# florianwechsung/alfi

Measured on AMD Instinct MI355X. Metric: V-cycles/sec on ldc3d P2-P0 (DoF*smooths/sec in dof_smooths_per_s), higher is better.
Workload: dtype f64

## Files before the change

### alfi_amd/_lib.py

```python
import ctypes
import os

from . import env

_HERE = os.path.dirname(os.path.abspath(__file__))
LIB_PATH = env.hip_lib() or os.path.join(_HERE, "libalfi_hip.so")

c_i32p = ctypes.POINTER(ctypes.c_int32)
c_i64p = ctypes.POINTER(ctypes.c_int64)
c_f64p = ctypes.POINTER(ctypes.c_double)
vp = ctypes.c_void_p


class CsrHost(ctypes.Structure):
    _fields_ = [("nrows", ctypes.c_int64), ("ncols", ctypes.c_int64), ("rowptr", vp), ("colidx", vp), ("vals", vp)]


class BsrHost(ctypes.Structure):
    _fields_ = [("nbrows", ctypes.c_int64), ("nbcols", ctypes.c_int64), ("rowptr", vp), ("colidx", vp), ("vals", vp)]


SIGNATURES = {
    "alfi_ctx_create": (ctypes.c_int, [ctypes.c_int, vp, ctypes.POINTER(vp)]),
    "alfi_ctx_destroy": (ctypes.c_int, [vp]),
# ... 6 lines not shown
    "alfi_memset0": (ctypes.c_int, [vp, vp, ctypes.c_int64]),
    "alfi_prof_enable": (ctypes.c_int, [vp, ctypes.c_int]),
    "alfi_prof_reset": (ctypes.c_int, [vp]),
    "alfi_prof_get": (ctypes.c_int, [vp, ctypes.c_int, ctypes.POINTER(ctypes.c_double), ctypes.POINTER(ctypes.c_int64)]),
    "alfi_prof_get_level": (ctypes.c_int, [vp, ctypes.c_int, ctypes.c_int, ctypes.POINTER(ctypes.c_double),
                                           ctypes.POINTER(ctypes.c_int64)]),
    "alfi_ctx_set_comm": (ctypes.c_int, [vp, vp, vp, vp, ctypes.c_int64]),
    "alfi_comm_unique_id": (ctypes.c_int, [vp, ctypes.c_int64]),
    "alfi_ctx_comm_init": (ctypes.c_int, [vp, vp, ctypes.c_int, ctypes.c_int]),
    "alfi_level_set_sum_exchange": (ctypes.c_int, [vp, ctypes.c_int, vp, vp, vp, ctypes.c_int64, vp, vp, vp]),
    "alfi_ctx_comm_stats": (ctypes.c_int, [vp, ctypes.POINTER(ctypes.c_int64), ctypes.POINTER(ctypes.c_int64),
                                           ctypes.POINTER(ctypes.c_int64), ctypes.c_int]),
    "alfi_ctx_comm_size": (ctypes.c_int, [vp, ctypes.POINTER(ctypes.c_int), ctypes.POINTER(ctypes.c_int)]),
    "alfi_ctx_comm_destroy": (ctypes.c_int, [vp]),
    "alfi_level_set_neighbours": (ctypes.c_int, [vp, ctypes.c_int, vp, vp, vp]),
    "alfi_level_set_partition": (ctypes.c_int, [vp, ctypes.c_int64, ctypes.c_int, ctypes.c_int64, vp, vp, vp,
                                                ctypes.c_int64]),
    "alfi_level_set_overlap": (ctypes.c_int, [vp, ctypes.c_int64, ctypes.c_int64]),
    "alfi_level_id": (ctypes.c_int, [vp, ctypes.POINTER(ctypes.c_int)]),
    "alfi_level_create": (ctypes.c_int, [vp, ctypes.c_int64, ctypes.c_int, vp, vp, vp, vp, ctypes.c_int64,
                                         ctypes.POINTER(vp)]),
    "alfi_level_destroy": (ctypes.c_int, [vp]),
    "alfi_level_update_values": (ctypes.c_int, [vp, vp]),
    "alfi_ctx_comm_allow_self": (ctypes.c_int, [vp, ctypes.c_int]),
    "alfi_vec_axpy": (ctypes.c_int, [vp, vp, vp, ctypes.c_double, ctypes.c_int64]),
    "alfi_vec_copy": (ctypes.c_int, [vp, vp, vp, ctypes.c_int64]),
    "alfi_vec_gather": (ctypes.c_int, [vp, vp, vp, vp, ctypes.c_int64, ctypes.c_int]),
    "alfi_vec_gather_csr": (ctypes.c_int, [vp, vp, vp, vp, vp, vp, ctypes.c_int64, ctypes.c_int]),
    "alfi_level_zero_bc": (ctypes.c_int, [vp, vp]),
    "alfi_saddle_dot": (ctypes.c_int, [vp, vp, vp, ctypes.POINTER(ctypes.c_double)]),
    "alfi_transfer_stats": (ctypes.c_int, [ctypes.POINTER(ctypes.c_int64), ctypes.POINTER(ctypes.c_int64), ctypes.c_int]),
    "alfi_level_halo_sum": (ctypes.c_int, [vp, vp]),
    "alfi_level_set_assembly": (ctypes.c_int, [vp, ctypes.c_int64, ctypes.c_int, vp, vp, vp, vp, vp, vp, ctypes.c_int, vp, vp, vp]),
    "alfi_ctx_set_assembly_scratch": (ctypes.c_int, [vp, ctypes.c_int64]),
    "alfi_level_assemble_supg": (ctypes.c_int, [vp, ctypes.c_double, ctypes.c_double, ctypes.c_double, vp, ctypes.c_double,
                                                ctypes.c_double, ctypes.c_int]),
    "alfi_level_assemble": (ctypes.c_int, [vp, ctypes.c_double, ctypes.c_double, ctypes.c_double, vp, ctypes.c_int]),
    "alfi_level_set_assembly_bc": (ctypes.c_int, [vp, vp, ctypes.c_int64]),
    "alfi_level_assembly_state_size": (ctypes.c_int, [vp, ctypes.POINTER(ctypes.c_int64)]),
    "alfi_level_assemble_mult": (ctypes.c_int, [vp, ctypes.c_double, ctypes.c_double, ctypes.c_double, vp, vp, vp]),
    "alfi_level_set_supg": (ctypes.c_int, [vp, ctypes.c_int, vp, vp, vp, vp, vp]),
    "alfi_level_supg": (ctypes.c_int, [vp, ctypes.c_double, ctypes.c_double, ctypes.c_double, vp, ctypes.c_int, vp]),
    "alfi_level_set_supg_load": (ctypes.c_int, [vp, vp]),
    "alfi_level_assemble_gls": (ctypes.c_int, [vp, ctypes.c_double, ctypes.c_double, ctypes.c_double, vp, vp, ctypes.c_double,
                                               ctypes.c_double, ctypes.c_int]),
    "alfi_level_gls": (ctypes.c_int, [vp, ctypes.c_double, ctypes.c_double, ctypes.c_double, vp, vp, ctypes.c_int, vp]),
    "alfi_level_apply_bc": (ctypes.c_int, [vp]),
    "alfi_level_set_facet_blocks": (ctypes.c_int, [vp, ctypes.c_int]),
    "alfi_level_set_burman": (ctypes.c_int, [vp, ctypes.c_int64, ctypes.c_int, ctypes.c_int, ctypes.c_int, ctypes.c_int] + [vp] * 14),
    "alfi_level_burman": (ctypes.c_int, [vp, ctypes.c_double, vp, ctypes.c_int, vp]),
    "alfi_patches_set_facet_correction": (ctypes.c_int, [vp, ctypes.c_int64, ctypes.c_int64, vp, vp, vp, vp]),
    "alfi_level_set_facet_beta": (ctypes.c_int, [vp, vp, ctypes.c_double]),
    "alfi_level_assemble_burman": (ctypes.c_int, [vp, ctypes.c_double, ctypes.c_double, ctypes.c_double, vp, ctypes.c_double,
                                                  ctypes.c_int]),
    "alfi_level_transpose": (ctypes.c_int, [vp]),
    "alfi_level_get_values": (ctypes.c_int, [vp, vp]),
    "alfi_level_size": (ctypes.c_int, [vp, ctypes.POINTER(ctypes.c_int64)]),
    "alfi_spmv": (ctypes.c_int, [vp, vp, vp]),
    "alfi_residual": (ctypes.c_int, [vp, vp, vp, vp]),
    "alfi_patches_set": (ctypes.c_int, [vp, ctypes.c_int64, vp, vp]),
    "alfi_patches_factor": (ctypes.c_int, [vp]),
    "alfi_patches_set_groups": (ctypes.c_int, [vp, vp]),
    "alfi_patches_factor_bytes": (ctypes.c_int, [vp, ctypes.POINTER(ctypes.c_int64)]),
    "alfi_patches_find_groups": (ctypes.c_int, [vp, vp]),
    "alfi_ctx_set_condense_min_bytes": (ctypes.c_int, [vp, ctypes.c_int64]),
    "alfi_patches_condensed": (ctypes.c_int, [vp, ctypes.POINTER(ctypes.c_int)]),
    "alfi_patches_set_storage": (ctypes.c_int, [vp, ctypes.c_int]),
    "alfi_patches_storage": (ctypes.c_int, [vp, ctypes.POINTER(ctypes.c_int)]),
    "alfi_patches_set_macro_storage": (ctypes.c_int, [vp, ctypes.c_int]),
    "alfi_ctx_set_f32_work_bytes": (ctypes.c_int, [vp, ctypes.c_int64]),
    "alfi_ctx_f32_work_bytes": (ctypes.c_int, [vp, ctypes.POINTER(ctypes.c_int64)]),
    "alfi_patches_set_canonical_order": (ctypes.c_int, [vp, vp]),
    "alfi_patch_apply_split": (ctypes.c_int, [vp, ctypes.c_int64, vp, vp]),
    "alfi_patches_check": (ctypes.c_int, [vp, ctypes.POINTER(ctypes.c_double), ctypes.POINTER(ctypes.c_int64),
                                          ctypes.POINTER(ctypes.c_int64), ctypes.POINTER(ctypes.c_double)]),
    "alfi_patches_set_partition_of_unity": (ctypes.c_int, [vp, ctypes.c_int]),
    "alfi_patches_set_multiplicative": (ctypes.c_int, [vp, ctypes.c_int64, vp, ctypes.c_int]),
    "alfi_patches_multiplicative_levels": (ctypes.c_int, [vp, ctypes.POINTER(ctypes.c_int64)]),
    "alfi_patch_apply": (ctypes.c_int, [vp, vp, vp]),
    "alfi_patches_stats": (ctypes.c_int, [vp, ctypes.POINTER(ctypes.c_int64), ctypes.POINTER(ctypes.c_int64),
                                          ctypes.POINTER(ctypes.c_int64)]),
    "alfi_patch_get_inverse": (ctypes.c_int, [vp, ctypes.c_int64, vp]),
    "alfi_smooth_fgmres": (ctypes.c_int, [vp, ctypes.c_int, vp, vp, ctypes.c_int]),
    "alfi_level_set_jacobi": (ctypes.c_int, [vp, ctypes.c_int]),
    "alfi_smooth_chebyshev": (ctypes.c_int, [vp, ctypes.c_int, ctypes.c_double, ctypes.c_double, vp, vp, ctypes.c_int]),
    "alfi_level_arnoldi": (ctypes.c_int, [vp, ctypes.c_int, vp, vp, ctypes.POINTER(ctypes.c_int)]),
    "alfi_coarse_factor": (ctypes.c_int, [vp]),
    "alfi_coarse_factor_sparse": (ctypes.c_int, [vp, vp, ctypes.c_int, ctypes.c_int]),
    "alfi_coarse_factor_bytes": (ctypes.c_int, [vp, ctypes.POINTER(ctypes.c_int64)]),
    "alfi_coarse_residual": (ctypes.c_int, [vp, ctypes.POINTER(ctypes.c_double)]),
    "alfi_coarse_set_inverse": (ctypes.c_int, [vp, vp, ctypes.c_int]),
    "alfi_coarse_solve": (ctypes.c_int, [vp, vp, vp]),
    "alfi_transfer_create": (ctypes.c_int, [vp, vp, vp, ctypes.POINTER(BsrHost), ctypes.POINTER(BsrHost),
                                            ctypes.POINTER(BsrHost), ctypes.POINTER(BsrHost), ctypes.POINTER(BsrHost),
                                            ctypes.c_int64, ctypes.c_int, vp, vp, vp, ctypes.POINTER(vp)]),
    "alfi_transfer_destroy": (ctypes.c_int, [vp]),
    "alfi_transfer_update": (ctypes.c_int, [vp, ctypes.c_double, ctypes.c_double]),
    "alfi_transfer_get_block_inverse": (ctypes.c_int, [vp, ctypes.c_int64, vp]),
    "alfi_prolong": (ctypes.c_int, [vp, vp, vp]),
    "alfi_transfer_set_injection": (ctypes.c_int, [vp, vp]),
    "alfi_transfer_set_injection_matrix": (ctypes.c_int, [vp, ctypes.POINTER(CsrHost)]),
    "alfi_inject": (ctypes.c_int, [vp, vp, vp]),
    "alfi_restrict": (ctypes.c_int, [vp, vp, vp, ctypes.c_int]),
    "alfi_mg_create": (ctypes.c_int, [vp, ctypes.c_int, ctypes.POINTER(vp), ctypes.POINTER(vp), ctypes.c_int,
                                      ctypes.c_int, ctypes.POINTER(vp)]),
    "alfi_mg_destroy": (ctypes.c_int, [vp]),
    "alfi_mg_vcycle": (ctypes.c_int, [vp, vp, vp]),
    "alfi_mg_fcycle": (ctypes.c_int, [vp, vp, vp]),
    "alfi_mg_set_smoother": (ctypes.c_int, [vp, ctypes.c_int, vp, vp]),
    "alfi_mg_set_cycles": (ctypes.c_int, [vp, ctypes.c_int]),
    "alfi_mg_cg": (ctypes.c_int, [vp, vp, vp, ctypes.c_double, ctypes.c_double, ctypes.c_int, ctypes.c_int,
                                  ctypes.POINTER(ctypes.c_int), ctypes.POINTER(ctypes.c_double)]),
    "alfi_ctx_set_graph": (ctypes.c_int, [vp, ctypes.c_int]),
    "alfi_saddle_create": (ctypes.c_int, [vp, ctypes.POINTER(CsrHost), ctypes.POINTER(CsrHost), vp, ctypes.c_double,
                                          ctypes.c_double, ctypes.c_int, ctypes.POINTER(vp)]),
    "alfi_saddle_destroy": (ctypes.c_int, [vp]),
    "alfi_saddle_set_mass_inverse": (ctypes.c_int, [vp, ctypes.POINTER(CsrHost)]),
    "alfi_saddle_update": (ctypes.c_int, [vp, ctypes.c_double, ctypes.c_double]),
    "alfi_saddle_solve": (ctypes.c_int, [vp, vp, vp, ctypes.c_double, ctypes.c_double, ctypes.c_int, ctypes.c_int,
                                         ctypes.POINTER(ctypes.c_int), ctypes.POINTER(ctypes.c_double)]),
    "alfi_level_halo_forward": (ctypes.c_int, [vp, vp]),
    "alfi_level_halo_reverse_add": (ctypes.c_int, [vp, vp]),
    "alfi_csr_create": (ctypes.c_int, [vp, ctypes.POINTER(CsrHost), ctypes.POINTER(vp)]),
    "alfi_csr_destroy": (ctypes.c_int, [vp]),
    "alfi_csr_mult": (ctypes.c_int, [vp, vp, vp, vp, ctypes.c_double, ctypes.c_int]),
    "alfi_saddle_mult": (ctypes.c_int, [vp, vp, vp]),
    "alfi_saddle_precond": (ctypes.c_int, [vp, vp, vp]),
    "alfi_saddle_set_velocity_solver": (ctypes.c_int, [vp, ctypes.c_int]),
    "alfi_saddle_factor_velocity": (ctypes.c_int, [vp, vp, ctypes.c_int, ctypes.c_int, ctypes.c_int64]),
    "alfi_saddle_velocity_solve": (ctypes.c_int, [vp, vp, vp]),
    "alfi_saddle_velocity_info": (ctypes.c_int, [vp, ctypes.POINTER(ctypes.c_int64), ctypes.POINTER(ctypes.c_double)]),
    "alfi_ctx_set_block_kernels": (ctypes.c_int, [vp, ctypes.c_int]),
    "alfi_patch_apply_block_info": (ctypes.c_int, [vp, ctypes.POINTER(ctypes.c_int)]),
    "alfi_spmv_block_info": (ctypes.c_int, [vp, ctypes.POINTER(ctypes.c_int)]),
    "alfi_patch_apply_block_width": (ctypes.c_int, [vp, ctypes.POINTER(ctypes.c_int)]),
    "alfi_spmv_block_width": (ctypes.c_int, [vp, ctypes.POINTER(ctypes.c_int)]),
    "alfi_ctx_set_block_lds_bytes": (ctypes.c_int, [vp, ctypes.c_int64]),
    "alfi_patch_apply_block": (ctypes.c_int, [vp, ctypes.c_int, vp, ctypes.c_int, vp, ctypes.c_int64, vp, ctypes.c_int64]),
    "alfi_spmv_block": (ctypes.c_int, [vp, ctypes.c_int, vp, ctypes.c_int, vp, ctypes.c_int64, vp, ctypes.c_int64]),
    "alfi_residual_block": (ctypes.c_int, [vp, ctypes.c_int, vp, ctypes.c_int, vp, ctypes.c_int64, vp, ctypes.c_int64, vp,
                                           ctypes.c_int64]),
    "alfi_smooth_fgmres_block_info": (ctypes.c_int, [vp, ctypes.c_int, ctypes.POINTER(ctypes.c_int)]),
    "alfi_smooth_fgmres_block_mode": (ctypes.c_int, [vp, ctypes.c_int, ctypes.POINTER(ctypes.c_int)]),
    "alfi_ctx_set_block_fused": (ctypes.c_int, [vp, ctypes.c_int]),
    "alfi_smooth_fgmres_block": (ctypes.c_int, [vp, ctypes.c_int, ctypes.c_int, vp, ctypes.c_int, vp, ctypes.c_int64, vp,
                                                ctypes.c_int64, ctypes.c_int]),
    "alfi_mg_vcycle_block": (ctypes.c_int, [vp, ctypes.c_int, vp, ctypes.c_int, vp, ctypes.c_int64, vp, ctypes.c_int64]),
    "alfi_mg_fcycle_block": (ctypes.c_int, [vp, ctypes.c_int, vp, ctypes.c_int, vp, ctypes.c_int64, vp, ctypes.c_int64]),
    "alfi_saddle_mult_block": (ctypes.c_int, [vp, ctypes.c_int, vp, ctypes.c_int, vp, ctypes.c_int64, vp, ctypes.c_int64]),
    "alfi_saddle_precond_block": (ctypes.c_int, [vp, ctypes.c_int, vp, ctypes.c_int, vp, ctypes.c_int64, vp, ctypes.c_int64]),
    "alfi_saddle_solve_block": (ctypes.c_int, [vp, ctypes.c_int, vp, ctypes.c_int, vp, ctypes.c_int64, vp, ctypes.c_int64,
                                               ctypes.c_double, ctypes.c_double, ctypes.c_int, ctypes.c_int, vp, vp]),
}

COMM_ID_BYTES = 128

EVENTS = ["PATCH_APPLY", "PATCH_SCATTER", "PATCH_FACTOR", "MATMULT", "BLAS1", "PROLONG", "RESTRICT", "COARSE", "COMM"]
PETSC_EVENT_NAMES = {"PATCH_APPLY": "PCPATCHApply", "PATCH_SCATTER": "PCPATCHScatter", "PATCH_FACTOR": "PCPatchComputeOp",
                     "MATMULT": "MatMult", "BLAS1": "KSPGMRESOrthog", "PROLONG": "SchoeberlProlong", "RESTRICT": "SchoeberlRestrict",
                     "COARSE": "MatSolve", "COMM": "SFBcastOpBegin"}

_lib = None


def comm_unique_id():
    buf = ctypes.create_string_buffer(COMM_ID_BYTES)
    lib = load()
    rc = lib.alfi_comm_unique_id(ctypes.cast(buf, vp), COMM_ID_BYTES)
    if rc != 0:
        raise RuntimeError("alfi_comm_unique_id failed (%d): %s" % (rc, lib.alfi_last_error(None).decode()))
    return buf.raw


def load():
    global _lib
    if _lib is not None:
        return _lib
    try:
        import torch
    except ImportError:
        pass
    if not os.path.exists(LIB_PATH):
        raise RuntimeError("libalfi_hip.so is missing (%s): build it with `python -m alfi_amd.build`; "
                           "alfi_amd has no CPU fallback" % LIB_PATH)
    lib = ctypes.CDLL(LIB_PATH)
    for name, (res, args) in SIGNATURES.items():
        fn = getattr(lib, name)
        fn.restype, fn.argtypes = res, args
    _lib = lib
    return lib
```

### alfi_amd/csrc/api_block.hip

```cpp
#include "api_internal.h"
#include "block_cols.h"

int alfi_ctx_set_block_kernels(alfi_ctx* ctx, int on) {
  if (!ctx) return alfi_set_error(nullptr, ALFI_E_ARG, "NULL context");
  ctx->block_kernels = on != 0;
  return 0;
}
int alfi_ctx_set_block_fused(alfi_ctx* ctx, int on) {
  if (!ctx) return alfi_set_error(nullptr, ALFI_E_ARG, "NULL context");
  ctx->block_fused = on != 0;
  return 0;
}

static int block_apply_waves(const alfi_level* L) {
  if (!L->ctx->block_kernels || !L->factored || L->jacobi || L->mult || level_is_partitioned(L)) return 0;
  if (L->held != HELD_F64 && L->held != HELD_F32) return 0;
  const int W = patch_apply_dense_waves(L, L->held == HELD_F32);
  return patch_apply_block_waves_ok(W) ? W : 0;
}
static int block_cond_apply_width(const alfi_level* L) {
  if (!L->ctx->block_kernels || !L->factored || L->jacobi || L->mult || level_is_partitioned(L)) return 0;
  if (L->held != HELD_COND || L->npatch < COND_PER_PATCH_MIN) return 0;
  if (L->lay.sum_n > INT32_MAX / BLOCK_NV) return 0;
  return block_cond_width(L->cplan.lds_front, L->cplan.lds_back, L->ctx->block_lds_bytes);
}
static int block_big_apply_width(const alfi_level* L) {
  if (!L->ctx->block_kernels || !L->factored || L->jacobi || L->mult || level_is_partitioned(L)) return 0;
  if (L->held != HELD_F64 && L->held != HELD_F32) return 0;
  if (L->lay.max_np <= SMALL_PATCH_MAX || L->npatch < BIG_BLOCK_MIN_PATCHES) return 0;
  if (L->lay.stage_len > INT32_MAX / BLOCK_NV) return 0;
  return block_big_width(L->lay.max_np, L->ctx->block_lds_bytes);
}
static int block_piece_apply_width(const alfi_level* L) {
  return L->held == HELD_COND ? block_cond_apply_width(L) : block_big_apply_width(L);
}
static int block_apply_width(const alfi_level* L) {
  return block_apply_waves(L) != 0 ? BLOCK_NV : block_piece_apply_width(L);
}
static int block_spmv_width(const alfi_level* L) {
  if (!L->ctx->block_kernels || level_is_partitioned(L)) return 0;
  const int w = bsr_spmv_block_width(L->A_own, L->ctx->block_lds_bytes);
  return w >= 2 ? w : 0;
}

int alfi_patch_apply_block_info(alfi_level* L, int* batched) {
  if (!L || !batched) return alfi_set_error(L ? L->ctx : nullptr, ALFI_E_ARG, "alfi_patch_apply_block_info: NULL argument");
  *batched = block_apply_width(L) >= 2 ? 1 : 0;
  return 0;
}
int alfi_patch_apply_block_width(alfi_level* L, int* width) {
  if (!L || !width) return alfi_set_error(L ? L->ctx : nullptr, ALFI_E_ARG, "alfi_patch_apply_block_width: NULL argument");
  *width = block_apply_width(L);
  return 0;
}
int alfi_ctx_set_block_lds_bytes(alfi_ctx* ctx, int64_t bytes) {
  if (!ctx) return alfi_set_error(nullptr, ALFI_E_ARG, "NULL context");
  int limit = 0;
  ALFI_HIP_CHECK(ctx, hipDeviceGetAttribute(&limit, hipDeviceAttributeMaxSharedMemoryPerBlock, ctx->device));
  ctx->block_lds_bytes = (int)std::min<int64_t>(std::max<int64_t>(bytes, 0), limit);
  return 0;
}
static bool level_applies_il(const alfi_level* L) { return L->il_valid && L->held == HELD_F64; }
static int block_smoother_mode(alfi_level* L, int k) {
  BlockSmoothFacts f;
  f.block_kernels = L->ctx->block_kernels;
  f.block_fused = L->ctx->block_fused;
  f.partitioned = level_is_partitioned(L);
  f.fused_iteration = smoother_takes_fused_iteration(L, k);
  f.applies_il = L->factored && level_applies_il(L);
  f.apply_waves = block_apply_waves(L);
  f.piece_width = block_piece_apply_width(L);
  return block_smooth_mode(f);
}
static bool block_smoother_lockstep(alfi_level* L, int k) { return block_smoother_mode(L, k) == BLOCK_SMOOTH_LOCKSTEP; }
int alfi_smooth_fgmres_block_mode(alfi_level* L, int k, int* mode) {
  if (!L || !mode || k < 1) return alfi_set_error(L ? L->ctx : nullptr, ALFI_E_ARG, "alfi_smooth_fgmres_block_mode: bad argument");
  *mode = block_smoother_mode(L, k);
  return 0;
}
int alfi_smooth_fgmres_block_info(alfi_level* L, int k, int* lockstep) {
  if (!L || !lockstep || k < 1) return alfi_set_error(L ? L->ctx : nullptr, ALFI_E_ARG, "alfi_smooth_fgmres_block_info: bad argument");
  *lockstep = block_smoother_lockstep(L, k) ? 1 : 0;
  return 0;
}
int alfi_spmv_block_info(alfi_level* L, int* batched) {
  if (!L || !batched) return alfi_set_error(L ? L->ctx : nullptr, ALFI_E_ARG, "alfi_spmv_block_info: NULL argument");
  *batched = block_spmv_width(L) >= 2 ? 1 : 0;
  return 0;
}
int alfi_spmv_block_width(alfi_level* L, int* width) {
  if (!L || !width) return alfi_set_error(L ? L->ctx : nullptr, ALFI_E_ARG, "alfi_spmv_block_width: NULL argument");
  *width = block_spmv_width(L);
  return 0;
}

int krylov_ws_ensure(alfi_ctx* ctx, KrylovWs* ws, int slots, int K, int64_t n) {
  if (ws->K == K && ws->slots == slots) return 0;
  ALFI_HIP_CHECK(ctx, hipStreamSynchronize(ctx->stream));
  krylov_ws_release(ws);
  ws->ldv = krylov_ldv(n);
  const KrylovWsDoubles d = krylov_ws_doubles(slots, K, ws->ldv);
  ALFI_CHECK(dev_alloc(ctx, &ws->V, d.V));
  ALFI_CHECK(dev_alloc(ctx, &ws->Z, d.Z));
  ALFI_CHECK(dev_alloc(ctx, &ws->w, d.w));
  ALFI_CHECK(dev_alloc(ctx, &ws->hs, d.hs));
  ALFI_HIP_CHECK(ctx, hipMemsetAsync(ws->hs, 0, sizeof(double) * (size_t)d.hs, ctx->stream));
  ws->K = K;
  ws->slots = slots;
  return 0;
}
void krylov_ws_release(KrylovWs* ws) {
  dev_free(ws->V);
  dev_free(ws->Z);
  dev_free(ws->w);
  dev_free(ws->hs);
  *ws = KrylovWs();
}

int slot_buf_resize(alfi_ctx* ctx, SlotBuf* buf, int slots, int64_t per) {
  ALFI_HIP_CHECK(ctx, hipStreamSynchronize(ctx->stream));
  slot_buf_release(buf);
  ALFI_CHECK(dev_alloc(ctx, &buf->p, slots * per));
  ALFI_HIP_CHECK(ctx, hipMemsetAsync(buf->p, 0, sizeof(double) * (size_t)std::max<int64_t>(slots * per, 1), ctx->stream));
  buf->slots = slots;
  buf->per = per;
  return 0;
}
int slot_buf_ensure(alfi_ctx* ctx, SlotBuf* buf, int ncol, int64_t per) {
  const int need = slot_buf_needed(*buf, ncol);
  return need == buf->slots ? 0 : slot_buf_resize(ctx, buf, need, per);
}
void slot_buf_release(SlotBuf* buf) {
  dev_free(buf->p);
  *buf = SlotBuf();
}

void block_release_patch_buffers(alfi_level* L) {
  slot_buf_release(&L->blk_stage);
  slot_buf_release(&L->blk_ctmp);
}
void release_workspaces(alfi_level* L) {
  block_release_patch_buffers(L);
  for (SlotBuf* b : {&L->blk_carry, &L->blk_part, &L->blk_mg_b, &L->blk_mg_x, &L->blk_mg_r}) slot_buf_release(b);
  krylov_ws_release(&L->ws);
  krylov_ws_release(&L->blk_ws);
}
void release_workspaces(alfi_saddle* S) {
  slot_buf_release(&S->blk_tmp_u);
  krylov_ws_release(&S->ws);
  krylov_ws_release(&S->blk_ws);
}

static int ensure_block_smoother(alfi_level* L, int ncol) {
  return krylov_ws_ensure(L->ctx, &L->blk_ws, block_slots_needed(L->blk_ws.slots, ncol), L->ws.K, L->n);
}

int block_patch_apply(alfi_level* L, const BlockCols& ic, const BlockCols& oc, const double* X, int64_t ldx, double* Y, int64_t ldy) {
  alfi_ctx* ctx = L->ctx;
  ctx->cur_tag = L->id;
  const int W = ic.n > 1 ? block_apply_waves(L) : 0;
  if (W != 0) {
    ALFI_CHECK(slot_buf_ensure(ctx, &L->blk_stage, ic.n, L->lay.stage_len));
    return launch_patch_apply_block(L, W, ic, oc, X, ldx, Y, ldy, L->blk_stage.p);
  }
  const int width = ic.n > 1 ? block_piece_apply_width(L) : 0;
  for (int k = 0; k < block_pieces(ic.n, width); ++k) {
    const BlockCols pi = block_piece(ic, width, k), po = block_piece(oc, width, k);
    if (pi.n == 1) {
      ALFI_CHECK(level_patch_apply(L, X + pi.c[0] * ldx, Y + po.c[0] * ldy));
      continue;
    }
    ALFI_CHECK(slot_buf_ensure(ctx, &L->blk_stage, pi.n, L->lay.stage_len));
    if (L->held != HELD_COND) {
      ALFI_CHECK(launch_big_apply_block(L, pi, po, X, ldx, Y, ldy, L->blk_stage.p));
      continue;
    }
    ALFI_CHECK(slot_buf_ensure(ctx, &L->blk_ctmp, pi.n, L->lay.sum_n));
    ALFI_CHECK(launch_cond_apply_block(L, pi, po, X, ldx, Y, ldy, L->blk_stage.p, L->blk_ctmp.p));
  }
  return 0;
}

int block_spmv(alfi_level* L, const BlockCols& ic, const BlockCols& oc, const double* X, int64_t ldx, double* Y, int64_t ldy,
               const double* B, int64_t ldb, int mode) {
  alfi_ctx* ctx = L->ctx;
  ctx->cur_tag = L->id;
  const int width = ic.n > 1 ? block_spmv_width(L) : 0;
  for (int k = 0; k < block_pieces(ic.n, width); ++k) {
    const BlockCols pi = block_piece(ic, width, k), po = block_piece(oc, width, k);
    if (pi.n == 1) {
      ALFI_CHECK(level_spmv(L, X + pi.c[0] * ldx, Y + po.c[0] * ldy, mode ? B + pi.c[0] * ldb : nullptr, mode));
      continue;
    }
    const DevBSR& A = L->A_own;
    if (!A.aligned) {
      const int64_t nchunks = (A.nnzb + SPMV_CHUNK - 1) / SPMV_CHUNK;
      ALFI_CHECK(slot_buf_ensure(ctx, &L->blk_carry, pi.n, nchunks * A.bs));
    }
    ProfScope prof(ctx, ALFI_EV_MATMULT);
    ALFI_CHECK(launch_bsr_spmv_block(ctx, A, pi, po, X, ldx, Y, ldy, B, ldb, 1.0, mode, L->blk_carry.p));
  }
  return 0;
}

static int block_smooth_fgmres_fused(alfi_level* L, int k, const BlockCols& cols, const double* B, int64_t ldb, double* X, int64_t ldx,
                                     int nonzero_guess) {
  alfi_ctx* ctx = L->ctx;
  const int nc = cols.n;
  ALFI_CHECK(ensure_block_smoother(L, nc));
  ALFI_CHECK(slot_buf_ensure(ctx, &L->blk_part, nc, block_partial_per_slot(RED_BLOCKS, RED_MAXV)));
  ALFI_CHECK(slot_buf_ensure(ctx, &L->blk_stage, nc, L->lay.stage_len));
  if (L->held == HELD_COND) ALFI_CHECK(slot_buf_ensure(ctx, &L->blk_ctmp, nc, L->lay.sum_n));
  const int64_t ldv = L->blk_ws.ldv;
  const BlockCols slots = block_chunk(nc, nullptr, 0);
  if (nonzero_guess) ALFI_CHECK(block_spmv(L, cols, slots, X, ldx, L->blk_ws.w, ldv, B, ldb, 1));
  {
    ProfScope prof(ctx, ALFI_EV_BLAS1);
    ALFI_CHECK(launch_first_norm_block(L, cols, nonzero_guess ? nullptr : B, ldb, X, ldx));
  }
  const int G = red_blocks_for(L->n);
  const bool il = level_applies_il(L);
  const int W = il ? 0 : block_apply_waves(L), width = il || W != 0 ? BLOCK_NV : block_piece_apply_width(L);
  const double* stage[BLOCK_NV];
  for (int s = 0; s < BLOCK_NV; ++s) stage[s] = L->blk_stage.slot(s < nc ? s : 0);
  for (int j = 0; j < k; ++j) {
    if (il) {
      ALFI_CHECK(launch_patch_apply_il_block(L, nc, L->blk_ws.w, ldv, L->blk_stage.p));
    } else if (W != 0) {
      ALFI_CHECK(launch_patch_apply_block(L, W, slots, slots, L->blk_ws.w, ldv, nullptr, 0, L->blk_stage.p));
    } else {
      for (int q = 0; q < block_pieces(nc, width); ++q) {
        const BlockCols pi = block_piece(slots, width, q);
        double* st = L->blk_stage.slot(pi.c[0]);
        if (pi.n == 1) {
          ALFI_CHECK(launch_patch_apply_range(L, 0, L->npatch, L->blk_ws.wv(pi.c[0])));
          stage[pi.c[0]] = L->stage;
        } else if (L->held != HELD_COND) {
          ALFI_CHECK(launch_big_apply_block(L, pi, pi, L->blk_ws.w, ldv, nullptr, 0, st));
        } else {
          ALFI_CHECK(launch_cond_apply_block(L, pi, pi, L->blk_ws.w, ldv, nullptr, 0, st, L->blk_ctmp.p));
        }
      }
    }
    {
      ProfScope prof(ctx, ALFI_EV_PATCH_SCATTER);
      ALFI_CHECK(launch_patch_sum_scale_block(L, nc, stage, j == 0 ? 0 : 1, G, j));
    }
    int nb = 0;
    {
      ProfScope prof(ctx, ALFI_EV_MATMULT);
      ALFI_CHECK(launch_bsr_spmv_dot_block(L, nc, j, &nb));
    }
    ProfScope prof(ctx, ALFI_EV_BLAS1);
    ALFI_CHECK(launch_multi_axpy_norm_block(L, nc, j, nb));
  }
  ProfScope prof(ctx, ALFI_EV_BLAS1);
  return launch_fgmres_finish_update_block(L, cols, k, G, X, ldx);
}

int block_smooth_fgmres(alfi_level* L, int k, const BlockCols& cols, const double* B, int64_t ldb, double* X, int64_t ldx,
                        int nonzero_guess) {
  ALFI_CHECK(ensure_fgmres_workspace(L, k));
  L->ctx->cur_tag = L->id;
  const int mode = cols.n == 1 ? BLOCK_SMOOTH_LOOP : block_smoother_mode(L, k);
  if (mode == BLOCK_SMOOTH_FUSED) return block_smooth_fgmres_fused(L, k, cols, B, ldb, X, ldx, nonzero_guess);
  if (mode == BLOCK_SMOOTH_LOOP) {
    for (int i = 0; i < cols.n; ++i) ALFI_CHECK(alfi_smooth_fgmres(L, k, B + cols.c[i] * ldb, X + cols.c[i] * ldx, nonzero_guess));
    return 0;
  }
  ALFI_CHECK(ensure_block_smoother(L, cols.n));
  return smooth_fgmres_general(L, L->blk_ws, k, cols, B, ldb, X, ldx, nonzero_guess);
}

int check_block_call(alfi_level* L, const char* what, int ncol, const int* cols, int nx, const BlockOperand* ops, int nops) {
  if (!L) return alfi_set_error(nullptr, ALFI_E_ARG, "%s: NULL level", what);
  if (level_is_partitioned(L)) return alfi_set_error(L->ctx, ALFI_E_ARG, "%s on a partitioned level (serial levels only)", what);
  return check_block_operands(L->ctx, what, L->n, ncol, cols, nx, ops, nops);
}
int check_block_operands(alfi_ctx* ctx, const char* what, int64_t n, int ncol, const int* cols, int nx, const BlockOperand* ops,
                         int nops) {
  for (int a = 0; a < nops; ++a) {
    if (!ops[a].p) return alfi_set_error(ctx, ALFI_E_ARG, "%s: NULL operand", what);
    if (const char* err = block_operand_error(n, ncol, cols, nx, ops[a].ld)) return alfi_set_error(ctx, ALFI_E_ARG, "%s: %s", what, err);
  }
  for (int a = 0; a < nops; ++a)
    for (int b = 0; b < nops; ++b)
      if (a != b && ops[a].written && block_operands_overlap(ops[a].p, ops[a].ld, ops[b].p, ops[b].ld, nx, n))
        return alfi_set_error(ctx, ALFI_E_ARG, "%s: an operand that is written overlaps another one", what);
  return 0;
}

int alfi_patch_apply_block(alfi_level* L, int ncol, const int* cols, int nx, const double* X, int64_t ldx, double* Y, int64_t ldy) {
  const BlockOperand ops[2] = {{X, ldx, false}, {Y, ldy, true}};
  ALFI_CHECK(check_block_call(L, "alfi_patch_apply_block", ncol, cols, nx, ops, 2));
  if (!level_pc_ready(L)) return alfi_set_error(L->ctx, ALFI_E_STATE, "alfi_patch_apply_block before alfi_patches_factor");
  for (int q = 0; q < block_chunks(ncol); ++q) {
    const BlockCols c = block_chunk(ncol, cols, q);
    ALFI_CHECK(block_patch_apply(L, c, c, X, ldx, Y, ldy));
  }
  return 0;
}

int alfi_spmv_block(alfi_level* L, int ncol, const int* cols, int nx, const double* X, int64_t ldx, double* Y, int64_t ldy) {
  const BlockOperand ops[2] = {{X, ldx, false}, {Y, ldy, true}};
  ALFI_CHECK(check_block_call(L, "alfi_spmv_block", ncol, cols, nx, ops, 2));
  for (int q = 0; q < block_chunks(ncol); ++q) {
    const BlockCols c = block_chunk(ncol, cols, q);
    ALFI_CHECK(block_spmv(L, c, c, X, ldx, Y, ldy, nullptr, 0, 0));
  }
  return 0;
}

int alfi_residual_block(alfi_level* L, int ncol, const int* cols, int nx, const double* B, int64_t ldb, const double* X, int64_t ldx,
                        double* R, int64_t ldr) {
  const BlockOperand ops[3] = {{B, ldb, false}, {X, ldx, false}, {R, ldr, true}};
  ALFI_CHECK(check_block_call(L, "alfi_residual_block", ncol, cols, nx, ops, 3));
  for (int q = 0; q < block_chunks(ncol); ++q) {
    const BlockCols c = block_chunk(ncol, cols, q);
    ALFI_CHECK(block_spmv(L, c, c, X, ldx, R, ldr, B, ldb, 1));
  }
  return 0;
}

int alfi_smooth_fgmres_block(alfi_level* L, int k, int ncol, const int* cols, int nx, const double* B, int64_t ldb, double* X,
                             int64_t ldx, int nonzero_guess) {
  const BlockOperand ops[2] = {{B, ldb, false}, {X, ldx, true}};
  ALFI_CHECK(check_block_call(L, "alfi_smooth_fgmres_block", ncol, cols, nx, ops, 2));
  if (k < 1) return alfi_set_error(L->ctx, ALFI_E_ARG, "k must be >= 1");
  if (!level_pc_ready(L)) return alfi_set_error(L->ctx, ALFI_E_STATE, "alfi_smooth_fgmres_block before alfi_patches_factor");
  for (int q = 0; q < block_chunks(ncol); ++q)
    ALFI_CHECK(block_smooth_fgmres(L, k, block_chunk(ncol, cols, q), B, ldb, X, ldx, nonzero_guess));
  return 0;
}
```

### alfi_amd/csrc/api_cycles.hip

```cpp
#include "api_internal.h"
#include "block_cols.h"

int alfi_coarse_set_inverse(alfi_level* L, const double* inv, int inv_is_device) {
  alfi_ctx* ctx = L->ctx;
  ALFI_HIP_CHECK(ctx, hipStreamSynchronize(ctx->stream));
  if (L->cinv_owned) dev_free(L->cinv);
  L->cinv = nullptr;
  L->cinv_owned = false;
  mf_free(L->mf);
  L->mf = nullptr;
  if (inv_is_device) {
    L->cinv = const_cast<double*>(inv);
  } else {
    ALFI_CHECK(dev_upload(ctx, &L->cinv, inv, L->n * L->n));
    L->cinv_owned = true;
  }
  return 0;
}

int alfi_coarse_factor(alfi_level* L) {
  alfi_ctx* ctx = L->ctx;
  if (L->has_halo && L->n_own != L->n)
    return alfi_set_error(ctx, ALFI_E_STATE, "alfi_coarse_factor needs a level owned by one rank");
  if (L->n > ((int64_t)1 << 17)) return alfi_set_error(ctx, ALFI_E_ARG, "coarse level of %lld dofs: the dense inverse would "
// ... 337 lines not shown
  if (par) ALFI_CHECK(halo_rev(T->coarse, drc));
  ProfScope prof(ctx, ALFI_EV_RESTRICT);
  ALFI_CHECK(launch_zero_dofs(ctx, drc, T->coarse->bc_dofs, T->coarse->nbc));
  return 0;
}

int alfi_mg_create(alfi_ctx* ctx, int nlevels, alfi_level** levels, alfi_transfer** transfers, int k,
                   int robust_restriction, alfi_mg** out) {
  if (!ctx || nlevels < 1 || !levels || (nlevels > 1 && !transfers) || !out)
    return alfi_set_error(ctx, ALFI_E_ARG, "bad arguments");
  for (int l = 1; l < nlevels; ++l) {
    if (transfers[l - 1]->coarse != levels[l - 1] || transfers[l - 1]->fine != levels[l])
      return alfi_set_error(ctx, ALFI_E_ARG, "transfer %d does not link levels %d and %d", l - 1, l - 1, l);
  }
  alfi_mg* mg = new alfi_mg();
  mg->ctx = ctx;
  mg->levels.assign(levels, levels + nlevels);
  if (nlevels > 1) mg->transfers.assign(transfers, transfers + nlevels - 1);
  mg->k = k;
  mg->robust = robust_restriction;
  for (int l = 0; l < nlevels; ++l) {
    alfi_level* L = levels[l];
    int rc = 0;
    if (!L->mg_b) rc = dev_alloc(ctx, &L->mg_b, L->n);
    if (rc == 0 && !L->mg_x) rc = dev_alloc(ctx, &L->mg_x, L->n);
    if (rc == 0 && !L->mg_r) rc = dev_alloc(ctx, &L->mg_r, L->n);
    if (rc == 0 && l > 0 && L->n_own > 0) rc = ensure_fgmres_workspace(L, k);
    if (rc != 0) {
      delete mg;
      return rc;
    }
  }
  *out = mg;
  return 0;
}

int alfi_mg_destroy(alfi_mg* mg) {
  if (!mg) return 0;
  (void)hipStreamSynchronize(mg->ctx->stream);
  for (CycleGraph& g : mg->graphs)
    if (g.exec) (void)hipGraphExecDestroy(g.exec);
  dev_free(mg->cg_r);
  dev_free(mg->cg_z);
  dev_free(mg->cg_p);
  dev_free(mg->cg_w);
  dev_free(mg->cg_s);
  delete mg;
  return 0;
}

static int mg_require_serial(alfi_mg* mg, const char* what) {
  for (alfi_level* L : mg->levels)
    if (level_is_partitioned(L)) return alfi_set_error(mg->ctx, ALFI_E_ARG, "%s on a partitioned hierarchy (serial levels only)", what);
  return 0;
}

int alfi_mg_set_smoother(alfi_mg* mg, int type, const double* emin, const double* emax) {
  if (!mg) return alfi_set_error(nullptr, ALFI_E_ARG, "NULL multigrid");
  alfi_ctx* ctx = mg->ctx;
  if (type != ALFI_SMOOTHER_FGMRES && type != ALFI_SMOOTHER_CHEBYSHEV)
    return alfi_set_error(ctx, ALFI_E_ARG, "smoother type %d (0 FGMRES, 1 Chebyshev)", type);
  if (type == ALFI_SMOOTHER_FGMRES) {
    mg->smoother = type;
    return 0;
  }
  ALFI_CHECK(mg_require_serial(mg, "alfi_mg_set_smoother(Chebyshev)"));
  const int nl = (int)mg->levels.size();
  if (nl > 1 && (!emin || !emax)) return alfi_set_error(ctx, ALFI_E_ARG, "Chebyshev smoother without intervals");
  for (int l = 1; l < nl; ++l)
    if (!(emin[l - 1] > 0.0) || !(emax[l - 1] > emin[l - 1]) || !std::isfinite(emax[l - 1]))
      return alfi_set_error(ctx, ALFI_E_ARG, "Chebyshev interval [%g, %g] of level %d: need 0 < emin < emax", emin[l - 1],
                            emax[l - 1], l);
  for (int l = 1; l < nl; ++l) ALFI_CHECK(ensure_cheb_workspace(mg->levels[l]));
  mg->emin.assign((size_t)nl, 0.0);
  mg->emax.assign((size_t)nl, 0.0);
  for (int l = 1; l < nl; ++l) {
    mg->emin[l] = emin[l - 1];
    mg->emax[l] = emax[l - 1];
  }
  mg->smoother = type;
  return 0;
}

int alfi_mg_set_cycles(alfi_mg* mg, int cycles) {
  if (!mg) return alfi_set_error(nullptr, ALFI_E_ARG, "NULL multigrid");
  if (cycles != 1 && cycles != 2) return alfi_set_error(mg->ctx, ALFI_E_ARG, "cycles %d (1 V, 2 W)", cycles);
  if (cycles > 1) ALFI_CHECK(mg_require_serial(mg, "alfi_mg_set_cycles(W)"));
  mg->cycles = cycles;
  return 0;
}

struct MgWork {
  double *b, *x, *r;
  int64_t ld;
};
typedef MgWork (*MgWorkOf)(const alfi_level*);
static MgWork own_work(const alfi_level* L) { return {L->mg_b, L->mg_x, L->mg_r, 0}; }
static MgWork block_work(const alfi_level* L) { return {L->blk_mg_b.p, L->blk_mg_x.p, L->blk_mg_r.p, L->blk_mg_b.per}; }

static int mg_smooth(alfi_mg* mg, int l, const BlockCols& cols, const double* B, int64_t ldb, double* X, int64_t ldx,
                     int nonzero_guess) {
  alfi_level* L = mg->levels[l];
  if (mg->smoother == ALFI_SMOOTHER_CHEBYSHEV) {
    for (int i = 0; i < cols.n; ++i)
      ALFI_CHECK(alfi_smooth_chebyshev(L, mg->k, mg->emin[l], mg->emax[l], B + cols.c[i] * ldb, X + cols.c[i] * ldx, nonzero_guess));
    return 0;
  }
  return block_smooth_fgmres(L, mg->k, cols, B, ldb, X, ldx, nonzero_guess);
}

static int vcycle(alfi_mg* mg, MgWorkOf work, int l, const BlockCols& cols, const double* B, int64_t ldb, double* X, int64_t ldx,
                  bool x_zero) {
  alfi_ctx* ctx = mg->ctx;
  alfi_level* L = mg->levels[l];
  const int nc = cols.n;
  if (l == 0) {
    for (int i = 0; i < nc && L->n_own > 0; ++i) ALFI_CHECK(alfi_coarse_solve(L, B + cols.c[i] * ldb, X + cols.c[i] * ldx));
    return 0;
  }
  alfi_transfer* T = mg->transfers[l - 1];
  const BlockCols slots = block_chunk(nc, nullptr, 0);
  const MgWork wl = work(L), wc = work(mg->levels[l - 1]);
  ALFI_CHECK(mg_smooth(mg, l, cols, B, ldb, X, ldx, x_zero ? 0 : 1));
  ALFI_CHECK(block_spmv(L, cols, slots, X, ldx, wl.r, wl.ld, B, ldb, 1));
  for (int i = 0; i < nc; ++i) ALFI_CHECK(alfi_restrict(T, wl.r + i * wl.ld, wc.b + i * wc.ld, mg->robust));
  const int cycles = l == 1 ? 1 : mg->cycles;
  for (int c = 0; c < cycles; ++c) ALFI_CHECK(vcycle(mg, work, l - 1, slots, wc.b, wc.ld, wc.x, wc.ld, c == 0));
  for (int i = 0; i < nc; ++i) ALFI_CHECK(alfi_prolong(T, wc.x + i * wc.ld, wl.r + i * wl.ld));
  ctx->cur_tag = L->id;
  for (int i = 0; i < nc; ++i) {
    ProfScope prof(ctx, ALFI_EV_BLAS1);
    ALFI_CHECK(launch_axpy(ctx, X + cols.c[i] * ldx, wl.r + i * wl.ld, 1.0, L->n_own));
  }
  return mg_smooth(mg, l, cols, B, ldb, X, ldx, 1);
}

static int fcycle(alfi_mg* mg, MgWorkOf work, const BlockCols& cols, const double* B, int64_t ldb, double* X, int64_t ldx) {
  const int Lmax = (int)mg->levels.size() - 1, nc = cols.n;
  if (Lmax == 0) return vcycle(mg, work, 0, cols, B, ldb, X, ldx, false);
  const BlockCols slots = block_chunk(nc, nullptr, 0);
  for (int i = 0; i < nc; ++i) {
    const double* bf = B + cols.c[i] * ldb;
    for (int l = Lmax; l >= 1; --l) {
      const MgWork wc = work(mg->levels[l - 1]);
      ALFI_CHECK(alfi_restrict(mg->transfers[l - 1], bf, wc.b + i * wc.ld, mg->robust));
      bf = wc.b + i * wc.ld;
    }
  }
  for (int l = 0; l < Lmax; ++l) {
    const MgWork wl = work(mg->levels[l]), wn = work(mg->levels[l + 1]);
    ALFI_CHECK(vcycle(mg, work, l, slots, wl.b, wl.ld, wl.x, wl.ld, l == 0));
    for (int i = 0; i < nc; ++i)
      ALFI_CHECK(alfi_prolong(mg->transfers[l], wl.x + i * wl.ld, l + 1 == Lmax ? X + cols.c[i] * ldx : wn.x + i * wn.ld));
  }
  return vcycle(mg, work, Lmax, cols, B, ldb, X, ldx, false);
}

static void cycle_signature(alfi_mg* mg, std::vector<uint64_t>* sig) {
  auto push = [&](const void* q) { sig->push_back((uint64_t)(uintptr_t)q); };
  auto pushd = [&](double v) {
    uint64_t u;
    memcpy(&u, &v, sizeof(u));
    sig->push_back(u);
  };
  sig->clear();
  sig->push_back((uint64_t)mg->k);
  sig->push_back((uint64_t)mg->robust);
  sig->push_back((uint64_t)mg->smoother);
  sig->push_back((uint64_t)mg->cycles);
  if (mg->smoother == ALFI_SMOOTHER_CHEBYSHEV)
    for (size_t l = 1; l < mg->levels.size(); ++l) {
      pushd(mg->emin[l]);
      pushd(mg->emax[l]);
    }
  for (alfi_level* L : mg->levels) {
    sig->push_back((uint64_t)(L->jacobi ? 1 : 0));
    push(L->jac_diag);
    push(L->cheb_d);
    push(L->A.vals);
    push(L->inv);
    push(L->inv32);
    sig->push_back((uint64_t)(L->held == HELD_F32 ? 1 : 0));
    push(L->cd.mat);
    push(L->cd.sinv);
    push(L->patch_ptr);
    push(L->patch_dofs);
    push(L->cinv);
    push(L->mf);
    push(L->ws.V);
    push(L->mult_seq);
    sig->push_back((uint64_t)L->npatch);
    sig->push_back((uint64_t)L->ws.K);
    sig->push_back((uint64_t)(L->mult ? 1 + (L->mult_symmetrise ? 1 : 0) + 4 * L->sweep.wave_ptr.size() : 0));
  }
  for (alfi_transfer* T : mg->transfers) {
    push(T->binv);
    pushd(T->nu);
    pushd(T->gamma);
  }
}

static int mg_ready(alfi_mg* mg) {
  alfi_ctx* ctx = mg->ctx;
  for (size_t l = 1; l < mg->levels.size(); ++l) {
    alfi_level* L = mg->levels[l];
    if (L->n_own > 0 && !level_pc_ready(L))
      return alfi_set_error(ctx, ALFI_E_STATE, "level %d: patches not factored", (int)l);
    if (mg->smoother == ALFI_SMOOTHER_CHEBYSHEV) ALFI_CHECK(ensure_cheb_workspace(L));
    if (L->jacobi && L->jac_version != L->op_version) {
      ALFI_CHECK(launch_jacobi_diag(ctx, L->A, L->jac_diag));
      L->jac_version = L->op_version;
    }
  }
  alfi_level* C = mg->levels[0];
  if (C->n_own > 0 && !C->cinv && !C->mf) return alfi_set_error(ctx, ALFI_E_STATE, "coarse level has no inverse");
  return 0;
}

static int run_cycle(alfi_mg* mg, int kind, const double* db, double* dx) {
  alfi_ctx* ctx = mg->ctx;
  ALFI_CHECK(mg_ready(mg));
  const BlockCols one = block_chunk(1, nullptr, 0);
  auto eager = [&]() {
    return kind ? fcycle(mg, own_work, one, db, 0, dx, 0) : vcycle(mg, own_work, (int)mg->levels.size() - 1, one, db, 0, dx, 0, false);
  };
  bool ok = ctx->use_graph && ctx->prof == 0;
  for (alfi_level* L : mg->levels) ok = ok && !L->has_halo;
  if (!ok) return eager();
  std::vector<uint64_t> sig;
  cycle_signature(mg, &sig);
  CycleGraph* G = nullptr;
  for (CycleGraph& g : mg->graphs)
    if (g.kind == kind && g.b == db && g.x == dx) G = &g;
  if (!G) {
    if (mg->graphs.size() >= 16) {
      for (CycleGraph& g : mg->graphs)
        if (g.exec) (void)hipGraphExecDestroy(g.exec);
      mg->graphs.clear();
    }
    CycleGraph g;
    g.kind = kind;
    g.b = db;
    g.x = dx;
    mg->graphs.push_back(g);
    return eager();
  }
  if (G->failed) return eager();
  if (G->exec && G->sig != sig) {
    (void)hipGraphExecDestroy(G->exec);
    G->exec = nullptr;
  }
  if (!G->exec) {
// ... 147 lines not shown
```

### alfi_amd/csrc/api_internal.h

```cpp
#pragma once
#include <cmath>
#include <cstdarg>
#include <cstdlib>
#include <cstring>
#include <algorithm>
#include "common.h"
#include "hs_layout.h"

template <typename T>
inline int dev_alloc(alfi_ctx* ctx, T** p, int64_t count) {
  *p = nullptr;
  if (count <= 0) count = 1;
  ALFI_HIP_CHECK(ctx, hipMalloc((void**)p, (size_t)count * sizeof(T)));
  return 0;
}
template <typename T>
inline int dev_upload(alfi_ctx* ctx, T** p, const T* host, int64_t count) {
  ALFI_CHECK(dev_alloc(ctx, p, count));
  if (count > 0) ALFI_HIP_CHECK(ctx, hipMemcpy(*p, host, (size_t)count * sizeof(T), hipMemcpyHostToDevice));
  return 0;
}
inline void dev_free(void* p) {
  if (p) (void)hipFree(p);
}
template <typename T>
inline int cond_upload(alfi_level* L, const T** dst, const std::vector<T>& src) {
  T* d = nullptr;
  ALFI_CHECK(dev_upload(L->ctx, &d, src.data(), (int64_t)src.size()));
  L->cond_allocs.push_back(d);
  *dst = d;
  return 0;
}

int check_dev_err(alfi_ctx* ctx);
int build_chunk_tables(alfi_ctx* ctx, DevBSR* d, const int32_t* rowptr, int64_t nbrows, int64_t break_row,
                       int64_t* nchunks_before = nullptr);
int upload_bsr(alfi_ctx* ctx, DevBSR* d, const alfi_bsr_host* h, int bs);
void free_bsr(DevBSR* d);
void free_cond(alfi_level* L);
int comm_allreduce(alfi_level* L, int64_t offset, int64_t count);
int halo_fwd(alfi_level* L, double* v);
int halo_fwd_begin(alfi_level* L, const double* v);
int halo_fwd_end(alfi_level* L, double* v);
int halo_rev(alfi_level* L, double* v);
int halo_sum(alfi_level* L, double* v);
int halo_rev_begin(alfi_level* L, const double* v);
int halo_rev_end(alfi_level* L, double* v);
void free_assembly(AssemblyDev* S);
int level_spmv(alfi_level* L, const double* dx, double* dy, const double* db, int mode, bool ghosts_current = false);
int level_patch_apply(alfi_level* L, const double* dx, double* dy, bool* ghosts_current = nullptr);
inline bool level_pc_ready(const alfi_level* L) { return L->factored || L->jacobi; }
inline bool level_is_partitioned(const alfi_level* L) { return L->distributed || L->has_halo || L->n_own != L->n; }
inline void set_held(alfi_level* L, PatchStoreHeld h) {
  L->held = h;
  L->cond = h == HELD_COND;
}
inline bool wants_f32(const alfi_level* L) { return L->store_req != STORE_REQ_F64; }
inline bool is_or_will_be_f32(const alfi_level* L) { return wants_f32(L) || L->held == HELD_F32; }
inline bool cond_by_caller(const alfi_level* L) { return L->cond && L->cond_by == COND_BY_CALLER; }
inline bool cond_by_own_choice(const alfi_level* L) { return L->cond && L->cond_by == COND_BY_LIBRARY; }
inline bool facet_rule_active(const alfi_level* L) { return L->fc_ptr && L->fc_scale != 0.0; }
void free_patch_factors(alfi_level* L);
void free_mult_schedule(alfi_level* L);
bool auto_cond_to_dense(alfi_level* L);
int ensure_fgmres_workspace(alfi_level* L, int k);
int ensure_cheb_workspace(alfi_level* L);
bool smoother_takes_fused_iteration(const alfi_level* L, int k, bool* flat_spmv = nullptr);
int smooth_fgmres_general(alfi_level* L, const KrylovWs& ws, int k, const BlockCols& cols, const double* B, int64_t ldb, double* X,
                          int64_t ldx, int nonzero_guess);
int krylov_ws_ensure(alfi_ctx* ctx, KrylovWs* ws, int slots, int K, int64_t n);
void krylov_ws_release(KrylovWs* ws);
int slot_buf_ensure(alfi_ctx* ctx, SlotBuf* buf, int ncol, int64_t per);
int slot_buf_resize(alfi_ctx* ctx, SlotBuf* buf, int slots, int64_t per);
void slot_buf_release(SlotBuf* buf);
void block_release_patch_buffers(alfi_level* L);
void release_workspaces(alfi_level* L);
void release_workspaces(alfi_saddle* S);
struct BlockCols;
struct BlockOperand {
  const double* p;
  int64_t ld;
  bool written;
};
int check_block_call(alfi_level* L, const char* what, int ncol, const int* cols, int nx, const BlockOperand* ops, int nops);
int check_block_operands(alfi_ctx* ctx, const char* what, int64_t n, int ncol, const int* cols, int nx, const BlockOperand* ops,
                         int nops);
int mg_fcycle_block_chunk(alfi_mg* mg, const BlockCols& cols, const double* B, int64_t ldb, double* X, int64_t ldx);
int block_patch_apply(alfi_level* L, const BlockCols& ic, const BlockCols& oc, const double* X, int64_t ldx, double* Y, int64_t ldy);
int block_spmv(alfi_level* L, const BlockCols& ic, const BlockCols& oc, const double* X, int64_t ldx, double* Y, int64_t ldy,
               const double* B, int64_t ldb, int mode);
int block_smooth_fgmres(alfi_level* L, int k, const BlockCols& cols, const double* B, int64_t ldb, double* X, int64_t ldx,
                        int nonzero_guess);
int upload_csr(alfi_ctx* ctx, DevCSR* d, const alfi_csr_host* h);
void free_csr(DevCSR* d);
```

### alfi_amd/csrc/api_saddle.hip

```cpp
#include "api_internal.h"
#include "block_cols.h"

int upload_csr(alfi_ctx* ctx, DevCSR* d, const alfi_csr_host* h) {
  d->nrows = h->nrows;
  d->ncols = h->ncols;
  d->nnz = h->rowptr[h->nrows];
  ALFI_CHECK(dev_upload(ctx, &d->rowptr, h->rowptr, h->nrows + 1));
  ALFI_CHECK(dev_upload(ctx, &d->colidx, h->colidx, d->nnz));
  ALFI_CHECK(dev_upload(ctx, &d->vals, h->vals, d->nnz));
  return 0;
}
void free_csr(DevCSR* d) {
  dev_free(d->rowptr);
  dev_free(d->colidx);
  dev_free(d->vals);
  *d = DevCSR();
}

int alfi_level_halo_forward(alfi_level* L, double* dv) {
  if (!L->distributed) return 0;
  L->ctx->cur_tag = L->id;
  return halo_fwd(L, dv);
}

// ... 435 lines not shown
    ctx->cur_tag = F->id;
    return comm_allreduce(F, offset, count);
  };
  auto list = [&](const bool* on) {
    BlockCols b = block_chunk(nc, nullptr, 0);
    int m = 0;
    for (int s = 0; s < nc; ++s)
      if (on[s]) b.c[m++] = s;
    b.n = m;
    for (int i = m; i < BLOCK_NV; ++i) b.c[i] = m ? b.c[0] : 0;
    return b;
  };
  auto read = [&](const bool* on, int off, double* out) -> int {
    for (int s = 0; s < nc; ++s)
      if (on[s]) ALFI_HIP_CHECK(ctx, hipMemcpyAsync(out + s, ws.h(s) + off, sizeof(double), hipMemcpyDeviceToHost, ctx->stream));
    ALFI_HIP_CHECK(ctx, hipStreamSynchronize(ctx->stream));
    return 0;
  };
  auto norm_init = [&](int s) -> int {
    ALFI_CHECK(launch_norm_partials(ctx, ws.wv(s), n));
    if (par) {
      ALFI_CHECK(launch_reduce_partials(ctx, ctx->red_partial, G, 1, nrm2));
      ALFI_CHECK(allreduce(RED_MAXV, 1));
      return launch_norm_init_finish(ctx, nrm2, 1, ws.h(s), K);
    }
    return launch_norm_init_finish(ctx, ctx->red_partial, G, ws.h(s), K);
  };
  bool active[BLOCK_NV] = {false, false, false, false}, all[BLOCK_NV] = {false, false, false, false};
  double bnorm[BLOCK_NV] = {0, 0, 0, 0}, tol[BLOCK_NV] = {0, 0, 0, 0}, val[BLOCK_NV] = {0, 0, 0, 0};
  int its[BLOCK_NV] = {0, 0, 0, 0};
  for (int s = 0; s < nc; ++s) {
    all[s] = true;
    ALFI_HIP_CHECK(ctx, hipMemsetAsync(ws.h(s), 0, sizeof(double) * hl.total, ctx->stream));
    ALFI_HIP_CHECK(ctx, hipMemsetAsync(xcol(s), 0, sizeof(double) * n, ctx->stream));
    ALFI_CHECK(launch_copy(ctx, ws.wv(s), bcol(s), n));
    ALFI_CHECK(norm_init(s));
  }
  ALFI_CHECK(read(all, hl.beta, bnorm));
  int nactive = 0;
  for (int s = 0; s < nc; ++s) {
    tol[s] = std::max(rtol * bnorm[s], atol);
    active[s] = !(bnorm[s] <= tol[s]);
    nactive += active[s] ? 1 : 0;
  }
  auto residual_of = [&](const bool* on) -> int {
    for (int s = 0; s < nc; ++s) {
      if (!on[s]) continue;
      ALFI_CHECK(alfi_saddle_mult(S, xcol(s), ws.wv(s)));
      ALFI_CHECK(launch_xmy(ctx, ws.wv(s), bcol(s), n));
      ALFI_CHECK(norm_init(s));
    }
    return 0;
  };
  int it = 0;
  while (nactive > 0 && it < max_it) {
    for (int s = 0; s < nc; ++s)
      if (active[s]) ALFI_CHECK(launch_scale_by_inv(ctx, ws.v(s, 0), ws.wv(s), ws.h(s) + hl.beta, n));
    int j = 0;
    bool cycle[BLOCK_NV];
    for (int s = 0; s < nc; ++s) cycle[s] = active[s];
    int ncycle = nactive;
    for (; j < K && it < max_it && ncycle > 0; ++j) {
      const BlockCols a = list(cycle);
      ALFI_CHECK(saddle_precond_chunk(S, a, nc, ws.v(0, j), ws.vs(), ws.z(0, j), ws.zs()));
      ALFI_CHECK(saddle_mult_chunk(S, a, ws.z(0, j), ws.zs(), ws.w, ldv));
      for (int s = 0; s < nc; ++s) {
        if (!cycle[s]) continue;
        double *hs = ws.h(s), *hdots = hdots_of(s);
        ALFI_CHECK(launch_multi_dot(ctx, ws.v(s, 0), ldv, j + 1, ws.wv(s), hdots, n));
        if (par) ALFI_CHECK(allreduce(0, j + 1));
        ALFI_CHECK(launch_multi_axpy_norm(ctx, ws.v(s, 0), ldv, j + 1, hdots, ws.wv(s), n, ctx->red_partial2, 0));
        if (par) {
          ALFI_CHECK(launch_reduce_partials(ctx, ctx->red_partial2, G, 1, nrm2));
          ALFI_CHECK(allreduce(RED_MAXV, 1));
        }
        ALFI_CHECK(launch_hessenberg_update(ctx, normpart, nblk, hdots, hs, j, K, nullptr));
      }
      ++it;
      ALFI_CHECK(read(cycle, hl.grs + j + 1, val));
      for (int s = 0; s < nc; ++s) {
        if (!cycle[s]) continue;
        its[s] = it;
        if (std::fabs(val[s]) <= tol[s]) {
          ALFI_CHECK(launch_fgmres_finish(ctx, ws.h(s), j + 1, K));
          ALFI_CHECK(launch_update_solution(ctx, xcol(s), ws.z(s, 0), ldv, j + 1, ws.h(s) + hl.y, n));
          cycle[s] = active[s] = false;
          --ncycle;
          --nactive;
        } else if (j + 1 < K) {
          ALFI_CHECK(launch_scale_by_inv(ctx, ws.v(s, j + 1), ws.wv(s), ws.h(s) + hl.tt, n));
        }
      }
    }
    for (int s = 0; s < nc; ++s) {
      if (!cycle[s]) continue;
      ALFI_CHECK(launch_fgmres_finish(ctx, ws.h(s), j, K));
      ALFI_CHECK(launch_update_solution(ctx, xcol(s), ws.z(s, 0), ldv, j, ws.h(s) + hl.y, n));
    }
    if (nactive == 0 || it >= max_it) break;
    ALFI_CHECK(residual_of(active));
    ALFI_CHECK(read(active, hl.beta, val));
    for (int s = 0; s < nc; ++s)
      if (active[s] && val[s] <= tol[s]) {
        active[s] = false;
        --nactive;
      }
  }
  ALFI_CHECK(residual_of(all));
  ALFI_CHECK(read(all, hl.beta, val));
  for (int s = 0; s < nc; ++s) {
    its_out[s] = its[s];
    rn_out[s] = val[s];
  }
  return 0;
}

static int check_restart(alfi_ctx* ctx, int restart) {
  if (restart < 1 || restart > RED_MAXV - 2) return alfi_set_error(ctx, ALFI_E_ARG, "restart must be in 1..%d", RED_MAXV - 2);
  return 0;
}

int alfi_saddle_solve(alfi_saddle* S, const double* db, double* dx, double rtol, double atol, int max_it, int restart,
                      int* iterations, double* residual_norm) {
  alfi_ctx* ctx = S->ctx;
  ALFI_CHECK(check_restart(ctx, restart));
  ALFI_CHECK(krylov_ws_ensure(ctx, &S->ws, 1, restart, S->nu_dofs + S->np_dofs));
  int its = 0;
  double rn = 0.0;
  ALFI_CHECK(saddle_solve_chunk(S, S->ws, block_chunk(1, nullptr, 0), db, 0, dx, 0, rtol, atol, max_it, &its, &rn));
  if (iterations) *iterations = its;
  if (residual_norm) *residual_norm = rn;
  return check_dev_err(ctx);
}

int alfi_saddle_solve_block(alfi_saddle* S, int ncol, const int* cols, int nx, const double* B, int64_t ldb, double* X, int64_t ldx,
                            double rtol, double atol, int max_it, int restart, int* iterations, double* residual_norms) {
  const BlockOperand ops[2] = {{B, ldb, false}, {X, ldx, true}};
  ALFI_CHECK(saddle_block_check(S, "alfi_saddle_solve_block", ncol, cols, nx, ops, 2));
  alfi_ctx* ctx = S->ctx;
  if (!iterations || !residual_norms) return alfi_set_error(ctx, ALFI_E_ARG, "alfi_saddle_solve_block: NULL result arrays");
  ALFI_CHECK(check_restart(ctx, restart));
  ALFI_CHECK(krylov_ws_ensure(ctx, &S->blk_ws, block_slots_needed(S->blk_ws.slots, ncol), restart, S->nu_dofs + S->np_dofs));
  for (int q = 0; q < block_chunks(ncol); ++q)
    ALFI_CHECK(saddle_solve_chunk(S, S->blk_ws, block_chunk(ncol, cols, q), B, ldb, X, ldx, rtol, atol, max_it,
                                  iterations + q * BLOCK_NV, residual_norms + q * BLOCK_NV));
  return check_dev_err(ctx);
}
```

### alfi_amd/csrc/api_smoother.hip

```cpp
#include <optional>
#include "api_internal.h"

int ensure_fgmres_workspace(alfi_level* L, int k) {
  if (k <= L->ws.K) return 0;
  if (k > RED_MAXV - 1) return alfi_set_error(L->ctx, ALFI_E_ARG, "k = %d exceeds the supported maximum %d", k, RED_MAXV - 1);
  return krylov_ws_ensure(L->ctx, &L->ws, 1, k, L->n);
}

static int smooth_fgmres_fused(alfi_level* L, int k, const double* db, double* dx, int nonzero_guess, bool flat_spmv) {
  alfi_ctx* ctx = L->ctx;
  const int K = L->ws.K;
  const int64_t n = L->n, ldv = L->ws.ldv;
  HsLayout hl(K);
  double *V = L->ws.V, *Z = L->ws.Z, *w = L->ws.w, *hs = L->ws.hs;
  double* hdots = hs + hl.hd;
  if (nonzero_guess) {
    ALFI_CHECK(alfi_residual(L, db, dx, w));
  } else {
    ALFI_HIP_CHECK(ctx, hipMemsetAsync(dx, 0, sizeof(double) * n, ctx->stream));
    ProfScope prof(ctx, ALFI_EV_BLAS1);
    ALFI_CHECK(launch_copy(ctx, w, db, n));
  }
  {
    ProfScope prof(ctx, ALFI_EV_BLAS1);
    ALFI_CHECK(launch_norm_partials(ctx, w, n));
  }
  const int G = red_blocks_for(n);
  const double* normpart = ctx->red_partial;
  for (int j = 0; j < k; ++j) {
    double* zj = Z + (int64_t)j * ldv;
    ALFI_CHECK(launch_patch_apply_range(L, 0, L->npatch, w));
    {
      ProfScope prof(ctx, ALFI_EV_PATCH_SCATTER);
      ALFI_CHECK(launch_patch_sum_scale(L, w, zj, V + (int64_t)j * ldv, normpart, G, hdots, hs, j, K));
    }
    int nb = 0;
    if (!flat_spmv) {
      ProfScope prof(ctx, ALFI_EV_MATMULT);
      ALFI_CHECK(launch_bsr_spmv_dot(ctx, L->A_own, zj, w, V, ldv, j + 1, ctx->red_partial, &nb));
    } else {
      const bool in_consumer = G <= 256;
      {
        ProfScope prof(ctx, ALFI_EV_MATMULT);
        ALFI_CHECK(launch_bsr_spmv(ctx, L->A_own, zj, w, nullptr, 1.0, 0));
      }
      ProfScope prof(ctx, ALFI_EV_BLAS1);
      ALFI_CHECK(launch_multi_dot(ctx, V, ldv, j + 1, w, in_consumer ? nullptr : hdots, n));
      nb = in_consumer ? G : 0;
    }
    ProfScope prof(ctx, ALFI_EV_BLAS1);
    ALFI_CHECK(launch_multi_axpy_norm(ctx, V, ldv, j + 1, hdots, w, n, ctx->red_partial2, nb));
    normpart = ctx->red_partial2;
  }
  ProfScope prof(ctx, ALFI_EV_BLAS1);
  ALFI_CHECK(launch_fgmres_finish_fused(ctx, normpart, G, hdots, hs, k, K));
  ALFI_CHECK(launch_update_solution(ctx, dx, Z, ldv, k, hs + hl.y, n));
  return 0;
}

bool smoother_takes_fused_iteration(const alfi_level* L, int k, bool* flat_spmv) {
  constexpr int64_t small_n = 50000;
  const bool fusable = !alfi_test_large_paths() && !L->distributed && L->n_own == L->n && !L->mult && k + 1 <= 16 &&
                       L->A_own.flat && !L->jacobi;
  const bool short_rows = L->max_row_blocks <= 32 || L->n <= small_n;
  if (flat_spmv) *flat_spmv = !short_rows;
  return fusable && short_rows;
}

int alfi_smooth_fgmres(alfi_level* L, int k, const double* db, double* dx, int nonzero_guess) {
  alfi_ctx* ctx = L->ctx;
  if (k < 1) return alfi_set_error(ctx, ALFI_E_ARG, "k must be >= 1");
  if (!level_pc_ready(L)) return alfi_set_error(ctx, ALFI_E_STATE, "alfi_smooth_fgmres before alfi_patches_factor");
  ALFI_CHECK(ensure_fgmres_workspace(L, k));
  ctx->cur_tag = L->id;
  bool flat_spmv = false;
  if (smoother_takes_fused_iteration(L, k, &flat_spmv)) return smooth_fgmres_fused(L, k, db, dx, nonzero_guess, flat_spmv);
  return smooth_fgmres_general(L, L->ws, k, block_chunk(1, nullptr, 0), db, 0, dx, 0, nonzero_guess);
}

namespace {
class Blas1Event {
 public:
  explicit Blas1Event(alfi_ctx* ctx) : ctx_(ctx) { open(); }
  void open() { ev_.emplace(ctx_, ALFI_EV_BLAS1); }
  void close() { ev_.reset(); }

 private:
  alfi_ctx* ctx_;
  std::optional<ProfScope> ev_;
};
}

int smooth_fgmres_general(alfi_level* L, const KrylovWs& ws, int k, const BlockCols& cols, const double* B, int64_t ldb, double* X,
                          int64_t ldx, int nonzero_guess) {
  alfi_ctx* ctx = L->ctx;
  const int K = ws.K, nc = cols.n;
  const bool one = nc == 1;
  const int64_t n = L->n_own;
  const int64_t ldv = ws.ldv;
  const bool par = L->distributed;
  HsLayout hl(K);
  const BlockCols slots = block_chunk(nc, nullptr, 0);
  auto hdots_of = [&](int s) { return par ? ctx->dred : ws.h(s) + hl.hd; };
  double* nrm2 = par ? ctx->dred + RED_MAXV : nullptr;
  auto event_ends = [&](Blas1Event& ev, bool reduce, int64_t offset, int64_t count) -> int {
    if (!one) return 0;
    ev.close();
    if (reduce) ALFI_CHECK(comm_allreduce(L, offset, count));
    ev.open();
    return 0;
  };
  if (nonzero_guess) {
    ALFI_CHECK(block_spmv(L, cols, slots, X, ldx, ws.w, ldv, B, ldb, 1));
  } else {
    for (int s = 0; s < nc; ++s) {
      ALFI_HIP_CHECK(ctx, hipMemsetAsync(X + cols.c[s] * ldx, 0, sizeof(double) * L->n, ctx->stream));
      ProfScope prof(ctx, ALFI_EV_BLAS1);
      ALFI_CHECK(launch_copy(ctx, ws.wv(s), B + cols.c[s] * ldb, n));
    }
  }
  const int G = red_blocks_for(n);
  const bool fused = !par && G <= 256 && k + 1 <= 16;
  const double* part1 = par ? nrm2 : ctx->red_partial;
  const double* part2 = par ? nrm2 : ctx->red_partial2;
  const int nblk = par ? 1 : G;
  for (int s = 0; s < nc; ++s) {
    Blas1Event ev(ctx);
    ALFI_CHECK(launch_norm_partials(ctx, ws.wv(s), n));
    if (par) ALFI_CHECK(launch_reduce_partials(ctx, ctx->red_partial, G, 1, nrm2));
    ALFI_CHECK(event_ends(ev, par, RED_MAXV, 1));
    ALFI_CHECK(launch_norm_init_finish(ctx, part1, nblk, ws.h(s), K));
    ALFI_CHECK(launch_scale_by_inv(ctx, ws.v(s, 0), ws.wv(s), ws.h(s) + hl.beta, n));
  }
  for (int j = 0; j < k; ++j) {
    if (one) {
      bool zghosts = false;
      ALFI_CHECK(level_patch_apply(L, ws.v(0, j), ws.z(0, j), &zghosts));
      ALFI_CHECK(level_spmv(L, ws.z(0, j), ws.w, nullptr, 0, zghosts));
    } else {
      ALFI_CHECK(block_patch_apply(L, slots, slots, ws.v(0, j), ws.vs(), ws.z(0, j), ws.zs()));
      ALFI_CHECK(block_spmv(L, slots, slots, ws.z(0, j), ws.zs(), ws.w, ldv, nullptr, 0, 0));
    }
    const bool pyth = par && !ctx->exact_norm;
    for (int s = 0; s < nc; ++s) {
      double *V = ws.v(s, 0), *w = ws.wv(s), *hs = ws.h(s), *hdots = hdots_of(s);
      const double* ww = pyth ? hdots + (j + 1) : nullptr;
      Blas1Event ev(ctx);
      ALFI_CHECK(launch_multi_dot(ctx, V, ldv, j + 1, w, fused ? nullptr : hdots, n));
      if (pyth) {
        ALFI_CHECK(launch_norm_partials(ctx, w, n));
        ALFI_CHECK(launch_reduce_partials(ctx, ctx->red_partial, G, 1, hdots + (j + 1)));
      }
      ALFI_CHECK(event_ends(ev, par, 0, pyth ? j + 2 : j + 1));
      ALFI_CHECK(launch_multi_axpy_norm(ctx, V, ldv, j + 1, hdots, w, n, ctx->red_partial2, fused ? G : 0));
      if (par && !pyth) ALFI_CHECK(launch_reduce_partials(ctx, ctx->red_partial2, G, 1, nrm2));
      ALFI_CHECK(event_ends(ev, par && !pyth, RED_MAXV, 1));
      if (j + 1 < k)
        ALFI_CHECK(launch_hessenberg_scale(ctx, part2, nblk, hdots, hs, j, K, ws.v(s, j + 1), w, n, ww));
      else
        ALFI_CHECK(launch_hessenberg_update(ctx, part2, nblk, hdots, hs, j, K, ww));
    }
  }
  for (int s = 0; s < nc; ++s) {
    ProfScope prof(ctx, ALFI_EV_BLAS1);
    ALFI_CHECK(launch_fgmres_finish(ctx, ws.h(s), k, K));
    ALFI_CHECK(launch_update_solution(ctx, X + cols.c[s] * ldx, ws.z(s, 0), ldv, k, ws.h(s) + hl.y, n));
  }
  return 0;
}

int ensure_cheb_workspace(alfi_level* L) {
  alfi_ctx* ctx = L->ctx;
  if (L->cheb_d) return 0;
  ALFI_HIP_CHECK(ctx, hipSetDevice(ctx->device));
  ALFI_CHECK(dev_alloc(ctx, &L->cheb_r, L->n));
  ALFI_CHECK(dev_alloc(ctx, &L->cheb_z, L->n));
  ALFI_CHECK(dev_alloc(ctx, &L->cheb_d, L->n));
  return 0;
}

int alfi_smooth_chebyshev(alfi_level* L, int k, double emin, double emax, const double* db, double* dx, int nonzero_guess) {
  if (!L) return alfi_set_error(nullptr, ALFI_E_ARG, "NULL level");
  alfi_ctx* ctx = L->ctx;
  if (level_is_partitioned(L))
    return alfi_set_error(ctx, ALFI_E_ARG, "alfi_smooth_chebyshev on a partitioned level (serial levels only)");
  if (k < 1) return alfi_set_error(ctx, ALFI_E_ARG, "k must be >= 1");
  if (!(emin > 0.0) || !(emax > emin) || !std::isfinite(emax))
    return alfi_set_error(ctx, ALFI_E_ARG, "Chebyshev interval [%g, %g]: need 0 < emin < emax", emin, emax);
  if (!db || !dx || db == dx) return alfi_set_error(ctx, ALFI_E_ARG, "alfi_smooth_chebyshev: b and x must be distinct vectors");
  if (!level_pc_ready(L)) return alfi_set_error(ctx, ALFI_E_STATE, "alfi_smooth_chebyshev before alfi_patches_factor");
  ALFI_CHECK(ensure_cheb_workspace(L));
  ctx->cur_tag = L->id;
  const int64_t n = L->n;
  const double theta = 0.5 * (emax + emin), delta = 0.5 * (emax - emin), sigma1 = theta / delta;
  double rho = 1.0 / sigma1;
  for (int i = 0; i < k; ++i) {
    const bool x_is_zero = i == 0 && !nonzero_guess;
    const double* r = db;
    if (!x_is_zero) {
      ALFI_CHECK(alfi_residual(L, db, dx, L->cheb_r));
      r = L->cheb_r;
    }
    ALFI_CHECK(level_patch_apply(L, r, L->cheb_z));
    double a = 0.0, c = 1.0 / theta;
    if (i > 0) {
      const double rho_new = 1.0 / (2.0 * sigma1 - rho);
      a = rho_new * rho;
      c = 2.0 * rho_new / delta;
      rho = rho_new;
    }
    ProfScope prof(ctx, ALFI_EV_BLAS1);
    ALFI_CHECK(launch_cheb_update(ctx, L->cheb_d, dx, L->cheb_z, a, c, n, i > 0 ? 0 : (x_is_zero ? 2 : 1)));
  }
  return 0;
}

int alfi_level_arnoldi(alfi_level* L, int m, const double* dv0, double* H_host, int* m_done) {
  if (!L) return alfi_set_error(nullptr, ALFI_E_ARG, "NULL level");
  alfi_ctx* ctx = L->ctx;
  if (level_is_partitioned(L))
    return alfi_set_error(ctx, ALFI_E_ARG, "alfi_level_arnoldi on a partitioned level (serial levels only)");
  if (m < 1 || m > 30) return alfi_set_error(ctx, ALFI_E_ARG, "Arnoldi steps %d not in 1..30", m);
  if (!dv0 || !H_host || !m_done) return alfi_set_error(ctx, ALFI_E_ARG, "NULL argument");
  if (!level_pc_ready(L)) return alfi_set_error(ctx, ALFI_E_STATE, "alfi_level_arnoldi before alfi_patches_factor");
  ALFI_HIP_CHECK(ctx, hipSetDevice(ctx->device));
  ctx->cur_tag = L->id;
  const int64_t n = L->n, ld = krylov_ldv(n);
  const int G = red_blocks_for(n);
  const int ldh = m + 2;
  double *V = nullptr, *z = nullptr, *w = nullptr, *Hd = nullptr;
  int rc = dev_alloc(ctx, &V, (int64_t)(m + 1) * ld);
  if (rc == 0) rc = dev_alloc(ctx, &z, ld);
  if (rc == 0) rc = dev_alloc(ctx, &w, ld);
  if (rc == 0) rc = dev_alloc(ctx, &Hd, (int64_t)m * ldh);
  if (rc == 0 && hipMemsetAsync(Hd, 0, sizeof(double) * m * ldh, ctx->stream) != hipSuccess) rc = ALFI_E_HIP;
  auto run = [&]() -> int {
    double* beta = Hd + (m + 1);
    {
      ProfScope prof(ctx, ALFI_EV_BLAS1);
      ALFI_CHECK(launch_norm_partials(ctx, dv0, n));
      ALFI_CHECK(launch_reduce_partials(ctx, ctx->red_partial, G, 1, beta));
      ALFI_CHECK(launch_sqrt_inplace(ctx, beta));
      ALFI_CHECK(launch_scale_by_inv(ctx, V, dv0, beta, n));
    }
    for (int j = 0; j < m; ++j) {
      double* h = Hd + (int64_t)j * ldh;
      ALFI_CHECK(level_spmv(L, V + (int64_t)j * ld, z, nullptr, 0));
      ALFI_CHECK(level_patch_apply(L, z, w));
// ... 33 lines not shown
```

### alfi_amd/csrc/common.h

```cpp
#pragma once
#include <hip/hip_runtime.h>
#include <atomic>
#include <cstdint>
#include <cstdio>
#include <string>
#include <thread>
#include <vector>
#include "alfi_hip.h"
#include "env.h"
#include "krylov_ws.h"
#include "patch_plan.h"

inline std::atomic<int64_t> g_alfi_h2d_bytes{0}, g_alfi_d2h_bytes{0};
inline hipError_t alfi_counted_memcpy(void* dst, const void* src, size_t n, hipMemcpyKind kind) {
  if (kind == hipMemcpyHostToDevice) g_alfi_h2d_bytes += (int64_t)n;
  else if (kind == hipMemcpyDeviceToHost) g_alfi_d2h_bytes += (int64_t)n;
  return hipMemcpy(dst, src, n, kind);
}
inline hipError_t alfi_counted_memcpy_async(void* dst, const void* src, size_t n, hipMemcpyKind kind, hipStream_t s) {
  if (kind == hipMemcpyHostToDevice) g_alfi_h2d_bytes += (int64_t)n;
  else if (kind == hipMemcpyDeviceToHost) g_alfi_d2h_bytes += (int64_t)n;
  return hipMemcpyAsync(dst, src, n, kind, s);
}
#define hipMemcpy(dst, src, n, kind) alfi_counted_memcpy(dst, src, n, kind)
// ... 311 lines not shown
  double* chk = nullptr;
  int32_t* chk_list = nullptr;
  int chk_cap = 0;
  double chk_worst = -1.0, chk_worst_after = -1.0;
  int64_t chk_flagged = 0, chk_repaired = 0;
  PatchStoreRequest store_req = STORE_REQ_F64;
  PatchStoreHeld held = HELD_NONE;
  CondDecision cond_by = COND_UNDECIDED;
  bool cond = false;
  CondDev cd;
  std::vector<void*> cond_allocs;
  CondPlan cplan;
  float* inv32 = nullptr;
  int64_t* inv32_ptr = nullptr;
  std::vector<int64_t> f32_ptr;
  int64_t inv32_floats = 0;
  int32_t* canon_rank = nullptr;
  bool mult = false, mult_symmetrise = false;
  int32_t* mult_seq = nullptr;
  SweepPlan sweep;
  int32_t *mult_items = nullptr, *mult_pred0 = nullptr, *mult_pred = nullptr, *mult_succ_ptr = nullptr, *mult_succ = nullptr;
  int32_t* mult_ctl = nullptr;
  int32_t* mult_rowtab = nullptr;
  KrylovWs ws, blk_ws;
  SlotBuf blk_part;
  bool jacobi = false;
  double* jac_diag = nullptr;
  uint64_t jac_version = ~(uint64_t)0;
  double *cheb_r = nullptr, *cheb_z = nullptr, *cheb_d = nullptr;
  double* cinv = nullptr;
  bool cinv_owned = false;
  struct MfDev* mf = nullptr;
  double cinv_residual = -1.0;
  double *mg_b = nullptr, *mg_x = nullptr, *mg_r = nullptr;
  SlotBuf blk_mg_b, blk_mg_x, blk_mg_r;
};

struct alfi_transfer {
  alfi_ctx* ctx = nullptr;
  alfi_level *coarse = nullptr, *fine = nullptr;
  int bs = 0;
  DevBSR P, PT, PTp, DI, DIT;
  bool ptp_alias = false;
  int64_t nblk = 0;
  int m = 0, ld = 0;
  int32_t* blk_dofs = nullptr;
  double *KII = nullptr, *DII = nullptr;
  double* binv = nullptr;
  bool patch_mode = false;
  int64_t bstride = 0;
  int64_t *pm_ptr = nullptr, *pm_inv_ptr = nullptr, *pm_stage_ptr = nullptr;
  int32_t* pm_iota = nullptr;
  double* pm_tmp = nullptr;
  double* pm_res = nullptr;
  double* pm_cor = nullptr;
  double* AIIt = nullptr;
  double *tI = nullptr, *bI = nullptr;
  double* tmp_f = nullptr;
  int32_t* inj = nullptr;
  struct DevCSR* injm = nullptr;
  double gamma = 0, nu = 0;
  bool ready = false;
  int* status = nullptr;
};

struct CycleGraph {
  int kind = 0;
  const double* b = nullptr;
  double* x = nullptr;
  std::vector<uint64_t> sig;
  hipGraphExec_t exec = nullptr;
  bool failed = false;
};

struct alfi_mg {
  alfi_ctx* ctx = nullptr;
  std::vector<alfi_level*> levels;
  std::vector<alfi_transfer*> transfers;
  int k = 0;
  int robust = 0;
  int smoother = 0;
  std::vector<double> emin, emax;
  int cycles = 1;
  double *cg_r = nullptr, *cg_z = nullptr, *cg_p = nullptr, *cg_w = nullptr, *cg_s = nullptr;
  std::vector<CycleGraph> graphs;
};

struct DevCSR {
  int64_t nrows = 0, ncols = 0, nnz = 0;
  int32_t* rowptr = nullptr;
  int32_t* colidx = nullptr;
  double* vals = nullptr;
};

struct alfi_saddle {
  alfi_ctx* ctx = nullptr;
  alfi_mg* mg = nullptr;
  alfi_level* fine = nullptr;
  int64_t nu_dofs = 0, np_dofs = 0;
  DevCSR B, BT;
  double* minv = nullptr;
  DevCSR Minv;
  bool has_Minv = false;
  double nu = 0, gamma = 0;
  bool remove_nullspace = false;
  bool par = false;
  int64_t n_loc = 0;
  double np_global = 0.0;
  double *wa = nullptr, *wb = nullptr, *wc = nullptr;
  KrylovWs ws, blk_ws;
  double *tmp_u = nullptr, *tmp_p = nullptr;
  double* dotbuf = nullptr;
  SlotBuf blk_tmp_u;
  int vkind = 0;
  struct MfDev* vmf = nullptr;
  uint64_t vmf_version = 0;
  double vmf_residual = -1.0;
};

int launch_bsr_spmv(alfi_ctx* ctx, const DevBSR& A, const double* x, double* y, const double* b, double alpha, int mode);
int upload_bsr_values(alfi_ctx* ctx, DevBSR* d, const double* host_vals);
int build_spmv_dedup(alfi_ctx* ctx, DevBSR* d);
struct BlockCols;
int bsr_spmv_block_width(const DevBSR& A, int64_t budget_bytes);
bool bsr_spmv_block_batched(const DevBSR& A, int64_t budget_bytes);
bool bsr_spmv_is_dedup(const DevBSR& A);
int launch_bsr_spmv_dedup_block(alfi_ctx* ctx, const DevBSR& A, const BlockCols& cols, const BlockCols& ocols, const double* X,
                                int64_t ldx, double* Y, int64_t ldy, const double* B, int64_t ldb, double alpha, int mode,
                                double* carry);
int launch_bsr_spmv_block(alfi_ctx* ctx, const DevBSR& A, const BlockCols& cols, const BlockCols& ocols, const double* X,
                          int64_t ldx, double* Y, int64_t ldy, const double* B, int64_t ldb, double alpha, int mode, double* carry);
int patch_apply_dense_waves(const alfi_level* lvl, bool f32);
bool patch_apply_block_waves_ok(int W);
int launch_patch_apply_block(alfi_level* lvl, int W, const BlockCols& cols, const BlockCols& ocols, const double* X, int64_t ldx,
                             double* Y, int64_t ldy, double* stage);
int launch_patch_sum_block(alfi_level* lvl, const BlockCols& cols, const BlockCols& ocols, const double* X, int64_t ldx, double* Y,
                           int64_t ldy, const double* stage);
int launch_cond_apply_block(alfi_level* lvl, const BlockCols& cols, const BlockCols& ocols, const double* X, int64_t ldx, double* Y,
                            int64_t ldy, double* stage, double* ctmp);
int launch_big_apply_block(alfi_level* lvl, const BlockCols& cols, const BlockCols& ocols, const double* X, int64_t ldx, double* Y,
                           int64_t ldy, double* stage);
int launch_patch_apply_il_block(alfi_level* lvl, int nc, const double* X, int64_t ldx, double* stage);
int launch_first_norm_block(alfi_level* lvl, const BlockCols& cols, const double* B, int64_t ldb, double* X, int64_t ldx);
int launch_patch_sum_scale_block(alfi_level* lvl, int nc, const double* const* stage, int normset, int nblocks, int j);
int launch_bsr_spmv_dot_block(alfi_level* lvl, int nc, int j, int* nblocks);
int launch_multi_axpy_norm_block(alfi_level* lvl, int nc, int j, int hblocks);
int launch_fgmres_finish_update_block(alfi_level* lvl, const BlockCols& cols, int k, int nblocks, double* X, int64_t ldx);
int launch_patch_gather_dense(alfi_level* lvl, double* inv, bool ranked);
int launch_patch_invert(alfi_level* lvl, double* inv);
struct PatchCheckAcc {
  double worst = -1.0, worst_after = -1.0;
  int64_t flagged = 0, repaired = 0;
};
int patch_probe_vector(alfi_level* lvl, double** probe_vec);
int patch_verify_and_repair_range(alfi_level* lvl, double* inv, int unpivoted_status, int64_t p0, int64_t p1,
                                  const double* probe_vec, PatchCheckAcc* acc);
int patch_check_finish(alfi_level* lvl, const PatchCheckAcc& acc);
int launch_patch_invert_arrays(alfi_ctx* ctx, int64_t npatch, int max_np, const int64_t* patch_ptr,
                               const int64_t* inv_ptr, double* inv, int* status);
int launch_patch_apply_arrays(alfi_ctx* ctx, int64_t npatch, const int64_t* patch_ptr, const int32_t* patch_dofs,
                              const int64_t* inv_ptr, const int64_t* stage_ptr, const double* inv, const double* x,
                              double* stage);
int launch_patch_apply(alfi_level* lvl, const double* x, double* y);
int launch_patch_apply_range(alfi_level* lvl, int64_t p0, int64_t p1, const double* x);
int launch_patch_apply_f64_range(alfi_level* lvl, const double* inv, int64_t p0, int64_t p1, const double* x);
int launch_big_apply_range(alfi_level* lvl, const double* inv, int64_t p0, int64_t p1, const double* x);
int launch_big_factor_transfer(alfi_transfer* tr);
int launch_big_apply_arrays(alfi_ctx* ctx, int64_t npatch, int max_np, const int64_t* patch_ptr,
                            const int32_t* patch_dofs, const int64_t* inv_ptr, const int64_t* stage_ptr, const double* inv,
                            const double* x, double* stage);
int mf_factor(alfi_level* lvl, const double* coords, int dim, int leaf_nodes);
int mf_solve(alfi_level* lvl, const double* b, double* x);
int mf_factor_slot(alfi_level* lvl, struct MfDev** slot, const double* coords, int dim, int leaf_nodes, int64_t max_bytes);
int mf_solve_slot(alfi_level* lvl, const struct MfDev* m, const double* b, double* x);
void mf_free(struct MfDev* m);
int64_t mf_bytes(const struct MfDev* m);
int launch_coarse_factor(alfi_level* lvl, double* out);
int launch_big_factor_range(alfi_level* lvl, double* inv, int64_t p0, int64_t p1);
int launch_big_apply_f32_range(alfi_level* lvl, int64_t p0, int64_t p1, const double* x);
int launch_cond_factor(alfi_level* lvl);
int launch_cond_apply_range(alfi_level* lvl, int64_t p0, int64_t p1, const double* x);
int launch_cond_schur_one(alfi_level* lvl, int64_t p, const int64_t* d_zero, double* scr);
int launch_patch_f32_convert_range(alfi_level* lvl, const double* src, int64_t p0, int64_t p1);
int launch_patch_unrank(alfi_level* lvl, double* inv);
int build_patch_il(alfi_level* lvl, const double* inv);
int launch_patch_sum(alfi_level* lvl, const double* x, double* y);
int launch_patch_sum_range(alfi_level* lvl, int64_t i0, int64_t i1, const double* x, double* y);
int launch_patch_mult_wave(alfi_level* lvl, const int32_t* seq, int64_t count, const double* x, double* y);
int launch_patch_mult_persistent(alfi_level* lvl, const double* x, double* y);
int launch_big_mult_wave(alfi_level* lvl, const int32_t* seq, int64_t count, const double* x, double* y);
int launch_big_mult_persistent(alfi_level* lvl, const double* x, double* y);
int launch_invert_small_any(alfi_ctx* ctx, int nmax, int64_t nmat, const int64_t* ptr, const int64_t* inv_ptr,
                            int fixed_n, int64_t fixed_stride, double* inv, int* status);
int launch_block_build_invert(alfi_transfer* tr);
int launch_block_gemv(alfi_transfer* tr, const double* in, double* out, bool gather_in);
int launch_scatter_sub(alfi_ctx* ctx, double* x, const int32_t* idx, const double* t, double alpha, int64_t n);
int launch_zero_dofs(alfi_ctx* ctx, double* x, const int32_t* idx, int64_t n);
int launch_copy_dofs(alfi_ctx* ctx, double* y, const double* x, const int32_t* idx, int64_t n);
int launch_dense_gemv(alfi_ctx* ctx, const double* A, const double* x, double* y, int64_t n);
int launch_copy(alfi_ctx* ctx, double* y, const double* x, int64_t n);
int launch_axpy(alfi_ctx* ctx, double* y, const double* x, double a, int64_t n);
int launch_norm_partials(alfi_ctx* ctx, const double* r, int64_t n);
int launch_norm_init_finish(alfi_ctx* ctx, const double* partial, int nblocks, double* hs, int K);
int launch_reduce_partials(alfi_ctx* ctx, const double* partial, int nblocks, int nv, double* out);
int red_blocks_for(int64_t n);
int launch_hessenberg_update(alfi_ctx* ctx, const double* partial, int nblocks, const double* h, double* hs, int j,
                             int K, const double* ww);
int launch_hessenberg_scale(alfi_ctx* ctx, const double* partial, int nblocks, const double* h, double* hs, int j, int K,
                            double* vnext, const double* w, int64_t n, const double* ww);
int launch_csr_spmv(alfi_ctx* ctx, const DevCSR& A, const double* x, double* y, const double* b, double alpha, int mode);
int launch_scale_rows(alfi_ctx* ctx, double* y, const double* x, const double* d, double a, int64_t n);
int launch_remove_mean(alfi_ctx* ctx, double* x, int64_t n);
int launch_inject_csr(alfi_ctx* ctx, const struct DevCSR& J, int bs, const double* xf, double* xc);
int launch_gather_csr(alfi_ctx* ctx, double* dst, const double* src, const int32_t* rowptr, const int32_t* colidx,
                      const double* w, int64_t nrows, int bs);
int launch_sum_to(alfi_ctx* ctx, const double* x, int64_t n, double* out);
int launch_sub_scaled(alfi_ctx* ctx, double* x, int64_t n, const double* s, double f);
int launch_add(alfi_ctx* ctx, double* y, const double* a, const double* b, int64_t n);
int launch_xmy(alfi_ctx* ctx, double* w, const double* b, int64_t n);
int launch_halo_pack(alfi_ctx* ctx, double* buf, const double* v, const int32_t* nodes, int64_t nnodes, int bs);
int launch_halo_sum(alfi_ctx* ctx, double* v, const double* buf, const int32_t* nodes, const int32_t* ptr, const int32_t* src,
                    int64_t nshared, int bs);
int launch_halo_add(alfi_ctx* ctx, double* v, const double* buf, const int32_t* rev_nodes, const int32_t* rev_ptr,
                    const int32_t* rev_pos, int64_t nuniq, int bs);
int launch_scale_by_inv(alfi_ctx* ctx, double* v, const double* w, const double* scal, int64_t n);
int launch_multi_dot(alfi_ctx* ctx, const double* V, int64_t stride, int nv, const double* w, double* out, int64_t n);
int launch_multi_axpy_norm(alfi_ctx* ctx, const double* V, int64_t stride, int nv, double* h, double* w, int64_t n,
                           double* norm_partial, int hblocks);
int launch_fgmres_finish(alfi_ctx* ctx, double* hs, int k, int K);
int launch_patch_sum_scale(alfi_level* lvl, const double* w, double* z, double* v, const double* normpart, int nblocks,
                           const double* h, double* hs, int j, int K);
int launch_bsr_spmv_dot(alfi_ctx* ctx, const DevBSR& A, const double* z, double* w, const double* V, int64_t stride, int nv,
                        double* partial, int* nblocks);
enum { ALFI_STAB_NONE = 0, ALFI_STAB_SUPG = 1, ALFI_STAB_GLS = 2 };
int launch_operator_refresh(alfi_level* lvl, double nu, double gamma, double adv, const double* d_state, bool with_elements,
                            int stab, const double* d_wind, double weight, double magic, bool accumulate, bool apply_bc,
                            double* out_vals);
int launch_element_mult(alfi_level* lvl, double nu, double gamma, double adv, const double* d_state, const double* dx, double* dy);
int launch_supg_residual(alfi_level* lvl, double nu, double weight, double magic, const double* d_state, const double* d_wind,
                         double* d_F);
int launch_burman(alfi_level* lvl, double weight, const double* d_state, bool add_to_operator, double* d_F);
int launch_patch_facet_correct(alfi_level* lvl, int64_t p0, int64_t nb, const int64_t* mat_ptr, double* dst, int big);
bool element_kernel_exists(int d, int nloc);
int launch_vals_from_lanes(alfi_ctx* ctx, const DevBSR& A, double* d_out);
int launch_transpose_mirror(alfi_ctx* ctx, const DevBSR& A, int32_t* mirror, int* bad);
int launch_transpose_swap(alfi_ctx* ctx, const DevBSR& A, const int32_t* mirror);
int launch_probe_fill(alfi_ctx* ctx, double* e, int64_t n);
int launch_probe_residual(alfi_ctx* ctx, const double* r, int64_t n, double* worst_host);
int launch_apply_bc(alfi_level* lvl);
int launch_patch_invert_mfma(alfi_ctx* ctx, int64_t npatch, int max_np, const int64_t* patch_ptr, const int64_t* inv_ptr,
                             double* inv, int* status, int* handled);
int launch_fgmres_finish_fused(alfi_ctx* ctx, const double* normpart, int nblocks, const double* h, double* hs, int k, int K);
int launch_update_solution(alfi_ctx* ctx, double* x, const double* Z, int64_t stride, int k, const double* y, int64_t n);
int launch_cheb_update(alfi_ctx* ctx, double* d, double* x, const double* z, double a, double c, int64_t n, int mode);
int launch_jacobi_diag(alfi_ctx* ctx, const DevBSR& A, double* diag);
int launch_jacobi_apply(alfi_ctx* ctx, double* y, const double* x, const double* diag, const uint8_t* bc, int64_t n);
int launch_cg_update_xr(alfi_ctx* ctx, double* x, double* r, const double* p, const double* w, const double* s, int cur, int64_t n);
int launch_cg_update_p(alfi_ctx* ctx, double* p, const double* z, const double* s, int cur, int first, int64_t n);
int launch_sqrt_inplace(alfi_ctx* ctx, double* s);
```

### alfi_amd/csrc/hs_layout.h

```cpp
#pragma once
#ifdef __HIPCC__
#define HS_LAYOUT_HD __host__ __device__
#else
#define HS_LAYOUT_HD
#endif
struct HsLayout {
  int K;
  int beta, tt, cs, sn, grs, y, hd, total;
  HS_LAYOUT_HD explicit HsLayout(int K_) : K(K_) {
    beta = 0;
    tt = 1;
    cs = 8 + K * (K + 1);
    sn = cs + K;
    grs = sn + K;
    y = grs + K + 1;
    hd = y + K;
    total = hd + K + 1;
  }
  HS_LAYOUT_HD int H(int j) const { return 8 + j * (K + 1); }
};
#undef HS_LAYOUT_HD

#ifdef __HIPCC__
__device__ inline double pythagoras_norm2(const double* ww, const double* h, int j) {
  double s = *ww;
  for (int i = 0; i <= j; ++i) s -= h[i] * h[i];
  return s > 0.0 ? s : 0.0;
}

__device__ inline void hessenberg_column(double* __restrict__ hs, int K, int j, const double* __restrict__ h,
                                                  double tt) {
  HsLayout L(K);
  hs[L.tt] = tt;
  double* hcol = hs + L.H(j);
  for (int i = 0; i <= j; ++i) hcol[i] = h[i];
  hcol[j + 1] = tt;
  double* cs = hs + L.cs;
  double* sn = hs + L.sn;
  double* grs = hs + L.grs;
  for (int i = 0; i < j; ++i) {
    const double t = hcol[i];
    hcol[i] = cs[i] * t + sn[i] * hcol[i + 1];
    hcol[i + 1] = -sn[i] * t + cs[i] * hcol[i + 1];
  }
  const double den = hypot(hcol[j], hcol[j + 1]);
  if (den != 0.0) {
    cs[j] = hcol[j] / den;
    sn[j] = hcol[j + 1] / den;
  } else {
    cs[j] = 1.0;
    sn[j] = 0.0;
  }
  grs[j + 1] = -sn[j] * grs[j];
  grs[j] = cs[j] * grs[j];
  hcol[j] = den;
  hcol[j + 1] = 0.0;
}


__device__ inline void fgmres_back_substitution(double* __restrict__ hs, int k, int K) {
  HsLayout L(K);
  double* y = hs + L.y;
  const double* grs = hs + L.grs;
  for (int i = k - 1; i >= 0; --i) {
    double s = grs[i];
    for (int q = i + 1; q < k; ++q) s -= hs[L.H(q) + i] * y[q];
    const double d = hs[L.H(i) + i];
    y[i] = d != 0.0 ? s / d : 0.0;
  }
}
#endif
```

### alfi_amd/csrc/kernels_block_fused.hip

```cpp
#include "common.h"
#include "hs_layout.h"
#include "block_cols.h"
#include "reduce.h"
#include "load_pair.h"

template <int G, bool NT, int NV>
__global__ __launch_bounds__(256) void patch_apply_il_block_kernel(int64_t p0, int64_t p1, int nc,
                                                                    const int64_t* __restrict__ patch_ptr,
                                                                    const int32_t* __restrict__ patch_dofs,
                                                                    const int64_t* __restrict__ stage_ptr,
                                                                    const double* __restrict__ il,
                                                                    const double* __restrict__ X, int64_t ldx,
                                                                    double* __restrict__ stage, int64_t stage_len) {
  constexpr int PW = 64 / G, LW = PW * G;
  const int wave = threadIdx.x >> 6, lane = threadIdx.x & 63;
  const int64_t w = p0 / PW + (int64_t)blockIdx.x * 4 + wave;
  const int q = lane / G, l = lane - q * G;
  const int64_t p = w * PW + q;
  const bool inwave = lane < LW && w * PW < p1;
  const bool live = inwave && p >= p0 && p < p1;
  int n = 0;
  int64_t off = 0;
  if (live) {
    off = patch_ptr[p];
// ... 185 lines not shown
}

__global__ __launch_bounds__(256) void first_norm_block_kernel(const double* __restrict__ B, int64_t ldb, double* __restrict__ X,
                                                                int64_t ldx, BlockCols cols, double* __restrict__ W, int64_t ldw,
                                                                double* __restrict__ partial, int64_t pstride, int64_t n) {
  const int s = blockIdx.y;
  double* w = W + s * ldw;
  const int64_t n2 = n >> 1;
  const bool last = (n & 1) && blockIdx.x == gridDim.x - 1 && threadIdx.x == 255;
  if (B) {
    const int64_t c = block_col(cols, s);
    const double* b = B + c * ldb;
    double* x = X + c * ldx;
    for (int64_t i = (int64_t)blockIdx.x * 256 + threadIdx.x; i < n2; i += (int64_t)gridDim.x * 256) {
      vec_d2 t;
      t.x = b[2 * i];
      t.y = b[2 * i + 1];
      st2(w, i, t);
      x[2 * i] = 0.0;
      x[2 * i + 1] = 0.0;
    }
    if (last) {
      w[n - 1] = b[n - 1];
      x[n - 1] = 0.0;
    }
  }
  double acc[1] = {0.0};
#pragma unroll 2
  for (int64_t i = (int64_t)blockIdx.x * 256 + threadIdx.x; i < n2; i += (int64_t)gridDim.x * 256) {
    const vec_d2 wi = ld2(w, i);
    const vec_d2 a = ld2(w, i);
    acc[0] = __builtin_fma(a.y, wi.y, __builtin_fma(a.x, wi.x, acc[0]));
  }
  if (last) {
    const double wi = w[n - 1];
    acc[0] = __builtin_fma(w[n - 1], wi, acc[0]);
  }
  block_store_partials<1>(acc, partial + s * pstride);
}

template <int NV>
__global__ __launch_bounds__(256) void multi_axpy_norm_block_kernel(const double* __restrict__ Vb, int64_t vs, int64_t stride,
                                                                     double* __restrict__ hb, int64_t hstride,
                                                                     double* __restrict__ Wb, int64_t ldw,
                                                                     double* __restrict__ partial, int64_t n,
                                                                     const double* __restrict__ hpart, int64_t pstride,
                                                                     int hblocks) {
  const int s = blockIdx.y;
  const double* V = Vb + s * vs;
  double* h = hb + s * hstride;
  double* w = Wb + s * ldw;
  double hv[NV];
  block_reduce_partials<NV>(hpart + s * pstride, hblocks, hv);
  if (blockIdx.x == 0 && threadIdx.x == 0) {
#pragma unroll
    for (int v = 0; v < NV; ++v) h[v] = hv[v];
  }
  double acc[1] = {0.0};
  const int64_t n2 = n >> 1;
#pragma unroll 2
  for (int64_t i = (int64_t)blockIdx.x * 256 + threadIdx.x; i < n2; i += (int64_t)gridDim.x * 256) {
    vec_d2 wi = ld2(w, i);
#pragma unroll
    for (int v = 0; v < NV; ++v) {
      const vec_d2 a = ld2(V + v * stride, i);
      wi.x = __builtin_fma(-hv[v], a.x, wi.x);
      wi.y = __builtin_fma(-hv[v], a.y, wi.y);
    }
    st2(w, i, wi);
    acc[0] = __builtin_fma(wi.y, wi.y, __builtin_fma(wi.x, wi.x, acc[0]));
  }
  if ((n & 1) && blockIdx.x == gridDim.x - 1 && threadIdx.x == 255) {
    double wi = w[n - 1];
#pragma unroll
    for (int v = 0; v < NV; ++v) wi = __builtin_fma(-hv[v], V[v * stride + n - 1], wi);
    w[n - 1] = wi;
    acc[0] = __builtin_fma(wi, wi, acc[0]);
  }
  block_store_partials<1>(acc, partial + s * pstride);
}

__global__ __launch_bounds__(256) void fgmres_finish_fused_block_kernel(const double* __restrict__ normpart, int64_t pstride,
                                                                        int nblocks, double* __restrict__ hsb, int64_t hstride,
                                                                        int k, int K) {
  double s2[1];
  block_reduce_partials<1>(normpart + blockIdx.y * pstride, nblocks, s2);
  if (threadIdx.x != 0) return;
  HsLayout L(K);
  double* hs = hsb + blockIdx.y * hstride;
  hessenberg_column(hs, K, k - 1, hs + L.hd, sqrt(s2[0]));
  double* y = hs + L.y;
  const double* grs = hs + L.grs;
  for (int i = k - 1; i >= 0; --i) {
    double s = grs[i];
    for (int q = i + 1; q < k; ++q) s -= hs[L.H(q) + i] * y[q];
    const double d = hs[L.H(i) + i];
    y[i] = d != 0.0 ? s / d : 0.0;
  }
}

template <int NV, bool VEC>
__global__ __launch_bounds__(256) void multi_axpy_add_block_kernel(const double* __restrict__ Zb, int64_t zs, int64_t stride,
                                                                    const double* __restrict__ yb, int64_t hstride,
                                                                    double* __restrict__ X, int64_t ldx, BlockCols cols,
                                                                    int64_t n) {
  const int s = blockIdx.y;
  const double* Z = Zb + s * zs;
  const double* y = yb + s * hstride;
  double* x = X + (int64_t)block_col(cols, s) * ldx;
  double yv[NV];
#pragma unroll
  for (int v = 0; v < NV; ++v) yv[v] = y[v];
  if (VEC) {
    const int64_t n2 = n >> 1;
#pragma unroll 2
    for (int64_t i = (int64_t)blockIdx.x * 256 + threadIdx.x; i < n2; i += (int64_t)gridDim.x * 256) {
      vec_d2 xi = ld2(x, i);
#pragma unroll
      for (int v = 0; v < NV; ++v) {
        const vec_d2 a = ld2(Z + v * stride, i);
        xi.x = __builtin_fma(yv[v], a.x, xi.x);
        xi.y = __builtin_fma(yv[v], a.y, xi.y);
      }
      st2(x, i, xi);
    }
    if ((n & 1) && blockIdx.x == 0 && threadIdx.x == 0) {
      double xi = x[n - 1];
#pragma unroll
      for (int v = 0; v < NV; ++v) xi = __builtin_fma(yv[v], Z[v * stride + n - 1], xi);
      x[n - 1] = xi;
    }
  } else {
    for (int64_t i = (int64_t)blockIdx.x * 256 + threadIdx.x; i < n; i += (int64_t)gridDim.x * 256) {
      double xi = x[i];
#pragma unroll
      for (int v = 0; v < NV; ++v) xi = __builtin_fma(yv[v], Z[v * stride + i], xi);
      x[i] = xi;
    }
  }
}

namespace {
struct Slots {
  int nc, K;
  int64_t n, ldv, vs, zs, hstride, pstride;
  double *V, *Z, *w, *hs, *part1, *part2;
};
Slots slots_of(const alfi_level* L, int nc) {
  Slots S;
  const KrylovWs& ws = L->blk_ws;
  S.nc = nc;
  S.K = ws.K;
  S.n = L->n;
  S.ldv = ws.ldv;
  S.vs = ws.vs();
  S.zs = ws.zs();
  S.hstride = ws.hstride();
  S.pstride = L->blk_part.per;
  S.V = ws.V;
  S.Z = ws.Z;
  S.w = ws.w;
  S.hs = ws.hs;
  S.part1 = L->blk_part.p;
  S.part2 = L->blk_part.p + block_partial_set(RED_BLOCKS, RED_MAXV);
  return S;
}
int check_slots(alfi_level* L, int nc) {
  if (nc < 2 || nc > BLOCK_NV || nc > L->blk_ws.slots || nc > L->blk_part.slots || L->blk_ws.K != L->ws.K)
    return alfi_set_error(L->ctx, ALFI_E_STATE, "block fused iteration on %d columns without its workspace", nc);
  return 0;
}
dim3 fused_ew_grid(int64_t n, int nc) {
  int64_t b = (n + 255) / 256;
  if (b > 8192) b = 8192;
  if (b < 1) b = 1;
  return dim3((unsigned)b, (unsigned)nc);
}
}

int launch_patch_apply_il_block(alfi_level* L, int nc, const double* X, int64_t ldx, double* stage) {
  alfi_ctx* ctx = L->ctx;
// ... 61 lines not shown

namespace {
template <int BS, int LPR, int NVEC>
int launch_spmv_dot_block_nc(alfi_ctx* ctx, const DevBSR& A, const Slots& S, int j, int nvec, int* nblocks) {
  const int64_t rows_per_block = 256 / LPR;
  int64_t g = (A.nbrows + rows_per_block - 1) / rows_per_block;
  if (g > RED_BLOCKS) g = RED_BLOCKS;
  if (g < 1) g = 1;
  *nblocks = (int)g;
#define ALFI_SDB(NCC)                                                                                                          \
  hipLaunchKernelGGL((bsr_spmv_dot_block_kernel<BS, LPR, NVEC, NCC>), dim3((unsigned)g), dim3(256), 0, ctx->stream, A.nbrows,   \
                     A.rowptr, A.colidx, A.vals, S.Z + (int64_t)j * S.ldv, S.zs, S.w, S.ldv, S.V, S.vs, S.ldv, nvec, S.part1,    \
                     S.pstride)
  switch (S.nc) {
    case 2: ALFI_SDB(2); break;
    case 3: ALFI_SDB(3); break;
    default: ALFI_SDB(4); break;
  }
#undef ALFI_SDB
  ALFI_HIP_CHECK(ctx, hipGetLastError());
  return 0;
}
template <int BS, int LPR>
int launch_spmv_dot_block_lpr(alfi_ctx* ctx, const DevBSR& A, const Slots& S, int j, int nvec, int* nblocks) {
  switch (block_dot_vectors(nvec)) {
    case 4: return launch_spmv_dot_block_nc<BS, LPR, 4>(ctx, A, S, j, nvec, nblocks);
    case 8: return launch_spmv_dot_block_nc<BS, LPR, 8>(ctx, A, S, j, nvec, nblocks);
    case 16: return launch_spmv_dot_block_nc<BS, LPR, 16>(ctx, A, S, j, nvec, nblocks);
  }
  return alfi_set_error(ctx, ALFI_E_STATE, "block fused SpMV with %d dot vectors", nvec);
}
}

int launch_bsr_spmv_dot_block(alfi_level* L, int nc, int j, int* nblocks) {
  alfi_ctx* ctx = L->ctx;
  ALFI_CHECK(check_slots(L, nc));
  const Slots S = slots_of(L, nc);
  const DevBSR& A = L->A_own;
  const int nvec = j + 1;
  if (!A.flat || nvec < 1 || nvec > 16) return alfi_set_error(ctx, ALFI_E_STATE, "fused SpMV needs the flat layout and <= 16 vectors");
  const double avg = A.nbrows > 0 ? (double)A.nnzb / (double)A.nbrows : 0.0;
  if (A.bs == 2) {
    if (avg <= 12) return launch_spmv_dot_block_lpr<2, 4>(ctx, A, S, j, nvec, nblocks);
    if (avg <= 40) return launch_spmv_dot_block_lpr<2, 8>(ctx, A, S, j, nvec, nblocks);
    return launch_spmv_dot_block_lpr<2, 32>(ctx, A, S, j, nvec, nblocks);
  }
  if (A.bs == 3) {
    if (avg <= 24) return launch_spmv_dot_block_lpr<3, 8>(ctx, A, S, j, nvec, nblocks);
    if (avg <= 48) return launch_spmv_dot_block_lpr<3, 16>(ctx, A, S, j, nvec, nblocks);
    return launch_spmv_dot_block_lpr<3, 32>(ctx, A, S, j, nvec, nblocks);
  }
  return alfi_set_error(ctx, ALFI_E_ARG, "unsupported block size %d", A.bs);
}

int launch_multi_axpy_norm_block(alfi_level* L, int nc, int j, int hblocks) {
  alfi_ctx* ctx = L->ctx;
  ALFI_CHECK(check_slots(L, nc));
  const Slots S = slots_of(L, nc);
  const int nvec = j + 1;
  if (nvec < 1 || nvec > 16 || hblocks < 1) return alfi_set_error(ctx, ALFI_E_STATE, "block fused projection with %d vectors", nvec);
  if (!vec2_ok(S.V, S.w, S.ldv)) return alfi_set_error(ctx, ALFI_E_STATE, "block workspace off a 16-byte boundary");
  const dim3 grid((unsigned)red_blocks_for(S.n), (unsigned)nc), block(256);
  const int64_t hd = HsLayout(S.K).hd;
#define ALFI_CASE(N)                                                                                                           \
  case N:                                                                                                                      \
    hipLaunchKernelGGL((multi_axpy_norm_block_kernel<N>), grid, block, 0, ctx->stream, S.V, S.vs, S.ldv, S.hs + hd, S.hstride,  \
                       S.w, S.ldv, S.part2, S.n, S.part1, S.pstride, hblocks);                                                  \
    break;
  switch (nvec) {
    ALFI_CASE(1) ALFI_CASE(2) ALFI_CASE(3) ALFI_CASE(4) ALFI_CASE(5) ALFI_CASE(6) ALFI_CASE(7) ALFI_CASE(8) ALFI_CASE(9)
    ALFI_CASE(10) ALFI_CASE(11) ALFI_CASE(12) ALFI_CASE(13) ALFI_CASE(14) ALFI_CASE(15) ALFI_CASE(16)
  }
#undef ALFI_CASE
  ALFI_HIP_CHECK(ctx, hipGetLastError());
  return 0;
}

int launch_fgmres_finish_update_block(alfi_level* L, const BlockCols& cols, int k, int nblocks, double* X, int64_t ldx) {
  alfi_ctx* ctx = L->ctx;
  ALFI_CHECK(check_slots(L, cols.n));
  const Slots S = slots_of(L, cols.n);
  if (k < 1 || k > 16) return alfi_set_error(ctx, ALFI_E_STATE, "block fused update with %d vectors", k);
  hipLaunchKernelGGL(fgmres_finish_fused_block_kernel, dim3(1, (unsigned)S.nc), dim3(256), 0, ctx->stream, S.part2, S.pstride,
                     nblocks, S.hs, S.hstride, k, S.K);
  ALFI_HIP_CHECK(ctx, hipGetLastError());
  if (S.n <= 0) return 0;
  const bool vec = vec2_ok(S.Z, X + (int64_t)cols.c[0] * ldx, S.ldv) && (ldx & 1) == 0;
  const dim3 grid = fused_ew_grid(vec ? (S.n + 1) / 2 : S.n, S.nc), block(256);
  const int64_t yo = HsLayout(S.K).y;
#define ALFI_CASE(N)                                                                                                           \
  case N:                                                                                                                      \
    if (vec)                                                                                                                   \
      hipLaunchKernelGGL((multi_axpy_add_block_kernel<N, true>), grid, block, 0, ctx->stream, S.Z, S.zs, S.ldv, S.hs + yo,      \
                         S.hstride, X, ldx, cols, S.n);                                                                        \
    else                                                                                                                       \
      hipLaunchKernelGGL((multi_axpy_add_block_kernel<N, false>), grid, block, 0, ctx->stream, S.Z, S.zs, S.ldv, S.hs + yo,     \
                         S.hstride, X, ldx, cols, S.n);                                                                        \
    break;
  switch (k) {
    ALFI_CASE(1) ALFI_CASE(2) ALFI_CASE(3) ALFI_CASE(4) ALFI_CASE(5) ALFI_CASE(6) ALFI_CASE(7) ALFI_CASE(8) ALFI_CASE(9)
    ALFI_CASE(10) ALFI_CASE(11) ALFI_CASE(12) ALFI_CASE(13) ALFI_CASE(14) ALFI_CASE(15) ALFI_CASE(16)
  }
#undef ALFI_CASE
  ALFI_HIP_CHECK(ctx, hipGetLastError());
  return 0;
}
```

### alfi_amd/csrc/kernels_vec.hip

```cpp
#include <cstdlib>
#include <cstring>
#include "common.h"
#include "hs_layout.h"
#include "reduce.h"

template <int BS, int LPR>
__global__ __launch_bounds__(256) void bsr_spmv_kernel(int64_t nbrows, const int32_t* __restrict__ rowptr,
                                                        const int32_t* __restrict__ colidx,
                                                        const double* __restrict__ vals, const double* __restrict__ x,
                                                        double* __restrict__ y, const double* __restrict__ b,
                                                        double alpha, int mode) {
  const int64_t row = ((int64_t)blockIdx.x * 256 + threadIdx.x) / LPR;
  const int l = threadIdx.x % LPR;
  double acc[BS];
#pragma unroll
  for (int r = 0; r < BS; ++r) acc[r] = 0.0;
  if (row < nbrows) {
    const int32_t lo = rowptr[row], hi = rowptr[row + 1];
    for (int32_t k = lo + l; k < hi; k += LPR) {
      const int64_t col = colidx[k];
      const double* v = vals + (int64_t)k * BS * BS;
      double xv[BS];
#pragma unroll
      for (int c = 0; c < BS; ++c) xv[c] = x[col * BS + c];
// ... 759 lines not shown
    }
  }
  for (int64_t i = (int64_t)blockIdx.x * 256 + threadIdx.x; i < n; i += (int64_t)gridDim.x * 256) {
    double s = 0.0;
    const int32_t q0 = dof_ptr[i], q1 = dof_ptr[i + 1];
    for (int32_t q = q0; q < q1; ++q) s += stage[dof_pos[q]];
    if (pou && q1 - q0 > 1) s /= (double)(q1 - q0);
    const double wi = w[i];
    z[i] = f * (bc_mask[i] ? wi : s);
    v[i] = f * wi;
  }
}

template <int BS, int LPR, int NV>
__global__ __launch_bounds__(256) void bsr_spmv_dot_kernel(int64_t nbrows, const int32_t* __restrict__ rowptr,
                                                            const int32_t* __restrict__ colflag,
                                                            const double* __restrict__ vals,
                                                            const double* __restrict__ z, double* __restrict__ w,
                                                            const double* __restrict__ V, int64_t stride,
                                                            double* __restrict__ partial) {
  constexpr int BB = BS * BS;
  const int l = threadIdx.x % LPR;
  double acc[NV];
#pragma unroll
  for (int v = 0; v < NV; ++v) acc[v] = 0.0;
  for (int64_t row = ((int64_t)blockIdx.x * 256 + threadIdx.x) / LPR; row < nbrows;
       row += (int64_t)gridDim.x * (256 / LPR)) {
    double s[BS];
#pragma unroll
    for (int r = 0; r < BS; ++r) s[r] = 0.0;
    const int32_t lo = rowptr[row], hi = rowptr[row + 1];
    for (int32_t k = lo + l; k < hi; k += LPR) {
      const int64_t col = colflag[k] & 0x7fffffff;
      const double* vb = vals + ((int64_t)k >> 6) * (64 * BB);
      const int kl = k & 63;
      double a[BB], xv[BS];
#pragma unroll
      for (int q = 0; q < BB / 2; ++q) {
        const spmv_d2 t = *(reinterpret_cast<const spmv_d2*>(vb + q * 128) + kl);
        a[2 * q] = t.x;
        a[2 * q + 1] = t.y;
      }
      if (BB & 1) a[BB - 1] = vb[(BB / 2) * 128 + kl];
#pragma unroll
      for (int c = 0; c < BS; ++c) xv[c] = z[col * BS + c];
#pragma unroll
      for (int r = 0; r < BS; ++r)
#pragma unroll
        for (int c = 0; c < BS; ++c) s[r] = __builtin_fma(a[r * BS + c], xv[c], s[r]);
    }
#pragma unroll
    for (int o = LPR / 2; o > 0; o >>= 1)
#pragma unroll
      for (int r = 0; r < BS; ++r) s[r] += __shfl_xor(s[r], o);
    if (l == 0) {
#pragma unroll
      for (int r = 0; r < BS; ++r) {
        const int64_t i = row * BS + r;
        w[i] = s[r];
#pragma unroll
        for (int v = 0; v < NV; ++v) acc[v] = __builtin_fma(V[v * stride + i], s[r], acc[v]);
      }
    }
  }
  block_store_partials<NV>(acc, partial);
}

__global__ __launch_bounds__(256) void hessenberg_update_kernel(const double* __restrict__ partial, int nblocks,
                                                                 const double* __restrict__ h,
                                                                 double* __restrict__ hs, int j, int K,
                                                                 const double* __restrict__ ww) {
  __shared__ double red[256];
  double s = 0.0;
  for (int b = threadIdx.x; b < nblocks; b += 256) s += partial[(int64_t)b * RED_MAXV];
  red[threadIdx.x] = s;
  __syncthreads();
  for (int o = 128; o > 0; o >>= 1) {
    if (threadIdx.x < o) red[threadIdx.x] += red[threadIdx.x + o];
    __syncthreads();
  }
  if (threadIdx.x == 0) hessenberg_column(hs, K, j, h, sqrt(ww ? pythagoras_norm2(ww, h, j) : red[0]));
}

__global__ void fgmres_finish_kernel(double* __restrict__ hs, int k, int K) {
  if (threadIdx.x != 0 || blockIdx.x != 0) return;
  fgmres_back_substitution(hs, k, K);
}

#define ALFI_NV_SWITCH(NVAL, MACRO) \
  switch (NVAL) {                   \
    MACRO(1) MACRO(2) MACRO(3) MACRO(4) MACRO(5) MACRO(6) MACRO(7) MACRO(8) MACRO(9) MACRO(10) MACRO(11) MACRO(12) \
    MACRO(13) MACRO(14) MACRO(15) MACRO(16)                                                                         \
  }

int red_blocks_for(int64_t n) {
  const int64_t g = (n + 4095) / 4096;
  return (int)(g < 1 ? 1 : (g > RED_BLOCKS ? RED_BLOCKS : g));
}

int launch_multi_dot(alfi_ctx* ctx, const double* V, int64_t stride, int nv, const double* w, double* out, int64_t n) {
  const int G = red_blocks_for(n);
  for (int v0 = 0; v0 < nv; v0 += 16) {
    const int cnt = nv - v0 < 16 ? nv - v0 : 16;
    const bool vec = vec2_ok(V + (int64_t)v0 * stride, w, stride);
#define ALFI_CASE(N)                                                                                              \
  case N:                                                                                                         \
    if (vec)                                                                                                      \
      hipLaunchKernelGGL((multi_dot_kernel<N, true>), dim3(G), dim3(256), 0, ctx->stream, V + (int64_t)v0 * stride, \
                         stride, w, ctx->red_partial, n);                                                         \
    else                                                                                                          \
      hipLaunchKernelGGL((multi_dot_kernel<N, false>), dim3(G), dim3(256), 0, ctx->stream, V + (int64_t)v0 * stride, \
                         stride, w, ctx->red_partial, n);                                                         \
    break;
    ALFI_NV_SWITCH(cnt, ALFI_CASE)
#undef ALFI_CASE
    ALFI_HIP_CHECK(ctx, hipGetLastError());
    if (out) {
      hipLaunchKernelGGL(reduce_partials_kernel, dim3(1), dim3(256), 0, ctx->stream, ctx->red_partial, G, cnt, out + v0);
      ALFI_HIP_CHECK(ctx, hipGetLastError());
    }
  }
  return 0;
}

int launch_multi_axpy_norm(alfi_ctx* ctx, const double* V, int64_t stride, int nv, double* h, double* w, int64_t n,
                           double* norm_partial, int hblocks) {
  const int G = red_blocks_for(n);
  for (int v0 = 0; v0 < nv; v0 += 16) {
    const int cnt = nv - v0 < 16 ? nv - v0 : 16;
    const bool vec = vec2_ok(V + (int64_t)v0 * stride, w, stride);
#define ALFI_CASE(N)                                                                                               \
  case N:                                                                                                          \
    if (vec)                                                                                                       \
      hipLaunchKernelGGL((multi_axpy_norm_kernel<N, true>), dim3(G), dim3(256), 0, ctx->stream,                    \
                         V + (int64_t)v0 * stride, stride, h + v0, w, norm_partial, n, ctx->red_partial, hblocks); \
    else                                                                                                           \
      hipLaunchKernelGGL((multi_axpy_norm_kernel<N, false>), dim3(G), dim3(256), 0, ctx->stream,                   \
                         V + (int64_t)v0 * stride, stride, h + v0, w, norm_partial, n, ctx->red_partial, hblocks); \
    break;
    ALFI_NV_SWITCH(cnt, ALFI_CASE)
#undef ALFI_CASE
    ALFI_HIP_CHECK(ctx, hipGetLastError());
  }
  return 0;
}

__global__ __launch_bounds__(256) void hessenberg_scale_kernel(const double* __restrict__ partial, int nblocks,
                                                                const double* __restrict__ h, double* __restrict__ hs,
                                                                int j, int K, double* __restrict__ vnext,
                                                                const double* __restrict__ w, int64_t n,
                                                                const double* __restrict__ ww) {
  __shared__ double red[256];
  double s = 0.0;
  for (int b = threadIdx.x; b < nblocks; b += 256) s += partial[(int64_t)b * RED_MAXV];
  red[threadIdx.x] = s;
  __syncthreads();
  for (int o = 128; o > 0; o >>= 1) {
    if (threadIdx.x < o) red[threadIdx.x] += red[threadIdx.x + o];
    __syncthreads();
  }
  const double tt = sqrt(ww ? pythagoras_norm2(ww, h, j) : red[0]);
  if (blockIdx.x == 0 && threadIdx.x == 0) hessenberg_column(hs, K, j, h, tt);
  const double f = tt != 0.0 ? 1.0 / tt : 0.0;
  if (((reinterpret_cast<uintptr_t>(vnext) | reinterpret_cast<uintptr_t>(w)) & 15) == 0) {
    const int64_t n2 = n >> 1;
    for (int64_t i = (int64_t)blockIdx.x * 256 + threadIdx.x; i < n2; i += (int64_t)gridDim.x * 256) {
      vec_d2 t = ld2(w, i);
      t.x *= f;
      t.y *= f;
// ... 58 lines not shown
    const int64_t u = e / bs;
    const int c = (int)(e - u * bs);
    const int64_t at = (int64_t)rev_nodes[u] * bs + c;
    double s = v[at];
    for (int32_t q = rev_ptr[u]; q < rev_ptr[u + 1]; ++q) s += buf[(int64_t)rev_pos[q] * bs + c];
    v[at] = s;
  }
}
__global__ void halo_sum_kernel(double* __restrict__ v, const double* __restrict__ buf, const int32_t* __restrict__ nodes,
                                const int32_t* __restrict__ ptr, const int32_t* __restrict__ src, int64_t total, int bs) {
  for (int64_t e = (int64_t)blockIdx.x * blockDim.x + threadIdx.x; e < total; e += (int64_t)gridDim.x * blockDim.x) {
    const int64_t u = e / bs;
    const int c = (int)(e - u * bs);
    const int64_t at = (int64_t)nodes[u] * bs + c;
    const double own = v[at];
    double s = 0.0;
    for (int32_t q = ptr[u]; q < ptr[u + 1]; ++q) s += src[q] < 0 ? own : buf[(int64_t)src[q] * bs + c];
    v[at] = s;
  }
}
int launch_halo_sum(alfi_ctx* ctx, double* v, const double* buf, const int32_t* nodes, const int32_t* ptr, const int32_t* src,
                    int64_t nshared, int bs) {
  ALFI_LAUNCH_EW(halo_sum_kernel, nshared * bs, v, buf, nodes, ptr, src, nshared * bs, bs);
  return 0;
}
int launch_halo_pack(alfi_ctx* ctx, double* buf, const double* v, const int32_t* nodes, int64_t nnodes, int bs) {
  ALFI_LAUNCH_EW(halo_pack_kernel, nnodes * bs, buf, v, nodes, nnodes * bs, bs);
  return 0;
}
int launch_halo_add(alfi_ctx* ctx, double* v, const double* buf, const int32_t* rev_nodes, const int32_t* rev_ptr,
                    const int32_t* rev_pos, int64_t nuniq, int bs) {
  ALFI_LAUNCH_EW(halo_add_kernel, nuniq * bs, v, buf, rev_nodes, rev_ptr, rev_pos, nuniq * bs, bs);
  return 0;
}

int launch_patch_sum_scale(alfi_level* L, const double* w, double* z, double* v, const double* normpart, int nblocks,
                           const double* h, double* hs, int j, int K) {
  alfi_ctx* ctx = L->ctx;
  const int64_t n = L->n;
  hipLaunchKernelGGL(patch_sum_scale_kernel, ew_grid(n), dim3(256), 0, ctx->stream, n, L->dof_ptr, L->dof_pos, L->stage,
                     L->bc_mask, w, z, v, normpart, nblocks, h, hs, j, K, L->pou ? 1 : 0);
  ALFI_HIP_CHECK(ctx, hipGetLastError());
  return 0;
}

template <int BS, int LPR>
static int launch_spmv_dot_lpr(alfi_ctx* ctx, const DevBSR& A, const double* z, double* w, const double* V, int64_t stride,
                               int nv, double* partial, int* nblocks) {
  const int64_t rows_per_block = 256 / LPR;
  int64_t g = (A.nbrows + rows_per_block - 1) / rows_per_block;
  if (g > RED_BLOCKS) g = RED_BLOCKS;
  if (g < 1) g = 1;
  *nblocks = (int)g;
#define ALFI_CASE(N)                                                                                                 \
  case N:                                                                                                            \
    hipLaunchKernelGGL((bsr_spmv_dot_kernel<BS, LPR, N>), dim3((unsigned)g), dim3(256), 0, ctx->stream, A.nbrows,      \
                       A.rowptr, A.colidx, A.vals, z, w, V, stride, partial);                                        \
    break;
  ALFI_NV_SWITCH(nv, ALFI_CASE)
#undef ALFI_CASE
  ALFI_HIP_CHECK(ctx, hipGetLastError());
  return 0;
}

int launch_bsr_spmv_dot(alfi_ctx* ctx, const DevBSR& A, const double* z, double* w, const double* V, int64_t stride, int nv,
                        double* partial, int* nblocks) {
  if (!A.flat || nv < 1 || nv > 16) return alfi_set_error(ctx, ALFI_E_STATE, "fused SpMV needs the flat layout and <= 16 vectors");
  const double avg = A.nbrows > 0 ? (double)A.nnzb / (double)A.nbrows : 0.0;
  if (A.bs == 2) {
    if (avg <= 12) return launch_spmv_dot_lpr<2, 4>(ctx, A, z, w, V, stride, nv, partial, nblocks);
    if (avg <= 40) return launch_spmv_dot_lpr<2, 8>(ctx, A, z, w, V, stride, nv, partial, nblocks);
    return launch_spmv_dot_lpr<2, 32>(ctx, A, z, w, V, stride, nv, partial, nblocks);
  }
  if (A.bs == 3) {
    if (avg <= 24) return launch_spmv_dot_lpr<3, 8>(ctx, A, z, w, V, stride, nv, partial, nblocks);
    if (avg <= 48) return launch_spmv_dot_lpr<3, 16>(ctx, A, z, w, V, stride, nv, partial, nblocks);
    return launch_spmv_dot_lpr<3, 32>(ctx, A, z, w, V, stride, nv, partial, nblocks);
  }
  return alfi_set_error(ctx, ALFI_E_ARG, "unsupported block size %d", A.bs);
}

__global__ __launch_bounds__(256) void fgmres_finish_fused_kernel(const double* __restrict__ normpart, int nblocks,
                                                                  const double* __restrict__ h, double* __restrict__ hs,
                                                                  int k, int K) {
  double s2[1];
  block_reduce_partials<1>(normpart, nblocks, s2);
  if (threadIdx.x != 0) return;
  hessenberg_column(hs, K, k - 1, h, sqrt(s2[0]));
  HsLayout L(K);
  double* y = hs + L.y;
  const double* grs = hs + L.grs;
  for (int i = k - 1; i >= 0; --i) {
    double s = grs[i];
    for (int q = i + 1; q < k; ++q) s -= hs[L.H(q) + i] * y[q];
    const double d = hs[L.H(i) + i];
    y[i] = d != 0.0 ? s / d : 0.0;
  }
}
int launch_fgmres_finish_fused(alfi_ctx* ctx, const double* normpart, int nblocks, const double* h, double* hs, int k, int K) {
  hipLaunchKernelGGL(fgmres_finish_fused_kernel, dim3(1), dim3(256), 0, ctx->stream, normpart, nblocks, h, hs, k, K);
  ALFI_HIP_CHECK(ctx, hipGetLastError());
  return 0;
}

int launch_fgmres_finish(alfi_ctx* ctx, double* hs, int k, int K) {
  hipLaunchKernelGGL(fgmres_finish_kernel, dim3(1), dim3(64), 0, ctx->stream, hs, k, K);
  ALFI_HIP_CHECK(ctx, hipGetLastError());
  return 0;
}

int launch_update_solution(alfi_ctx* ctx, double* x, const double* Z, int64_t stride, int k, const double* y,
                           int64_t n) {
  for (int v0 = 0; v0 < k; v0 += 16) {
    const int cnt = k - v0 < 16 ? k - v0 : 16;
    const bool vec = vec2_ok(Z + (int64_t)v0 * stride, x, stride);
    const dim3 grid = ew_grid(vec ? (n + 1) / 2 : n);
#define ALFI_CASE(N)                                                                                                \
  case N:                                                                                                           \
    if (vec)                                                                                                        \
      hipLaunchKernelGGL((multi_axpy_add_kernel<N, true>), grid, dim3(256), 0, ctx->stream, Z + (int64_t)v0 * stride, \
                         stride, y + v0, x, n);                                                                     \
    else                                                                                                            \
      hipLaunchKernelGGL((multi_axpy_add_kernel<N, false>), grid, dim3(256), 0, ctx->stream, Z + (int64_t)v0 * stride, \
                         stride, y + v0, x, n);                                                                     \
    break;
    ALFI_NV_SWITCH(cnt, ALFI_CASE)
#undef ALFI_CASE
    ALFI_HIP_CHECK(ctx, hipGetLastError());
  }
  return 0;
}

__global__ void block_build_kernel(int64_t nblk, int m, int ld, int64_t stride, const double* __restrict__ K,
                                   const double* __restrict__ D, double nu, double gamma, double* __restrict__ S) {
  const int64_t total = nblk * m * ld;
  for (int64_t e = (int64_t)blockIdx.x * blockDim.x + threadIdx.x; e < total; e += (int64_t)gridDim.x * blockDim.x) {
    const int64_t blk = e / (m * ld);
    const int64_t in = e - blk * m * ld;
    const int r = (int)(in / ld), c = (int)(in % ld);
    S[blk * stride + in] = c < m ? nu * K[(blk * m + r) * m + c] + gamma * D[(blk * m + r) * m + c] : 0.0;
  }
}

__global__ void block_operator_t_kernel(int64_t nblk, int m, int ld, const double* __restrict__ K, const double* __restrict__ D,
                                        double nu, double gamma, double* __restrict__ At) {
  const int64_t total = nblk * m * ld;
  for (int64_t e = (int64_t)blockIdx.x * blockDim.x + threadIdx.x; e < total; e += (int64_t)gridDim.x * blockDim.x) {
    const int64_t blk = e / ((int64_t)m * ld);
    const int64_t in = e - blk * (int64_t)m * ld;
    const int j = (int)(in / ld), i = (int)(in % ld);
    At[e] = i < m ? nu * K[(blk * m + i) * m + j] + gamma * D[(blk * m + i) * m + j] : 0.0;
  }
}

int launch_block_build_invert(alfi_transfer* tr) {
  alfi_ctx* ctx = tr->ctx;
  const int64_t total = tr->nblk * tr->m * tr->ld;
  if (tr->patch_mode && tr->AIIt)
    ALFI_LAUNCH_EW(block_operator_t_kernel, total, tr->nblk, tr->m, tr->ld, tr->KII, tr->DII, tr->nu, tr->gamma, tr->AIIt);
  if (tr->m > SMALL_PATCH_MAX) return launch_big_factor_transfer(tr);
  const int64_t stride = tr->patch_mode ? tr->bstride : (int64_t)tr->m * tr->ld;
  ALFI_LAUNCH_EW(block_build_kernel, total, tr->nblk, tr->m, tr->ld, stride, tr->KII, tr->DII, tr->nu, tr->gamma,
                 tr->binv);
  if (tr->patch_mode)
    return launch_patch_invert_arrays(ctx, tr->nblk, tr->m, tr->pm_ptr, tr->pm_inv_ptr, tr->binv, tr->status);
  return launch_invert_small_any(ctx, tr->m, tr->nblk, nullptr, nullptr, tr->m, (int64_t)tr->m * tr->ld, tr->binv,
                                 tr->status);
}

template <int G>
__global__ __launch_bounds__(256) void block_gemv_kernel(int64_t nblk, int m, int ld, const double* __restrict__ binv,
                                                          const int32_t* __restrict__ blk_dofs,
                                                          const double* __restrict__ in, double* __restrict__ out,
                                                          int gather) {
  const int64_t blk = ((int64_t)blockIdx.x * 256 + threadIdx.x) / G;
  const int i = threadIdx.x % G;
  const bool valid = blk < nblk && i < m;
  double xi = 0.0;
  if (valid) xi = gather ? in[blk_dofs[blk * m + i]] : in[blk * m + i];
  const double* T = binv + (valid ? blk * (int64_t)m * ld : 0);
  double acc = 0.0;
  for (int j = 0; j < m; ++j) {
    const double xj = __shfl(xi, j, G);
    if (valid) acc = __builtin_fma(T[(int64_t)j * ld + i], xj, acc);
  }
  if (valid) out[blk * m + i] = acc;
}

__global__ void compact_rows_kernel(double* __restrict__ out, const double* __restrict__ in, int64_t total, int m,
                                    int ld) {
  for (int64_t e = (int64_t)blockIdx.x * blockDim.x + threadIdx.x; e < total; e += (int64_t)gridDim.x * blockDim.x)
    out[e] = in[(e / m) * ld + e % m];
}

constexpr int BR_U = 8;
__global__ __launch_bounds__(256) void block_residual_kernel(int m, int ld, const double* __restrict__ At,
                                                              const int32_t* __restrict__ idx, const double* __restrict__ in,
                                                              const double* __restrict__ t, double* __restrict__ r) {
  __shared__ double ts[PATCH_MAX];
  const int64_t blk = blockIdx.x;
  for (int i = threadIdx.x; i < m; i += 256) ts[i] = t[blk * m + i];
  __syncthreads();
  const double* A = At + blk * (int64_t)m * ld;
  for (int p = threadIdx.x; 2 * p < m; p += 256) {
    const double* col = A + 2 * p;
    double a0 = 0.0, a1 = 0.0;
    int j = 0;
    for (; j + BR_U <= m; j += BR_U) {
      vec_d2 a[BR_U];
#pragma unroll
      for (int u = 0; u < BR_U; ++u) a[u] = __builtin_nontemporal_load(reinterpret_cast<const vec_d2*>(col + (int64_t)(j + u) * ld));
#pragma unroll
      for (int u = 0; u < BR_U; ++u) {
        a0 = __builtin_fma(a[u].x, ts[j + u], a0);
        a1 = __builtin_fma(a[u].y, ts[j + u], a1);
// ... 288 lines not shown
```

### alfi_amd/csrc/krylov_ws.h

```cpp
#pragma once
#include <cstdint>
#include "block_cols.h"
#include "hs_layout.h"

inline int64_t krylov_ldv(int64_t n) { return (n + 1) & ~(int64_t)1; }

struct KrylovWs {
  double *V = nullptr, *Z = nullptr, *w = nullptr, *hs = nullptr;
  int K = 0, slots = 0;
  int64_t ldv = 0;
  int64_t vs() const { return (int64_t)(K + 1) * ldv; }
  int64_t zs() const { return (int64_t)K * ldv; }
  int64_t hstride() const { return HsLayout(K).total; }
  double* v(int s, int j) const { return V + s * vs() + j * ldv; }
  double* z(int s, int j) const { return Z + s * zs() + j * ldv; }
  double* wv(int s) const { return w + s * ldv; }
  double* h(int s) const { return hs + s * hstride(); }
};
struct KrylovWsDoubles {
  int64_t V, Z, w, hs;
};
inline KrylovWsDoubles krylov_ws_doubles(int slots, int K, int64_t ldv) {
  KrylovWs t;
  t.K = K;
  t.ldv = ldv;
  return {slots * t.vs(), slots * t.zs(), slots * ldv, slots * t.hstride()};
}

struct SlotBuf {
  double* p = nullptr;
  int slots = 0;
  int64_t per = 0;
  double* slot(int s) const { return p + s * per; }
};
inline int slot_buf_needed(const SlotBuf& b, int ncol) { return block_slots_needed(b.slots, ncol); }
```

### alfi_amd/hip.py

```python
import ctypes
import numpy as np

from . import _lib, env
from ._lib import BsrHost, CsrHost, vp


class AlfiHipError(RuntimeError):
    code = None


E_ARG, E_STATE = -2, -3


def _ptr(a):
    return None if a is None else a.ctypes.data_as(vp)


class Context(object):
    def __init__(self, device=0, stream=None):
        self.lib = _lib.load()
        h = vp()
        rc = self.lib.alfi_ctx_create(int(device), vp(stream) if stream else None, ctypes.byref(h))
        if rc != 0:
            raise AlfiHipError("alfi_ctx_create failed (%d): %s -- alfi_amd needs an MI355X; there is no CPU fallback"
# ... 441 lines not shown
        b = ctypes.c_int64()
        self.ctx.check(self.ctx.lib.alfi_patches_factor_bytes(self.h, ctypes.byref(b)))
        return b.value

    def set_partition_of_unity(self, on=True):
        self.ctx.check(self.ctx.lib.alfi_patches_set_partition_of_unity(self.h, 1 if on else 0))

    def set_multiplicative(self, iterset, symmetrise):
        it = np.ascontiguousarray(iterset if iterset is not None else [], dtype=np.int64)
        self.ctx.check(self.ctx.lib.alfi_patches_set_multiplicative(self.h, len(it), _ptr(it), 1 if symmetrise else 0))
        self._record_storage()
        nw = ctypes.c_int64()
        self.ctx.check(self.ctx.lib.alfi_patches_multiplicative_levels(self.h, ctypes.byref(nw)))
        return nw.value

    def factor(self):
        self.ctx.check(self.ctx.lib.alfi_patches_factor(self.h))
        self._record_storage()

    def factor_with_fallback(self):
        try:
            self.factor()
            self._warn_if_flagged()
            return False
        except AlfiHipError as e:
            if "condensed" not in str(e):
                raise
        self.set_patch_groups(None)
        self.factor()
        self._warn_if_flagged()
        return True

    def _warn_if_flagged(self):
        worst, flagged, repaired, after = self.patch_check()
        if flagged > repaired:
            import warnings
            warnings.warn("alfi_patches_factor: %d of %d flagged patch factors stay above the probe tolerance after the "
                          "pivoted repair (worst residual %.2e): the patch operators are ill-conditioned"
                          % (flagged - repaired, flagged, after))

    def patch_check(self):
        w, wa = ctypes.c_double(), ctypes.c_double()
        f, r = ctypes.c_int64(), ctypes.c_int64()
        self.ctx.check(self.ctx.lib.alfi_patches_check(self.h, ctypes.byref(w), ctypes.byref(f), ctypes.byref(r),
                                                       ctypes.byref(wa)))
        return w.value, f.value, r.value, wa.value

    def patch_stats(self):
        a, b, c = ctypes.c_int64(), ctypes.c_int64(), ctypes.c_int64()
        self.ctx.check(self.ctx.lib.alfi_patches_stats(self.h, ctypes.byref(a), ctypes.byref(b), ctypes.byref(c)))
        return a.value, b.value, c.value

    def patch_inverse(self, p, n):
        out = np.empty((n, n))
        self.ctx.check(self.ctx.lib.alfi_patch_get_inverse(self.h, int(p), _ptr(out)))
        return out

    def patch_apply(self, x, y):
        self.ctx.check(self.ctx.lib.alfi_patch_apply(self.h, x.ptr, y.ptr))

    def patch_apply_split(self, split, x, y):
        self.ctx.check(self.ctx.lib.alfi_patch_apply_split(self.h, int(split), x.ptr, y.ptr))

    def spmv(self, x, y):
        self.ctx.check(self.ctx.lib.alfi_spmv(self.h, x.ptr, y.ptr))

    def zero_bc(self, v):
        self.ctx.check(self.ctx.lib.alfi_level_zero_bc(self.h, v.ptr))

    def halo_forward(self, v):
        self.ctx.check(self.ctx.lib.alfi_level_halo_forward(self.h, v.ptr))

    def halo_sum(self, v):
        self.ctx.check(self.ctx.lib.alfi_level_halo_sum(self.h, v.ptr))

    def halo_reverse_add(self, v):
        self.ctx.check(self.ctx.lib.alfi_level_halo_reverse_add(self.h, v.ptr))

    def residual(self, b, x, r):
        self.ctx.check(self.ctx.lib.alfi_residual(self.h, b.ptr, x.ptr, r.ptr))

    def smooth(self, k, b, x, nonzero_guess=True):
        self.ctx.check(self.ctx.lib.alfi_smooth_fgmres(self.h, int(k), b.ptr, x.ptr, 1 if nonzero_guess else 0))

    def patch_apply_block(self, X, Y, cols=None):
        ncol, cp, nx, keep = _block_args(self.n, cols, X, Y)
        self.ctx.check(self.ctx.lib.alfi_patch_apply_block(self.h, ncol, cp, nx, X.ptr, X.ld, Y.ptr, Y.ld))

    def spmv_block(self, X, Y, cols=None):
        ncol, cp, nx, keep = _block_args(self.n, cols, X, Y)
        self.ctx.check(self.ctx.lib.alfi_spmv_block(self.h, ncol, cp, nx, X.ptr, X.ld, Y.ptr, Y.ld))

    def residual_block(self, B, X, R, cols=None):
        ncol, cp, nx, keep = _block_args(self.n, cols, B, X, R)
        self.ctx.check(self.ctx.lib.alfi_residual_block(self.h, ncol, cp, nx, B.ptr, B.ld, X.ptr, X.ld, R.ptr, R.ld))

    def smooth_block(self, k, B, X, nonzero_guess=True, cols=None):
        ncol, cp, nx, keep = _block_args(self.n, cols, B, X)
        self.ctx.check(self.ctx.lib.alfi_smooth_fgmres_block(self.h, int(k), ncol, cp, nx, B.ptr, B.ld, X.ptr, X.ld,
                                                             1 if nonzero_guess else 0))

    def patch_apply_block_batched(self):
        b = ctypes.c_int()
        self.ctx.check(self.ctx.lib.alfi_patch_apply_block_info(self.h, ctypes.byref(b)))
        return bool(b.value)

    def patch_apply_block_width(self):
        w = ctypes.c_int()
        self.ctx.check(self.ctx.lib.alfi_patch_apply_block_width(self.h, ctypes.byref(w)))
        return int(w.value)

    def smooth_block_lockstep(self, k):
        b = ctypes.c_int()
        self.ctx.check(self.ctx.lib.alfi_smooth_fgmres_block_info(self.h, int(k), ctypes.byref(b)))
        return bool(b.value)

    def smooth_block_mode(self, k):
        m = ctypes.c_int()
        self.ctx.check(self.ctx.lib.alfi_smooth_fgmres_block_mode(self.h, int(k), ctypes.byref(m)))
        return int(m.value)

    def spmv_block_batched(self):
        b = ctypes.c_int()
        self.ctx.check(self.ctx.lib.alfi_spmv_block_info(self.h, ctypes.byref(b)))
        return bool(b.value)

    def spmv_block_width(self):
        w = ctypes.c_int()
        self.ctx.check(self.ctx.lib.alfi_spmv_block_width(self.h, ctypes.byref(w)))
        return int(w.value)

    def set_jacobi(self, on=True):
        self.ctx.check(self.ctx.lib.alfi_level_set_jacobi(self.h, 1 if on else 0))

    def smooth_chebyshev(self, k, emin, emax, b, x, nonzero_guess=True):
        self.ctx.check(self.ctx.lib.alfi_smooth_chebyshev(self.h, int(k), float(emin), float(emax), b.ptr, x.ptr,
                                                          1 if nonzero_guess else 0))

    def arnoldi(self, m, v0):
        H = np.zeros((int(m) + 1, int(m)))
        done = ctypes.c_int()
        self.ctx.check(self.ctx.lib.alfi_level_arnoldi(self.h, int(m), v0.ptr, _ptr(H), ctypes.byref(done)))
        return H, done.value

    def set_coarse_inverse(self, inv):
        if isinstance(inv, (int, np.integer)):
            self.ctx.check(self.ctx.lib.alfi_coarse_set_inverse(self.h, vp(int(inv)), 1))
        else:
            inv = np.ascontiguousarray(inv, dtype=np.float64)
            assert inv.shape == (self.n, self.n)
            self.ctx.check(self.ctx.lib.alfi_coarse_set_inverse(self.h, _ptr(inv), 0))

    def coarse_factor(self):
        self.ctx.check(self.ctx.lib.alfi_coarse_factor(self.h))
        return self.coarse_residual()

    def coarse_factor_sparse(self, node_coords=None, leaf_nodes=0):
        if node_coords is None:
            self.ctx.check(self.ctx.lib.alfi_coarse_factor_sparse(self.h, None, 0, int(leaf_nodes)))
        else:
            xy = np.ascontiguousarray(node_coords, dtype=np.float64)
            assert xy.ndim == 2 and xy.shape[0] * self.bs == self.n, (xy.shape, self.n, self.bs)
            self.ctx.check(self.ctx.lib.alfi_coarse_factor_sparse(self.h, _ptr(xy), int(xy.shape[1]), int(leaf_nodes)))
        return self.coarse_residual()

    def coarse_factor_auto(self, node_coords=None, mode=None, geometric=False):
# ... 143 lines not shown
                dl.set_patches(L.patch_ptr, L.patch_dofs)
                if getattr(L, "patch_groups", None) is not None and env.condense():
                    dl.set_patch_groups(L.patch_groups)
                elif not env.condense():
                    dl.set_patch_groups(None)
                ask_patch_storage(dl, patch_factor_dtype)
                dl.factor_with_fallback()
                note_patch_level(L, dl)
            elif coarse_inv is not None:
                dl.set_coarse_inverse(coarse_inv)
            else:
                dl.coarse_factor_auto(getattr(getattr(L, "V", None), "node_coords", None), coarse)
            dlevels.append(dl)
        self._from_device_levels(ctx, dlevels, transfers, k, robust_restriction)
        if verbose:
            print("[alfi_amd] device hierarchy ready in %.1fs" % (time.time() - t0), flush=True)

    def _from_device_levels(self, ctx, dlevels, transfers, k, robust_restriction):
        self.ctx = ctx
        self.levels, self.transfers = list(dlevels), []
        for i, T in enumerate(transfers):
            dt = Transfer(ctx, self.levels[i], self.levels[i + 1], T)
            dt.update(T.nu, T.gamma)
            self.transfers.append(dt)
        lv = (vp * len(self.levels))(*[l.h for l in self.levels])
        tr = (vp * max(1, len(self.transfers)))(*[t.h for t in self.transfers])
        h = vp()
        ctx.check(ctx.lib.alfi_mg_create(ctx.h, len(self.levels), lv, tr, int(k), 1 if robust_restriction else 0,
                                         ctypes.byref(h)))
        self.h = h
        self.k = k
        ctx.sync()

    def variant(self, robust_restriction):
        other = Multigrid.__new__(Multigrid)
        other.ctx, other.levels, other.transfers, other.k = self.ctx, self.levels, self.transfers, self.k
        lv = (vp * len(self.levels))(*[l.h for l in self.levels])
        tr = (vp * max(1, len(self.transfers)))(*[t.h for t in self.transfers])
        h = vp()
        self.ctx.check(self.ctx.lib.alfi_mg_create(self.ctx.h, len(self.levels), lv, tr, int(self.k),
                                                   1 if robust_restriction else 0, ctypes.byref(h)))
        other.h = h
        return other

    def close_handle(self):
        if self.h:
            self.ctx.lib.alfi_mg_destroy(self.h)
            self.h = None

    def vcycle(self, b, x):
        self.ctx.check(self.ctx.lib.alfi_mg_vcycle(self.h, b.ptr, x.ptr))

    def fcycle(self, b, x):
        self.ctx.check(self.ctx.lib.alfi_mg_fcycle(self.h, b.ptr, x.ptr))

    def vcycle_block(self, B, X, cols=None):
        ncol, cp, nx, keep = _block_args(self.levels[-1].n, cols, B, X)
        self.ctx.check(self.ctx.lib.alfi_mg_vcycle_block(self.h, ncol, cp, nx, B.ptr, B.ld, X.ptr, X.ld))

    def fcycle_block(self, B, X, cols=None):
        ncol, cp, nx, keep = _block_args(self.levels[-1].n, cols, B, X)
        self.ctx.check(self.ctx.lib.alfi_mg_fcycle_block(self.h, ncol, cp, nx, B.ptr, B.ld, X.ptr, X.ld))

    SMOOTHERS = {"fgmres": 0, "chebyshev": 1}
    CYCLES = {"v": 1, "w": 2}

    def set_smoother(self, kind, bounds=None):
        if kind not in self.SMOOTHERS:
            raise ValueError("smoother %r (fgmres or chebyshev)" % (kind,))
        if kind == "fgmres":
            self.ctx.check(self.ctx.lib.alfi_mg_set_smoother(self.h, 0, None, None))
            return
        b = np.ascontiguousarray(bounds, dtype=np.float64).reshape(-1, 2)
        if b.shape[0] != len(self.levels) - 1:
            raise ValueError("need one (emin, emax) pair per level above the coarsest: %d, got %d" % (len(self.levels) - 1, b.shape[0]))
        emin, emax = np.ascontiguousarray(b[:, 0]), np.ascontiguousarray(b[:, 1])
        self.ctx.check(self.ctx.lib.alfi_mg_set_smoother(self.h, 1, _ptr(emin), _ptr(emax)))

    def set_cycle_type(self, kind):
        if kind not in self.CYCLES:
            raise ValueError("cycle type %r (v or w)" % (kind,))
        self.ctx.check(self.ctx.lib.alfi_mg_set_cycles(self.h, self.CYCLES[kind]))

    def chebyshev_bounds(self, steps=10, esteig=(0.0, 0.1, 0.0, 1.1), seed=0):
        a, b, c, d = (float(t) for t in esteig)
        out = []
        for L in self.levels[1:]:
            v = np.random.default_rng(seed).standard_normal(L.n)
            dv = self.ctx.vec(v)
            L.zero_bc(dv)
            H, m = L.arnoldi(steps, dv)
            if m < 1:
                raise AlfiHipError("chebyshev_bounds: the Arnoldi iteration broke down at once (zero operator?)")
            ritz = np.linalg.eigvals(H[:m, :m]).real
            lmin, lmax = float(ritz.min()), float(ritz.max())
            out.append((a * lmin + b * lmax, c * lmin + d * lmax))
        return out

    def cg(self, b, x, rtol=1e-8, atol=0.0, max_it=200, full=False):
        its, rn = ctypes.c_int(), ctypes.c_double()
        self.ctx.check(self.ctx.lib.alfi_mg_cg(self.h, b.ptr, x.ptr, float(rtol), float(atol), int(max_it), 1 if full else 0,
                                               ctypes.byref(its), ctypes.byref(rn)))
        return its.value, rn.value

    def close(self):
        if self.h:
            self.ctx.lib.alfi_mg_destroy(self.h)
            self.h = None
        for t in self.transfers:
            t.close()
        for l in self.levels:
            l.close()


class RawVec(object):

    def __init__(self, ptr, n, ctx=None, parent=None):
        self.ptr, self.n, self.ctx, self._parent = vp(int(ptr)), int(n), ctx, parent

    def set(self, a):
        a = np.ascontiguousarray(a, dtype=np.float64)
        assert a.shape == (self.n,)
        self.ctx.check(self.ctx.lib.alfi_memcpy_h2d(self.ctx.h, self.ptr, _ptr(a), self.n * 8))

    def get(self):
        out = np.empty(self.n, dtype=np.float64)
        self.ctx.check(self.ctx.lib.alfi_memcpy_d2h(self.ctx.h, _ptr(out), self.ptr, self.n * 8))
        return out


def view(v, off, n):
    assert 0 <= off and off + n <= v.n
    return RawVec(v.ptr.value + 8 * int(off), n, ctx=getattr(v, "ctx", None), parent=v)


class Csr(object):

    def __init__(self, ctx, M):
        import scipy.sparse as sp
        M = sp.csr_matrix(M)
        M.sort_indices()
        rp = np.ascontiguousarray(M.indptr, dtype=np.int32)
        ci = np.ascontiguousarray(M.indices, dtype=np.int32)
        va = np.ascontiguousarray(M.data, dtype=np.float64)
        st = CsrHost(M.shape[0], M.shape[1], _ptr(rp), _ptr(ci), _ptr(va))
        self.ctx, self.shape = ctx, M.shape
        h = vp()
        ctx.check(ctx.lib.alfi_csr_create(ctx.h, ctypes.byref(st), ctypes.byref(h)))
        self.h = h

    def mult(self, x, y, b=None, alpha=1.0, mode=0):
        self.ctx.check(self.ctx.lib.alfi_csr_mult(self.h, x.ptr, y.ptr, b.ptr if b is not None else None, float(alpha),
                                                  int(mode)))

    def close(self):
        if self.h:
            self.ctx.lib.alfi_csr_destroy(self.h)
            self.h = None


class Saddle(object):

    def __init__(self, mg, B, mass_diag, nu, gamma, remove_constant_nullspace=True, mass_inv=None, n_u=None):
        import scipy.sparse as sp
        self.mg, self.ctx = mg, mg.ctx
        B = sp.csr_matrix(B)
# ... 100 lines not shown
```

### include/alfi_hip.h

```cpp
#ifndef ALFI_HIP_H
#define ALFI_HIP_H
#include <stdint.h>

#ifdef __cplusplus
extern "C" {
#endif

#define ALFI_OK 0
#define ALFI_E_HIP -1
#define ALFI_E_ARG -2
#define ALFI_E_STATE -3
#define ALFI_E_SINGULAR -4
#define ALFI_E_COMM -5

typedef struct alfi_ctx alfi_ctx;
typedef struct alfi_level alfi_level;
typedef struct alfi_transfer alfi_transfer;
typedef struct alfi_mg alfi_mg;

int alfi_ctx_create(int device, void* stream, alfi_ctx** out);
int alfi_ctx_destroy(alfi_ctx* ctx);
int alfi_ctx_sync(alfi_ctx* ctx);
const char* alfi_last_error(alfi_ctx* ctx);
int alfi_malloc(alfi_ctx* ctx, int64_t bytes, void** dptr);
// ... 28 lines not shown
int alfi_ctx_comm_destroy(alfi_ctx* ctx);
enum { ALFI_COMM_ALLREDUCE = 0, ALFI_COMM_HALO_FWD = 1, ALFI_COMM_HALO_REV = 2, ALFI_COMM_HALO_FWD_BEGIN = 3,
       ALFI_COMM_HALO_FWD_END = 4, ALFI_COMM_HALO_REV_BEGIN = 5, ALFI_COMM_HALO_REV_END = 6,
       ALFI_COMM_HALO_SUM = 7  };
typedef int (*alfi_comm_fn)(void* user, int op, int level_id, int64_t offset, int64_t count);
int alfi_ctx_set_comm(alfi_ctx* ctx, alfi_comm_fn fn, void* user, double* dred, int64_t dred_len);

int alfi_level_create(alfi_ctx* ctx, int64_t nbrows, int bs, const int32_t* browptr_host, const int32_t* bcolidx_host,
                      const double* bvals_host, const int32_t* bc_dofs_host, int64_t nbc, alfi_level** out);
int alfi_level_destroy(alfi_level* lvl);
int alfi_level_set_partition(alfi_level* lvl, int64_t nb_owned, int distributed, int64_t nsend,
                             const int32_t* send_nodes_host, double* d_sendbuf, double* d_recvbuf, int64_t nb_ghost);
int alfi_level_set_neighbours(alfi_level* lvl, int nnbr, const int32_t* ranks_host, const int64_t* send_nodes_host,
                              const int64_t* recv_nodes_host);
int alfi_level_set_sum_exchange(alfi_level* lvl, int nnbr, const int32_t* ranks_host, const int64_t* counts_host,
                                const int32_t* send_nodes_host, int64_t nshared, const int32_t* sum_nodes_host,
                                const int32_t* sum_ptr_host, const int32_t* sum_src_host);
int alfi_level_set_overlap(alfi_level* lvl, int64_t nb_interior, int64_t npatch_interior);
int alfi_level_update_values(alfi_level* lvl, const double* bvals_host);
int alfi_level_set_assembly(alfi_level* lvl, int64_t ncell, int nloc, const int32_t* cell_nodes, const double* grad,
                            const double* vol, const double* S, const double* bI, const double* T1, int full_div,
                            const int64_t* cptr, const int32_t* ccell, const uint16_t* cba);
int alfi_level_assemble(alfi_level* lvl, double nu, double gamma, double adv, const double* d_state, int apply_bc);
int alfi_ctx_set_assembly_scratch(alfi_ctx* ctx, int64_t max_bytes);
int alfi_level_set_assembly_bc(alfi_level* lvl, const int32_t* bc_dofs_host, int64_t nbc);
int alfi_level_assembly_state_size(alfi_level* lvl, int64_t* n);
int alfi_level_assemble_mult(alfi_level* lvl, double nu, double gamma, double adv, const double* d_state, const double* dx,
                             double* dy);
int alfi_level_set_supg(alfi_level* lvl, int nq, const double* wq, const double* phi, const double* dphi, const double* d2phi,
                        const double* hcell);
int alfi_level_assemble_supg(alfi_level* lvl, double nu, double gamma, double adv, const double* d_state, double weight,
                             double magic, int apply_bc);
int alfi_level_supg(alfi_level* lvl, double nu, double weight, double magic, const double* d_state, int add_to_operator,
                    double* d_F);
int alfi_level_set_supg_load(alfi_level* lvl, const double* fq);
int alfi_level_assemble_gls(alfi_level* lvl, double nu, double gamma, double adv, const double* d_state, const double* d_wind,
                            double weight, double magic, int apply_bc);
int alfi_level_gls(alfi_level* lvl, double nu, double weight, double magic, const double* d_state, const double* d_wind,
                   int add_to_operator, double* d_F);
int alfi_level_apply_bc(alfi_level* lvl);
int alfi_level_set_facet_blocks(alfi_level* lvl, int on);
int alfi_level_set_burman(alfi_level* lvl, int64_t nfacet, int nu, int nqs, int nqn, int ncfg, const int32_t* funion,
                          const int32_t* cfg, const double* J, const double* area, const double* coef, const double* ws,
                          const double* wn, const double* phin, const int64_t* bptr, const int32_t* bfac, const uint16_t* bab,
                          const int64_t* nptr, const int32_t* nfac, const uint16_t* na);
int alfi_level_burman(alfi_level* lvl, double weight, const double* d_state, int add_to_operator, double* d_F);
int alfi_level_assemble_burman(alfi_level* lvl, double nu, double gamma, double adv, const double* d_state, double weight,
                               int apply_bc);
int alfi_patches_set_facet_correction(alfi_level* lvl, int64_t nfacet, int64_t nrow, const int64_t* ptr, const int32_t* col,
                                      const int32_t* fac, const double* s);
int alfi_level_set_facet_beta(alfi_level* lvl, const double* beta_host, double scale);
int alfi_level_transpose(alfi_level* lvl);
int alfi_level_get_values(alfi_level* lvl, double* bvals_host);
int alfi_level_size(alfi_level* lvl, int64_t* n);
int alfi_level_id(alfi_level* lvl, int* id);
int alfi_spmv(alfi_level* lvl, const double* dx, double* dy);
int alfi_residual(alfi_level* lvl, const double* db, const double* dx, double* dr);

int alfi_patches_set(alfi_level* lvl, int64_t npatch, const int64_t* patch_ptr_host, const int32_t* patch_dofs_host);
int alfi_patches_factor(alfi_level* lvl);
int alfi_patches_set_groups(alfi_level* lvl, const int32_t* group_host);
int alfi_patches_factor_bytes(alfi_level* lvl, int64_t* bytes);
int alfi_patches_find_groups(alfi_level* lvl, int32_t* group_out_host);
int alfi_ctx_set_condense_min_bytes(alfi_ctx* ctx, int64_t min_bytes);
int alfi_patches_condensed(alfi_level* lvl, int* mode);
#define ALFI_STORAGE_F64 0
#define ALFI_STORAGE_F32 1
int alfi_patches_set_storage(alfi_level* lvl, int dtype);
int alfi_patches_storage(alfi_level* lvl, int* dtype);
int alfi_patches_set_macro_storage(alfi_level* lvl, int dtype);
int alfi_ctx_set_f32_work_bytes(alfi_ctx* ctx, int64_t bytes);
int alfi_ctx_f32_work_bytes(alfi_ctx* ctx, int64_t* bytes);
int alfi_patches_set_canonical_order(alfi_level* lvl, const int32_t* rank_host);
int alfi_patch_apply_split(alfi_level* lvl, int64_t split, const double* x_dev, double* y_dev);
int alfi_patches_check(alfi_level* lvl, double* worst_residual, int64_t* flagged, int64_t* repaired, double* worst_after);
int alfi_patch_apply(alfi_level* lvl, const double* dx, double* dy);
int alfi_patches_set_partition_of_unity(alfi_level* lvl, int on);
int alfi_patches_set_multiplicative(alfi_level* lvl, int64_t nit, const int64_t* iterset_host, int symmetrise);
int alfi_patches_multiplicative_levels(alfi_level* lvl, int64_t* nwave);
int alfi_patches_stats(alfi_level* lvl, int64_t* npatch, int64_t* sum_n, int64_t* sum_n2);
int alfi_patch_get_inverse(alfi_level* lvl, int64_t p, double* out_host);

int alfi_smooth_fgmres(alfi_level* lvl, int k, const double* db, double* dx, int nonzero_guess);

int alfi_level_set_jacobi(alfi_level* lvl, int on);
int alfi_smooth_chebyshev(alfi_level* lvl, int k, double emin, double emax, const double* db, double* dx, int nonzero_guess);
int alfi_level_arnoldi(alfi_level* lvl, int m, const double* dv0, double* H_host, int* m_done);

int alfi_coarse_factor(alfi_level* lvl);
int alfi_coarse_factor_sparse(alfi_level* lvl, const double* node_coords, int dim, int leaf_nodes);
int alfi_coarse_factor_bytes(alfi_level* lvl, int64_t* bytes);
int alfi_coarse_residual(alfi_level* lvl, double* worst);
int alfi_coarse_set_inverse(alfi_level* lvl, const double* inv, int inv_is_device);
int alfi_coarse_solve(alfi_level* lvl, const double* db, double* dx);

typedef struct {
  int64_t nbrows, nbcols;
  const int32_t* rowptr;
  const int32_t* colidx;
  const double* vals;
} alfi_bsr_host;
int alfi_transfer_create(alfi_ctx* ctx, alfi_level* coarse, alfi_level* fine, const alfi_bsr_host* P,
                         const alfi_bsr_host* PT, const alfi_bsr_host* PT_plain, const alfi_bsr_host* D_I,
                         const alfi_bsr_host* D_IT, int64_t nblk, int m, const int32_t* blk_dofs_host,
                         const double* K_II_host, const double* D_II_host, alfi_transfer** out);
int alfi_transfer_destroy(alfi_transfer* tr);
int alfi_transfer_update(alfi_transfer* tr, double nu, double gamma);
int alfi_transfer_get_block_inverse(alfi_transfer* tr, int64_t blk, double* out_host);
int alfi_prolong(alfi_transfer* tr, const double* dxc, double* dxf);
int alfi_restrict(alfi_transfer* tr, const double* drf, double* drc, int robust);

int alfi_transfer_set_injection(alfi_transfer* tr, const int32_t* fine_node_host);
int alfi_inject(alfi_transfer* tr, const double* dxf, double* dxc);

int alfi_mg_create(alfi_ctx* ctx, int nlevels, alfi_level** levels, alfi_transfer** transfers, int k,
                   int robust_restriction, alfi_mg** out);
int alfi_mg_destroy(alfi_mg* mg);
int alfi_mg_vcycle(alfi_mg* mg, const double* db, double* dx);
int alfi_mg_fcycle(alfi_mg* mg, const double* db, double* dx);
#define ALFI_SMOOTHER_FGMRES 0
#define ALFI_SMOOTHER_CHEBYSHEV 1
int alfi_mg_set_smoother(alfi_mg* mg, int type, const double* emin_host, const double* emax_host);
int alfi_mg_set_cycles(alfi_mg* mg, int cycles);
int alfi_mg_cg(alfi_mg* mg, const double* db, double* dx, double rtol, double atol, int max_it, int full, int* iterations,
               double* residual_norm);
int alfi_ctx_set_graph(alfi_ctx* ctx, int on);

typedef struct alfi_saddle alfi_saddle;
typedef struct {
  int64_t nrows, ncols;
  const int32_t* rowptr;
  const int32_t* colidx;
  const double* vals;
} alfi_csr_host;
int alfi_saddle_create(alfi_mg* mg, const alfi_csr_host* B, const alfi_csr_host* BT, const double* mass_diag_host,
                       double nu, double gamma, int remove_constant_nullspace, alfi_saddle** out);
int alfi_saddle_destroy(alfi_saddle* s);
int alfi_saddle_set_mass_inverse(alfi_saddle* s, const alfi_csr_host* Minv);
int alfi_saddle_update(alfi_saddle* s, double nu, double gamma);
int alfi_saddle_solve(alfi_saddle* s, const double* db, double* dx, double rtol, double atol, int max_it, int restart,
                      int* iterations, double* residual_norm);
int alfi_level_halo_forward(alfi_level* lvl, double* dv);
int alfi_level_halo_reverse_add(alfi_level* lvl, double* dv);
int alfi_level_halo_sum(alfi_level* lvl, double* dv);
typedef struct alfi_csr alfi_csr;
int alfi_csr_create(alfi_ctx* ctx, const alfi_csr_host* M, alfi_csr** out);
int alfi_transfer_set_injection_matrix(alfi_transfer* tr, const alfi_csr_host* J);
int alfi_csr_destroy(alfi_csr* m);
int alfi_csr_mult(alfi_csr* m, const double* dx, double* dy, const double* db, double alpha, int mode);
int alfi_vec_axpy(alfi_ctx* ctx, double* dy, const double* dx, double a, int64_t n);
int alfi_vec_copy(alfi_ctx* ctx, double* dy, const double* dx, int64_t n);
int alfi_vec_gather(alfi_ctx* ctx, double* dst, const double* dsrc, const int32_t* d_idx, int64_t nidx, int bs);
int alfi_vec_gather_csr(alfi_ctx* ctx, double* dst, const double* dsrc, const int32_t* d_rowptr, const int32_t* d_colidx,
                        const double* d_weights, int64_t nrows, int bs);
int alfi_level_zero_bc(alfi_level* lvl, double* dv);
int alfi_saddle_dot(alfi_saddle* s, const double* dx, const double* dy, double* out_host);
int alfi_transfer_stats(int64_t* h2d_bytes, int64_t* d2h_bytes, int reset);
int alfi_saddle_mult(alfi_saddle* s, const double* dx, double* dy);
int alfi_saddle_precond(alfi_saddle* s, const double* dx, double* dy);
#define ALFI_VELOCITY_MG 0
#define ALFI_VELOCITY_DIRECT 1
int alfi_saddle_set_velocity_solver(alfi_saddle* s, int kind);
int alfi_saddle_factor_velocity(alfi_saddle* s, const double* node_coords, int dim, int leaf_nodes, int64_t max_bytes);
int alfi_saddle_velocity_solve(alfi_saddle* s, const double* db, double* dx);
int alfi_saddle_velocity_info(alfi_saddle* s, int64_t* bytes, double* probe_residual);

int alfi_ctx_set_block_kernels(alfi_ctx* ctx, int on);
int alfi_patch_apply_block_info(alfi_level* lvl, int* batched);
int alfi_spmv_block_info(alfi_level* lvl, int* batched);
int alfi_patch_apply_block_width(alfi_level* lvl, int* width);
int alfi_spmv_block_width(alfi_level* lvl, int* width);
int alfi_ctx_set_block_lds_bytes(alfi_ctx* ctx, int64_t bytes);
int alfi_patch_apply_block(alfi_level* lvl, int ncol, const int* cols, int nx, const double* X, int64_t ldx, double* Y, int64_t ldy);
int alfi_spmv_block(alfi_level* lvl, int ncol, const int* cols, int nx, const double* X, int64_t ldx, double* Y, int64_t ldy);
int alfi_residual_block(alfi_level* lvl, int ncol, const int* cols, int nx, const double* B, int64_t ldb, const double* X,
                        int64_t ldx, double* R, int64_t ldr);
int alfi_smooth_fgmres_block_info(alfi_level* lvl, int k, int* lockstep);
int alfi_smooth_fgmres_block_mode(alfi_level* lvl, int k, int* mode);
int alfi_ctx_set_block_fused(alfi_ctx* ctx, int on);
int alfi_smooth_fgmres_block(alfi_level* lvl, int k, int ncol, const int* cols, int nx, const double* B, int64_t ldb, double* X,
                             int64_t ldx, int nonzero_guess);
int alfi_mg_vcycle_block(alfi_mg* mg, int ncol, const int* cols, int nx, const double* B, int64_t ldb, double* X, int64_t ldx);
int alfi_mg_fcycle_block(alfi_mg* mg, int ncol, const int* cols, int nx, const double* B, int64_t ldb, double* X, int64_t ldx);
int alfi_saddle_mult_block(alfi_saddle* s, int ncol, const int* cols, int nx, const double* X, int64_t ldx, double* Y, int64_t ldy);
int alfi_saddle_precond_block(alfi_saddle* s, int ncol, const int* cols, int nx, const double* X, int64_t ldx, double* Y, int64_t ldy);
int alfi_saddle_solve_block(alfi_saddle* s, int ncol, const int* cols, int nx, const double* B, int64_t ldb, double* X, int64_t ldx,
                            double rtol, double atol, int max_it, int restart, int* iterations, double* residual_norms);

#ifdef __cplusplus
}
#endif
#endif
```

Before: 8.963.

## Recover post-smoothing residual from FGMRES Krylov basis instead of extra SpMV

After the FGMRES pre-smoother, the V-cycle now forms the residual as a linear combination of the Arnoldi basis vectors. The coefficients come from the Givens-rotated least-squares data, computed in the finish kernels. This replaces a full operator application (block SpMV) before restriction with a streaming combination of k+1 vectors. The new path is on by default for serial FGMRES levels. It adds extra reads of the basis vectors and depends on the Arnoldi relation holding accurately, so rounding drift could make the residual differ slightly.

```diff
diff --git a/alfi_amd/_lib.py b/alfi_amd/_lib.py
--- a/alfi_amd/_lib.py
+++ b/alfi_amd/_lib.py
@@ -112,6 +112,7 @@
                                           ctypes.POINTER(ctypes.c_int64)]),
     "alfi_patch_get_inverse": (ctypes.c_int, [vp, ctypes.c_int64, vp]),
     "alfi_smooth_fgmres": (ctypes.c_int, [vp, ctypes.c_int, vp, vp, ctypes.c_int]),
+    "alfi_smooth_fgmres_residual": (ctypes.c_int, [vp, ctypes.c_int, vp]),
     "alfi_level_set_jacobi": (ctypes.c_int, [vp, ctypes.c_int]),
     "alfi_smooth_chebyshev": (ctypes.c_int, [vp, ctypes.c_int, ctypes.c_double, ctypes.c_double, vp, vp, ctypes.c_int]),
     "alfi_level_arnoldi": (ctypes.c_int, [vp, ctypes.c_int, vp, vp, ctypes.POINTER(ctypes.c_int)]),
@@ -139,6 +140,7 @@
     "alfi_mg_fcycle": (ctypes.c_int, [vp, vp, vp]),
     "alfi_mg_set_smoother": (ctypes.c_int, [vp, ctypes.c_int, vp, vp]),
     "alfi_mg_set_cycles": (ctypes.c_int, [vp, ctypes.c_int]),
+    "alfi_mg_set_krylov_residual": (ctypes.c_int, [vp, ctypes.c_int]),
     "alfi_mg_cg": (ctypes.c_int, [vp, vp, vp, ctypes.c_double, ctypes.c_double, ctypes.c_int, ctypes.c_int,
                                   ctypes.POINTER(ctypes.c_int), ctypes.POINTER(ctypes.c_double)]),
     "alfi_ctx_set_graph": (ctypes.c_int, [vp, ctypes.c_int]),
diff --git a/alfi_amd/csrc/api_block.hip b/alfi_amd/csrc/api_block.hip
--- a/alfi_amd/csrc/api_block.hip
+++ b/alfi_amd/csrc/api_block.hip
@@ -104,7 +104,9 @@
   ALFI_CHECK(dev_alloc(ctx, &ws->Z, d.Z));
   ALFI_CHECK(dev_alloc(ctx, &ws->w, d.w));
   ALFI_CHECK(dev_alloc(ctx, &ws->hs, d.hs));
+  ALFI_CHECK(dev_alloc(ctx, &ws->rc, d.rc));
   ALFI_HIP_CHECK(ctx, hipMemsetAsync(ws->hs, 0, sizeof(double) * (size_t)d.hs, ctx->stream));
+  ALFI_HIP_CHECK(ctx, hipMemsetAsync(ws->rc, 0, sizeof(double) * (size_t)d.rc, ctx->stream));
   ws->K = K;
   ws->slots = slots;
   return 0;
@@ -114,6 +116,7 @@
   dev_free(ws->Z);
   dev_free(ws->w);
   dev_free(ws->hs);
+  dev_free(ws->rc);
   *ws = KrylovWs();
 }
 
@@ -259,17 +262,26 @@
 }
 
 int block_smooth_fgmres(alfi_level* L, int k, const BlockCols& cols, const double* B, int64_t ldb, double* X, int64_t ldx,
-                        int nonzero_guess) {
+                        int nonzero_guess, double* R, int64_t ldr) {
   ALFI_CHECK(ensure_fgmres_workspace(L, k));
   L->ctx->cur_tag = L->id;
   const int mode = cols.n == 1 ? BLOCK_SMOOTH_LOOP : block_smoother_mode(L, k);
-  if (mode == BLOCK_SMOOTH_FUSED) return block_smooth_fgmres_fused(L, k, cols, B, ldb, X, ldx, nonzero_guess);
   if (mode == BLOCK_SMOOTH_LOOP) {
-    for (int i = 0; i < cols.n; ++i) ALFI_CHECK(alfi_smooth_fgmres(L, k, B + cols.c[i] * ldb, X + cols.c[i] * ldx, nonzero_guess));
+    for (int i = 0; i < cols.n; ++i) {
+      ALFI_CHECK(alfi_smooth_fgmres(L, k, B + cols.c[i] * ldb, X + cols.c[i] * ldx, nonzero_guess));
+      if (R) ALFI_CHECK(krylov_residual(L, L->ws, k, block_chunk(1, nullptr, 0), R + i * ldr, 0));
+    }
     return 0;
   }
-  ALFI_CHECK(ensure_block_smoother(L, cols.n));
-  return smooth_fgmres_general(L, L->blk_ws, k, cols, B, ldb, X, ldx, nonzero_guess);
+  L->blk_ws.res_k = 0;
+  if (mode == BLOCK_SMOOTH_FUSED) {
+    ALFI_CHECK(block_smooth_fgmres_fused(L, k, cols, B, ldb, X, ldx, nonzero_guess));
+  } else {
+    ALFI_CHECK(ensure_block_smoother(L, cols.n));
+    ALFI_CHECK(smooth_fgmres_general(L, L->blk_ws, k, cols, B, ldb, X, ldx, nonzero_guess));
+  }
+  L->blk_ws.res_k = k;
+  return R ? krylov_residual(L, L->blk_ws, k, block_chunk(cols.n, nullptr, 0), R, ldr) : 0;
 }
 
 int check_block_call(alfi_level* L, const char* what, int ncol, const int* cols, int nx, const BlockOperand* ops, int nops) {
@@ -329,6 +341,6 @@
   if (k < 1) return alfi_set_error(L->ctx, ALFI_E_ARG, "k must be >= 1");
   if (!level_pc_ready(L)) return alfi_set_error(L->ctx, ALFI_E_STATE, "alfi_smooth_fgmres_block before alfi_patches_factor");
   for (int q = 0; q < block_chunks(ncol); ++q)
-    ALFI_CHECK(block_smooth_fgmres(L, k, block_chunk(ncol, cols, q), B, ldb, X, ldx, nonzero_guess));
-  return 0;
-}
+    ALFI_CHECK(block_smooth_fgmres(L, k, block_chunk(ncol, cols, q), B, ldb, X, ldx, nonzero_guess, nullptr, 0));
+  return 0;
+}
diff --git a/alfi_amd/csrc/api_cycles.hip b/alfi_amd/csrc/api_cycles.hip
--- a/alfi_amd/csrc/api_cycles.hip
+++ b/alfi_amd/csrc/api_cycles.hip
@@ -443,6 +443,12 @@
   return 0;
 }
 
+int alfi_mg_set_krylov_residual(alfi_mg* mg, int on) {
+  if (!mg) return alfi_set_error(nullptr, ALFI_E_ARG, "NULL multigrid");
+  mg->krylov_residual = on != 0;
+  return 0;
+}
+
 int alfi_mg_set_cycles(alfi_mg* mg, int cycles) {
   if (!mg) return alfi_set_error(nullptr, ALFI_E_ARG, "NULL multigrid");
   if (cycles != 1 && cycles != 2) return alfi_set_error(mg->ctx, ALFI_E_ARG, "cycles %d (1 V, 2 W)", cycles);
@@ -459,15 +465,19 @@
 static MgWork own_work(const alfi_level* L) { return {L->mg_b, L->mg_x, L->mg_r, 0}; }
 static MgWork block_work(const alfi_level* L) { return {L->blk_mg_b.p, L->blk_mg_x.p, L->blk_mg_r.p, L->blk_mg_b.per}; }
 
+static inline bool mg_krylov_residual(const alfi_mg* mg, const alfi_level* L) {
+  return mg->smoother == ALFI_SMOOTHER_FGMRES && !level_is_partitioned(L) && mg->krylov_residual;
+}
+
 static int mg_smooth(alfi_mg* mg, int l, const BlockCols& cols, const double* B, int64_t ldb, double* X, int64_t ldx,
-                     int nonzero_guess) {
+                     int nonzero_guess, double* R = nullptr, int64_t ldr = 0) {
   alfi_level* L = mg->levels[l];
   if (mg->smoother == ALFI_SMOOTHER_CHEBYSHEV) {
     for (int i = 0; i < cols.n; ++i)
       ALFI_CHECK(alfi_smooth_chebyshev(L, mg->k, mg->emin[l], mg->emax[l], B + cols.c[i] * ldb, X + cols.c[i] * ldx, nonzero_guess));
     return 0;
   }
-  return block_smooth_fgmres(L, mg->k, cols, B, ldb, X, ldx, nonzero_guess);
+  return block_smooth_fgmres(L, mg->k, cols, B, ldb, X, ldx, nonzero_guess, R, ldr);
 }
 
 static int vcycle(alfi_mg* mg, MgWorkOf work, int l, const BlockCols& cols, const double* B, int64_t ldb, double* X, int64_t ldx,
@@ -482,8 +492,12 @@
   alfi_transfer* T = mg->transfers[l - 1];
   const BlockCols slots = block_chunk(nc, nullptr, 0);
   const MgWork wl = work(L), wc = work(mg->levels[l - 1]);
-  ALFI_CHECK(mg_smooth(mg, l, cols, B, ldb, X, ldx, x_zero ? 0 : 1));
-  ALFI_CHECK(block_spmv(L, cols, slots, X, ldx, wl.r, wl.ld, B, ldb, 1));
+  if (mg_krylov_residual(mg, L)) {
+    ALFI_CHECK(mg_smooth(mg, l, cols, B, ldb, X, ldx, x_zero ? 0 : 1, wl.r, wl.ld));
+  } else {
+    ALFI_CHECK(mg_smooth(mg, l, cols, B, ldb, X, ldx, x_zero ? 0 : 1));
+    ALFI_CHECK(block_spmv(L, cols, slots, X, ldx, wl.r, wl.ld, B, ldb, 1));
+  }
   for (int i = 0; i < nc; ++i) ALFI_CHECK(alfi_restrict(T, wl.r + i * wl.ld, wc.b + i * wc.ld, mg->robust));
   const int cycles = l == 1 ? 1 : mg->cycles;
   for (int c = 0; c < cycles; ++c) ALFI_CHECK(vcycle(mg, work, l - 1, slots, wc.b, wc.ld, wc.x, wc.ld, c == 0));
@@ -529,6 +543,7 @@
   sig->push_back((uint64_t)mg->robust);
   sig->push_back((uint64_t)mg->smoother);
   sig->push_back((uint64_t)mg->cycles);
+  sig->push_back((uint64_t)(mg->krylov_residual ? 1 : 0));
   if (mg->smoother == ALFI_SMOOTHER_CHEBYSHEV)
     for (size_t l = 1; l < mg->levels.size(); ++l) {
       pushd(mg->emin[l]);
diff --git a/alfi_amd/csrc/api_internal.h b/alfi_amd/csrc/api_internal.h
--- a/alfi_amd/csrc/api_internal.h
+++ b/alfi_amd/csrc/api_internal.h
@@ -68,6 +68,7 @@
 bool smoother_takes_fused_iteration(const alfi_level* L, int k, bool* flat_spmv = nullptr);
 int smooth_fgmres_general(alfi_level* L, const KrylovWs& ws, int k, const BlockCols& cols, const double* B, int64_t ldb, double* X,
                           int64_t ldx, int nonzero_guess);
+int krylov_residual(alfi_level* L, const KrylovWs& ws, int k, const BlockCols& slots, double* R, int64_t ldr);
 int krylov_ws_ensure(alfi_ctx* ctx, KrylovWs* ws, int slots, int K, int64_t n);
 void krylov_ws_release(KrylovWs* ws);
 int slot_buf_ensure(alfi_ctx* ctx, SlotBuf* buf, int ncol, int64_t per);
@@ -90,6 +91,6 @@
 int block_spmv(alfi_level* L, const BlockCols& ic, const BlockCols& oc, const double* X, int64_t ldx, double* Y, int64_t ldy,
                const double* B, int64_t ldb, int mode);
 int block_smooth_fgmres(alfi_level* L, int k, const BlockCols& cols, const double* B, int64_t ldb, double* X, int64_t ldx,
-                        int nonzero_guess);
+                        int nonzero_guess, double* R, int64_t ldr);
 int upload_csr(alfi_ctx* ctx, DevCSR* d, const alfi_csr_host* h);
 void free_csr(DevCSR* d);
diff --git a/alfi_amd/csrc/api_saddle.hip b/alfi_amd/csrc/api_saddle.hip
--- a/alfi_amd/csrc/api_saddle.hip
+++ b/alfi_amd/csrc/api_saddle.hip
@@ -541,7 +541,7 @@
         if (!cycle[s]) continue;
         its[s] = it;
         if (std::fabs(val[s]) <= tol[s]) {
-          ALFI_CHECK(launch_fgmres_finish(ctx, ws.h(s), j + 1, K));
+          ALFI_CHECK(launch_fgmres_finish(ctx, ws.h(s), j + 1, K, nullptr));
           ALFI_CHECK(launch_update_solution(ctx, xcol(s), ws.z(s, 0), ldv, j + 1, ws.h(s) + hl.y, n));
           cycle[s] = active[s] = false;
           --ncycle;
@@ -553,7 +553,7 @@
     }
     for (int s = 0; s < nc; ++s) {
       if (!cycle[s]) continue;
-      ALFI_CHECK(launch_fgmres_finish(ctx, ws.h(s), j, K));
+      ALFI_CHECK(launch_fgmres_finish(ctx, ws.h(s), j, K, nullptr));
       ALFI_CHECK(launch_update_solution(ctx, xcol(s), ws.z(s, 0), ldv, j, ws.h(s) + hl.y, n));
     }
     if (nactive == 0 || it >= max_it) break;
diff --git a/alfi_amd/csrc/api_smoother.hip b/alfi_amd/csrc/api_smoother.hip
--- a/alfi_amd/csrc/api_smoother.hip
+++ b/alfi_amd/csrc/api_smoother.hip
@@ -53,7 +53,7 @@
     normpart = ctx->red_partial2;
   }
   ProfScope prof(ctx, ALFI_EV_BLAS1);
-  ALFI_CHECK(launch_fgmres_finish_fused(ctx, normpart, G, hdots, hs, k, K));
+  ALFI_CHECK(launch_fgmres_finish_fused(ctx, normpart, G, hdots, hs, k, K, L->ws.c(0)));
   ALFI_CHECK(launch_update_solution(ctx, dx, Z, ldv, k, hs + hl.y, n));
   return 0;
 }
@@ -73,9 +73,38 @@
   if (!level_pc_ready(L)) return alfi_set_error(ctx, ALFI_E_STATE, "alfi_smooth_fgmres before alfi_patches_factor");
   ALFI_CHECK(ensure_fgmres_workspace(L, k));
   ctx->cur_tag = L->id;
+  L->ws.res_k = 0;
   bool flat_spmv = false;
-  if (smoother_takes_fused_iteration(L, k, &flat_spmv)) return smooth_fgmres_fused(L, k, db, dx, nonzero_guess, flat_spmv);
-  return smooth_fgmres_general(L, L->ws, k, block_chunk(1, nullptr, 0), db, 0, dx, 0, nonzero_guess);
+  if (smoother_takes_fused_iteration(L, k, &flat_spmv)) {
+    ALFI_CHECK(smooth_fgmres_fused(L, k, db, dx, nonzero_guess, flat_spmv));
+  } else {
+    ALFI_CHECK(smooth_fgmres_general(L, L->ws, k, block_chunk(1, nullptr, 0), db, 0, dx, 0, nonzero_guess));
+  }
+  L->ws.res_k = k;
+  return 0;
+}
+
+int krylov_residual(alfi_level* L, const KrylovWs& ws, int k, const BlockCols& slots, double* R, int64_t ldr) {
+  alfi_ctx* ctx = L->ctx;
+  ctx->cur_tag = L->id;
+  const HsLayout hl(ws.K);
+  for (int i = 0; i < slots.n; ++i) {
+    const int s = slots.c[i];
+    ProfScope prof(ctx, ALFI_EV_BLAS1);
+    ALFI_CHECK(launch_krylov_residual(ctx, R + s * ldr, ws.v(s, 0), ws.ldv, k, ws.c(s), ws.wv(s), ws.h(s) + hl.tt, L->n_own));
+  }
+  return 0;
+}
+
+int alfi_smooth_fgmres_residual(alfi_level* L, int k, double* dr) {
+  if (!L) return alfi_set_error(nullptr, ALFI_E_ARG, "NULL level");
+  alfi_ctx* ctx = L->ctx;
+  if (!dr) return alfi_set_error(ctx, ALFI_E_ARG, "alfi_smooth_fgmres_residual: NULL vector");
+  if (level_is_partitioned(L))
+    return alfi_set_error(ctx, ALFI_E_ARG, "alfi_smooth_fgmres_residual on a partitioned level (serial levels only)");
+  if (k < 1 || L->ws.res_k != k)
+    return alfi_set_error(ctx, ALFI_E_STATE, "alfi_smooth_fgmres_residual(k = %d) does not follow alfi_smooth_fgmres with that k", k);
+  return krylov_residual(L, L->ws, k, block_chunk(1, nullptr, 0), dr, 0);
 }
 
 namespace {
@@ -163,7 +192,7 @@
   }
   for (int s = 0; s < nc; ++s) {
     ProfScope prof(ctx, ALFI_EV_BLAS1);
-    ALFI_CHECK(launch_fgmres_finish(ctx, ws.h(s), k, K));
+    ALFI_CHECK(launch_fgmres_finish(ctx, ws.h(s), k, K, ws.c(s)));
     ALFI_CHECK(launch_update_solution(ctx, X + cols.c[s] * ldx, ws.z(s, 0), ldv, k, ws.h(s) + hl.y, n));
   }
   return 0;
diff --git a/alfi_amd/csrc/common.h b/alfi_amd/csrc/common.h
--- a/alfi_amd/csrc/common.h
+++ b/alfi_amd/csrc/common.h
@@ -417,6 +417,7 @@
   int smoother = 0;
   std::vector<double> emin, emax;
   int cycles = 1;
+  bool krylov_residual = true;
   double *cg_r = nullptr, *cg_z = nullptr, *cg_p = nullptr, *cg_w = nullptr, *cg_s = nullptr;
   std::vector<CycleGraph> graphs;
 };
@@ -562,7 +563,7 @@
 int launch_multi_dot(alfi_ctx* ctx, const double* V, int64_t stride, int nv, const double* w, double* out, int64_t n);
 int launch_multi_axpy_norm(alfi_ctx* ctx, const double* V, int64_t stride, int nv, double* h, double* w, int64_t n,
                            double* norm_partial, int hblocks);
-int launch_fgmres_finish(alfi_ctx* ctx, double* hs, int k, int K);
+int launch_fgmres_finish(alfi_ctx* ctx, double* hs, int k, int K, double* c);
 int launch_patch_sum_scale(alfi_level* lvl, const double* w, double* z, double* v, const double* normpart, int nblocks,
                            const double* h, double* hs, int j, int K);
 int launch_bsr_spmv_dot(alfi_ctx* ctx, const DevBSR& A, const double* z, double* w, const double* V, int64_t stride, int nv,
@@ -585,7 +586,10 @@
 int launch_apply_bc(alfi_level* lvl);
 int launch_patch_invert_mfma(alfi_ctx* ctx, int64_t npatch, int max_np, const int64_t* patch_ptr, const int64_t* inv_ptr,
                              double* inv, int* status, int* handled);
-int launch_fgmres_finish_fused(alfi_ctx* ctx, const double* normpart, int nblocks, const double* h, double* hs, int k, int K);
+int launch_fgmres_finish_fused(alfi_ctx* ctx, const double* normpart, int nblocks, const double* h, double* hs, int k, int K,
+                               double* c);
+int launch_krylov_residual(alfi_ctx* ctx, double* r, const double* V, int64_t stride, int k, const double* c, const double* w,
+                           const double* tt, int64_t n);
 int launch_update_solution(alfi_ctx* ctx, double* x, const double* Z, int64_t stride, int k, const double* y, int64_t n);
 int launch_cheb_update(alfi_ctx* ctx, double* d, double* x, const double* z, double a, double c, int64_t n, int mode);
 int launch_jacobi_diag(alfi_ctx* ctx, const DevBSR& A, double* diag);
diff --git a/alfi_amd/csrc/hs_layout.h b/alfi_amd/csrc/hs_layout.h
--- a/alfi_amd/csrc/hs_layout.h
+++ b/alfi_amd/csrc/hs_layout.h
@@ -19,6 +19,25 @@
   }
   HS_LAYOUT_HD int H(int j) const { return 8 + j * (K + 1); }
 };
+
+HS_LAYOUT_HD inline void fgmres_residual_coefficients(const double* hs, int k, int K, double* c) {
+  HsLayout L(K);
+  const double* y = hs + L.y;
+  const double* grs = hs + L.grs;
+  const double* cs = hs + L.cs;
+  const double* sn = hs + L.sn;
+  for (int i = 0; i < k; ++i) {
+    double s = grs[i];
+    for (int q = i; q < k; ++q) s -= hs[L.H(q) + i] * y[q];
+    c[i] = s;
+  }
+  c[k] = grs[k];
+  for (int i = k - 1; i >= 0; --i) {
+    const double a = c[i], b = c[i + 1];
+    c[i] = cs[i] * a - sn[i] * b;
+    c[i + 1] = sn[i] * a + cs[i] * b;
+  }
+}
 #undef HS_LAYOUT_HD
 
 #ifdef __HIPCC__
diff --git a/alfi_amd/csrc/kernels_block_fused.hip b/alfi_amd/csrc/kernels_block_fused.hip
--- a/alfi_amd/csrc/kernels_block_fused.hip
+++ b/alfi_amd/csrc/kernels_block_fused.hip
@@ -291,7 +291,7 @@
 
 __global__ __launch_bounds__(256) void fgmres_finish_fused_block_kernel(const double* __restrict__ normpart, int64_t pstride,
                                                                         int nblocks, double* __restrict__ hsb, int64_t hstride,
-                                                                        int k, int K) {
+                                                                        int k, int K, double* __restrict__ rcb) {
   double s2[1];
   block_reduce_partials<1>(normpart + blockIdx.y * pstride, nblocks, s2);
   if (threadIdx.x != 0) return;
@@ -306,6 +306,7 @@
     const double d = hs[L.H(i) + i];
     y[i] = d != 0.0 ? s / d : 0.0;
   }
+  fgmres_residual_coefficients(hs, k, K, rcb + blockIdx.y * (K + 1));
 }
 
 template <int NV, bool VEC>
@@ -533,7 +534,7 @@
   const Slots S = slots_of(L, cols.n);
   if (k < 1 || k > 16) return alfi_set_error(ctx, ALFI_E_STATE, "block fused update with %d vectors", k);
   hipLaunchKernelGGL(fgmres_finish_fused_block_kernel, dim3(1, (unsigned)S.nc), dim3(256), 0, ctx->stream, S.part2, S.pstride,
-                     nblocks, S.hs, S.hstride, k, S.K);
+                     nblocks, S.hs, S.hstride, k, S.K, L->blk_ws.rc);
   ALFI_HIP_CHECK(ctx, hipGetLastError());
   if (S.n <= 0) return 0;
   const bool vec = vec2_ok(S.Z, X + (int64_t)cols.c[0] * ldx, S.ldv) && (ldx & 1) == 0;
diff --git a/alfi_amd/csrc/kernels_vec.hip b/alfi_amd/csrc/kernels_vec.hip
--- a/alfi_amd/csrc/kernels_vec.hip
+++ b/alfi_amd/csrc/kernels_vec.hip
@@ -865,9 +865,10 @@
   if (threadIdx.x == 0) hessenberg_column(hs, K, j, h, sqrt(ww ? pythagoras_norm2(ww, h, j) : red[0]));
 }
 
-__global__ void fgmres_finish_kernel(double* __restrict__ hs, int k, int K) {
+__global__ void fgmres_finish_kernel(double* __restrict__ hs, int k, int K, double* __restrict__ c) {
   if (threadIdx.x != 0 || blockIdx.x != 0) return;
   fgmres_back_substitution(hs, k, K);
+  if (c) fgmres_residual_coefficients(hs, k, K, c);
 }
 
 #define ALFI_NV_SWITCH(NVAL, MACRO) \
@@ -1092,7 +1093,7 @@
 
 __global__ __launch_bounds__(256) void fgmres_finish_fused_kernel(const double* __restrict__ normpart, int nblocks,
                                                                   const double* __restrict__ h, double* __restrict__ hs,
-                                                                  int k, int K) {
+                                                                  int k, int K, double* __restrict__ c) {
   double s2[1];
   block_reduce_partials<1>(normpart, nblocks, s2);
   if (threadIdx.x != 0) return;
@@ -1106,15 +1107,17 @@
     const double d = hs[L.H(i) + i];
     y[i] = d != 0.0 ? s / d : 0.0;
   }
-}
-int launch_fgmres_finish_fused(alfi_ctx* ctx, const double* normpart, int nblocks, const double* h, double* hs, int k, int K) {
-  hipLaunchKernelGGL(fgmres_finish_fused_kernel, dim3(1), dim3(256), 0, ctx->stream, normpart, nblocks, h, hs, k, K);
-  ALFI_HIP_CHECK(ctx, hipGetLastError());
-  return 0;
-}
-
-int launch_fgmres_finish(alfi_ctx* ctx, double* hs, int k, int K) {
-  hipLaunchKernelGGL(fgmres_finish_kernel, dim3(1), dim3(64), 0, ctx->stream, hs, k, K);
+  fgmres_residual_coefficients(hs, k, K, c);
+}
+int launch_fgmres_finish_fused(alfi_ctx* ctx, const double* normpart, int nblocks, const double* h, double* hs, int k, int K,
+                               double* c) {
+  hipLaunchKernelGGL(fgmres_finish_fused_kernel, dim3(1), dim3(256), 0, ctx->stream, normpart, nblocks, h, hs, k, K, c);
+  ALFI_HIP_CHECK(ctx, hipGetLastError());
+  return 0;
+}
+
+int launch_fgmres_finish(alfi_ctx* ctx, double* hs, int k, int K, double* c) {
+  hipLaunchKernelGGL(fgmres_finish_kernel, dim3(1), dim3(64), 0, ctx->stream, hs, k, K, c);
   ALFI_HIP_CHECK(ctx, hipGetLastError());
   return 0;
 }
@@ -1141,6 +1144,79 @@
   return 0;
 }
 
+template <int NV, bool VEC>
+__global__ __launch_bounds__(256) void krylov_residual_kernel(const double* __restrict__ V, int64_t stride,
+                                                               const double* __restrict__ c, const double* __restrict__ w,
+                                                               const double* __restrict__ tt, bool first,
+                                                               double* __restrict__ r, int64_t n) {
+  double cv[NV];
+#pragma unroll
+  for (int v = 0; v < NV; ++v) cv[v] = c[v];
+  double cw = 0.0;
+  if (w) cw = *tt != 0.0 ? c[NV] / *tt : 0.0;
+  if (VEC) {
+    const int64_t n2 = n >> 1;
+#pragma unroll 2
+    for (int64_t i = (int64_t)blockIdx.x * 256 + threadIdx.x; i < n2; i += (int64_t)gridDim.x * 256) {
+      vec_d2 ri;
+      ri.x = 0.0;
+      ri.y = 0.0;
+      if (!first) ri = ld2(r, i);
+#pragma unroll
+      for (int v = 0; v < NV; ++v) {
+        const vec_d2 a = ld2(V + v * stride, i);
+        ri.x = __builtin_fma(cv[v], a.x, ri.x);
+        ri.y = __builtin_fma(cv[v], a.y, ri.y);
+      }
+      if (w) {
+        const vec_d2 a = ld2(w, i);
+        ri.x = __builtin_fma(cw, a.x, ri.x);
+        ri.y = __builtin_fma(cw, a.y, ri.y);
+      }
+      st2(r, i, ri);
+    }
+    if ((n & 1) && blockIdx.x == 0 && threadIdx.x == 0) {
+      double ri = first ? 0.0 : r[n - 1];
+#pragma unroll
+      for (int v = 0; v < NV; ++v) ri = __builtin_fma(cv[v], V[v * stride + n - 1], ri);
+      if (w) ri = __builtin_fma(cw, w[n - 1], ri);
+      r[n - 1] = ri;
+    }
+  } else {
+    for (int64_t i = (int64_t)blockIdx.x * 256 + threadIdx.x; i < n; i += (int64_t)gridDim.x * 256) {
+      double ri = first ? 0.0 : r[i];
+#pragma unroll
+      for (int v = 0; v < NV; ++v) ri = __builtin_fma(cv[v], V[v * stride + i], ri);
+      if (w) ri = __builtin_fma(cw, w[i], ri);
+      r[i] = ri;
+    }
+  }
+}
+
+int launch_krylov_residual(alfi_ctx* ctx, double* r, const double* V, int64_t stride, int k, const double* c, const double* w,
+                           const double* tt, int64_t n) {
+  for (int v0 = 0; v0 < k; v0 += 16) {
+    const int cnt = k - v0 < 16 ? k - v0 : 16;
+    const double* wl = v0 + cnt == k ? w : nullptr;
+    const bool first = v0 == 0;
+    const bool vec = vec2_ok(V + (int64_t)v0 * stride, r, stride) && vec2_ok(w, r, stride);
+    const dim3 grid = ew_grid(vec ? (n + 1) / 2 : n);
+#define ALFI_CASE(N)                                                                                                   \
+  case N:                                                                                                              \
+    if (vec)                                                                                                           \
+      hipLaunchKernelGGL((krylov_residual_kernel<N, true>), grid, dim3(256), 0, ctx->stream, V + (int64_t)v0 * stride, \
+                         stride, c + v0, wl, tt, first, r, n);                                                         \
+    else                                                                                                               \
+      hipLaunchKernelGGL((krylov_residual_kernel<N, false>), grid, dim3(256), 0, ctx->stream, V + (int64_t)v0 * stride, \
+                         stride, c + v0, wl, tt, first, r, n);                                                         \
+    break;
+    ALFI_NV_SWITCH(cnt, ALFI_CASE)
+#undef ALFI_CASE
+    ALFI_HIP_CHECK(ctx, hipGetLastError());
+  }
+  return 0;
+}
+
 __global__ void block_build_kernel(int64_t nblk, int m, int ld, int64_t stride, const double* __restrict__ K,
                                    const double* __restrict__ D, double nu, double gamma, double* __restrict__ S) {
   const int64_t total = nblk * m * ld;
diff --git a/alfi_amd/csrc/krylov_ws.h b/alfi_amd/csrc/krylov_ws.h
--- a/alfi_amd/csrc/krylov_ws.h
+++ b/alfi_amd/csrc/krylov_ws.h
@@ -6,8 +6,9 @@
 inline int64_t krylov_ldv(int64_t n) { return (n + 1) & ~(int64_t)1; }
 
 struct KrylovWs {
-  double *V = nullptr, *Z = nullptr, *w = nullptr, *hs = nullptr;
+  double *V = nullptr, *Z = nullptr, *w = nullptr, *hs = nullptr, *rc = nullptr;
   int K = 0, slots = 0;
+  int res_k = 0;
   int64_t ldv = 0;
   int64_t vs() const { return (int64_t)(K + 1) * ldv; }
   int64_t zs() const { return (int64_t)K * ldv; }
@@ -16,15 +17,16 @@
   double* z(int s, int j) const { return Z + s * zs() + j * ldv; }
   double* wv(int s) const { return w + s * ldv; }
   double* h(int s) const { return hs + s * hstride(); }
+  double* c(int s) const { return rc + s * (K + 1); }
 };
 struct KrylovWsDoubles {
-  int64_t V, Z, w, hs;
+  int64_t V, Z, w, hs, rc;
 };
 inline KrylovWsDoubles krylov_ws_doubles(int slots, int K, int64_t ldv) {
   KrylovWs t;
   t.K = K;
   t.ldv = ldv;
-  return {slots * t.vs(), slots * t.zs(), slots * ldv, slots * t.hstride()};
+  return {slots * t.vs(), slots * t.zs(), slots * ldv, slots * t.hstride(), (int64_t)slots * (K + 1)};
 }
 
 struct SlotBuf {
diff --git a/alfi_amd/hip.py b/alfi_amd/hip.py
--- a/alfi_amd/hip.py
+++ b/alfi_amd/hip.py
@@ -547,6 +547,9 @@
 
     def smooth(self, k, b, x, nonzero_guess=True):
         self.ctx.check(self.ctx.lib.alfi_smooth_fgmres(self.h, int(k), b.ptr, x.ptr, 1 if nonzero_guess else 0))
+
+    def smooth_residual(self, k, r):
+        self.ctx.check(self.ctx.lib.alfi_smooth_fgmres_residual(self.h, int(k), r.ptr))
 
     def patch_apply_block(self, X, Y, cols=None):
         ncol, cp, nx, keep = _block_args(self.n, cols, X, Y)
@@ -856,6 +859,9 @@
             raise ValueError("cycle type %r (v or w)" % (kind,))
         self.ctx.check(self.ctx.lib.alfi_mg_set_cycles(self.h, self.CYCLES[kind]))
 
+    def set_krylov_residual(self, on):
+        self.ctx.check(self.ctx.lib.alfi_mg_set_krylov_residual(self.h, 1 if on else 0))
+
     def chebyshev_bounds(self, steps=10, esteig=(0.0, 0.1, 0.0, 1.1), seed=0):
         a, b, c, d = (float(t) for t in esteig)
         out = []
diff --git a/include/alfi_hip.h b/include/alfi_hip.h
--- a/include/alfi_hip.h
+++ b/include/alfi_hip.h
@@ -134,6 +134,7 @@
 int alfi_patch_get_inverse(alfi_level* lvl, int64_t p, double* out_host);
 
 int alfi_smooth_fgmres(alfi_level* lvl, int k, const double* db, double* dx, int nonzero_guess);
+int alfi_smooth_fgmres_residual(alfi_level* lvl, int k, double* dr);
 
 int alfi_level_set_jacobi(alfi_level* lvl, int on);
 int alfi_smooth_chebyshev(alfi_level* lvl, int k, double emin, double emax, const double* db, double* dx, int nonzero_guess);
@@ -174,6 +175,7 @@
 #define ALFI_SMOOTHER_CHEBYSHEV 1
 int alfi_mg_set_smoother(alfi_mg* mg, int type, const double* emin_host, const double* emax_host);
 int alfi_mg_set_cycles(alfi_mg* mg, int cycles);
+int alfi_mg_set_krylov_residual(alfi_mg* mg, int on);
 int alfi_mg_cg(alfi_mg* mg, const double* db, double* dx, double rtol, double atol, int max_it, int full, int* iterations,
                double* residual_norm);
 int alfi_ctx_set_graph(alfi_ctx* ctx, int on);
```

Result: no change. 9.140, median of 3 (+2.0%).
